# ZJU-FAST-Lab/Implicit-SVSDF-Planner

Measured on AMD Instinct MI355X. Metric: SVSDF query-points/sec (cost+grad) per optimizer evaluation, higher is better.
Workload: dtype f64

## Files before the change

implicit-svsdf-planner_amd/csrc/svsdf_body_classify.hpp:

```cpp
  extern __shared__ double classify_lds[];
  const TrajL tr = stage_traj(trg, classify_lds);
  const int start = ctl->start, count = ctl->count;
  const int lane = (int)(threadIdx.x & 63);
  for (int e0 = (int)((blockIdx.x * blockDim.x + threadIdx.x) & ~63u); e0 < count; e0 += gridDim.x * blockDim.x) {
    const int e = e0 + lane;
    const bool in_range = e < count;
    const int i = start + (in_range ? e : 0);
    const double px = px_[i], py = py_[i];
    const double sdf = sdf_[i], ts = t_[i];
    const bool inter = in_range && !(sdf > 0);
    double vx = 0.0, vy = 0.0, w = 0.0;
    if (in_range && sdf > 0) {
      int piece = 0;
      const Pose p = pose_at(tr, ts, piece);
      double rx, ry;
      if constexpr (SC) {
        double i00, i11;
        scale_inv(scl, ts, i00, i11);
        rel_scaled(p, px, py, i00, i11, rx, ry);
      } else {
        const double dx = px - p.x, dy = py - p.y;
        rx = p.cs * dx + p.sn * dy;
        ry = (-p.sn) * dx + p.cs * dy;
      }
      double gx, gy;
      shape_grad<SHAPE>(sp, rx, ry, gx, gy);
      res_sdf[i] = sdf; res_t[i] = ts; res_gx[i] = gx; res_gy[i] = gy;
    } else if (inter) {
      double sl;
      int piece = locate_local(tr, ts, 0, sl);
      piece_vel(tr.c + piece * 18, sl, vx, vy, w);
      if (sqrt(vx * vx + vy * vy + w * w) < 0.01) {
        if (ts < 0.1) {
          for (double t_scan = ts; t_scan <= tr.dur; t_scan += 0.1) {
            piece = locate_local(tr, t_scan, piece, sl);
            piece_vel(tr.c + piece * 18, sl, vx, vy, w);
            if (sqrt(vx * vx + vy * vy + w * w) >= 0.01) break;
          }
        } else if (ts > tr.dur - 0.1) {
          for (double t_scan = ts; t_scan >= 0; t_scan -= 0.1) {
// ... 41 lines not shown
```

implicit-svsdf-planner_amd/csrc/svsdf_capi.hip:

```cpp
#include "svsdf_ctx.hpp"

using namespace svsdf;
using namespace svsdf_impl;

namespace {

double shape_circumradius(int shape_id, const double *poly_xy, int nverts) {
  switch (shape_id) {
    case SVSDF_SHAPE_sdUnevenCapsule: return 6.0;
    case SVSDF_SHAPE_sdCutDisk: return 5.0;
    case SVSDF_SHAPE_sdTrapezoid: return std::sqrt(3.0 * 3.0 + 2.0 * 2.0);
    case SVSDF_SHAPE_sdRhombus: return 4.5;
    case SVSDF_SHAPE_star: return 2.8;
    case SVSDF_SHAPE_sdTunnel: return std::sqrt(2.5 * 2.5 + 1.5 * 1.5);
    case SVSDF_SHAPE_sdHorseshoe: return std::hypot(1.5 + 0.20, 1.55);
    case SVSDF_SHAPE_sdHeart: return 4.0 * (std::sqrt(0.25 * 0.25 + 0.75 * 0.75) + std::sqrt(2.0) / 4.0);
    case SVSDF_SHAPE_sdOrientedVesica: return std::sqrt(2.0 * 2.0 + 4.0 * 4.0);
    case SVSDF_SHAPE_sdRoundedCross: return 2.0;
    case SVSDF_SHAPE_sdRoundedX: return 3.0 / std::sqrt(2.0) + 0.25;
    case SVSDF_SHAPE_bigX: return 5.0 / std::sqrt(2.0) + 0.25;
    case SVSDF_SHAPE_sdMoon: return 3.0;
    case SVSDF_SHAPE_sdPie: return 3.0;
    case SVSDF_SHAPE_sdPie2: return 3.0;
    case SVSDF_SHAPE_sdArc: return 2.3333 + 0.5;
// ... 136 lines not shown
    pa.hdr.slabs = reinterpret_cast<const PolyRec *>(ctx->d_poly + o_slab);
    pa.hdr.over = reinterpret_cast<const unsigned short *>(ctx->d_poly + o_over);
    std::memcpy(blob.data(), &pa.hdr, sizeof(PolyAccel));
    std::memcpy(blob.data() + o_edges, pa.edges.data(), pa.edges.size() * sizeof(PolyEdge));
    std::memcpy(blob.data() + o_cell, pa.cells.data(), pa.cells.size() * sizeof(PolyRec));
    std::memcpy(blob.data() + o_slab, pa.slabs.data(), pa.slabs.size() * sizeof(PolyRec));
    if (!pa.over.empty()) std::memcpy(blob.data() + o_over, pa.over.data(), pa.over.size() * sizeof(unsigned short));
    if (hipMemcpy(ctx->d_poly, blob.data(), total, hipMemcpyHostToDevice) != hipSuccess)
      return bail("hipMemcpy polygon failed");
    sp.nverts = (int)pa.edges.size();
    sp.accel = reinterpret_cast<const PolyAccel *>(ctx->d_poly);
    sp.edges = pa.hdr.edges;
    ctx->poly_lds = sp.nverts <= kPolyLdsMaxVerts;
    if (const char *e = std::getenv("SVSDF_POLY_LDS")) ctx->poly_lds = ctx->poly_lds && std::atoi(e) != 0;
    ctx->cfg.polygon_nverts = (int)(v.size() / 2);
    ctx->cfg.polygon_nloops = (int)loops.size();
  }
  ctx->G_env = 0;
  if (const char *e = std::getenv("SVSDF_G")) { const int g = std::atoi(e); if (g == 1 || g == 2 || g == 4 || g == 8 || g == 16 || g == 32) { ctx->G_env = g; ctx->G = g; ctx->G_late = std::max(g, 8); } }
  if (const char *e = std::getenv("SVSDF_G_LATE")) { const int g = std::atoi(e); if (g == 1 || g == 2 || g == 4 || g == 8 || g == 16 || g == 32) { ctx->G_late = g; ctx->G_late_env = g; } }
  if (const char *e = std::getenv("SVSDF_PRUNE")) ctx->prune = std::atoi(e) != 0;
  if (const char *e = std::getenv("SVSDF_BATCHES")) ctx->want_batches = (std::string(e) == "measure") ? -1 : std::max(0, std::min(std::atoi(e), (int)kMaxBatches));
  if (const char *e = std::getenv("SVSDF_SELECT_DELTA")) { ctx->select_delta = std::atof(e); ctx->select_env = true; }
  {
    int n = 0;
    if (hipDeviceGetAttribute(&n, hipDeviceAttributeMultiprocessorCount, ctx->device) == hipSuccess && n > 0) ctx->n_cu = n;
    if (hipDeviceGetAttribute(&n, hipDeviceAttributeMaxSharedMemoryPerBlock, ctx->device) == hipSuccess && n > 0) ctx->lds_limit = (size_t)n;
    if (hipDeviceGetAttribute(&n, hipDeviceAttributeWallClockRate, ctx->device) == hipSuccess && n > 0) ctx->wall_clock_khz = (double)n;
  }
  if (const char *e = std::getenv("SVSDF_CULL")) { ctx->cull = std::atoi(e) != 0; ctx->cull2 = std::atoi(e) >= 2; }
  if (const char *e = std::getenv("SVSDF_ROUND_BPC")) ctx->round_blocks_per_cu = std::max(1, std::min(std::atoi(e), 16));
  if (const char *e = std::getenv("SVSDF_SCAN_ANCHORS")) ctx->scan_anchors = std::atoi(e) != 0;
  if (const char *e = std::getenv("SVSDF_LAYER_TABLES")) { const int v = std::atoi(e); ctx->layer_tables = (std::string(e) == "auto") ? -1 : (v == 0 || v == 2 || v == 3) ? v : -1; }
  if (const char *e = std::getenv("SVSDF_TAIL_DUO")) ctx->tail_duo = std::atoi(e) != 0;
  if (const char *e = std::getenv("SVSDF_TAIL_LOCAL")) ctx->tail_local = std::atoi(e) != 0;
  if (const char *e = std::getenv("SVSDF_TAIL_LATENCY")) ctx->tail_latency = std::atoi(e) != 0;
  if (const char *e = std::getenv("SVSDF_TAIL")) ctx->tail_mode = (std::string(e) == "off") ? -2 : (std::string(e) == "auto") ? -1 : std::max(0, std::atoi(e));
  if (const char *e = std::getenv("SVSDF_UB_FULL")) { ctx->ub_full = std::atoi(e) != 0; ctx->ub_lazy = std::atoi(e) == 2; ctx->ub_anchor = std::atoi(e) == 3; ctx->ub_env = true; }
  if (const char *e = std::getenv("SVSDF_PROFILE")) ctx->profile = std::atoi(e) != 0;
  if (const char *e = std::getenv("SVSDF_PIECE_TIME")) {
    ctx->cfg.flags &= ~(SVSDF_FLAG_EXACT_PIECE_TIME | SVSDF_FLAG_FAST_PIECE_TIME);
    if (std::string(e) == "exact") ctx->cfg.flags |= SVSDF_FLAG_EXACT_PIECE_TIME;
    else if (std::string(e) == "fast") ctx->cfg.flags |= SVSDF_FLAG_FAST_PIECE_TIME;
  }
  for (int b = 0; b < kMaxBatches; ++b) {
    if (hipEventCreateWithFlags(&ctx->ev_done[b], hipEventDisableTiming) != hipSuccess)
      return bail("event creation failed");
  }
  if (hipEventCreateWithFlags(&ctx->ev_prep, hipEventDisableTiming) != hipSuccess) return bail("event creation failed");
  if (hipMalloc((void **)&ctx->d_traj, sizeof(TrajDev)) != hipSuccess ||
      hipMalloc((void **)&ctx->d_ctl, kMaxBatches * sizeof(BatchCtl) + 8 * 8 * (kMaxIter + 4)) != hipSuccess ||
      hipMalloc((void **)&ctx->d_nonfinite, sizeof(int)) != hipSuccess ||
      hipMalloc((void **)&ctx->d_sums, kOutPartial * sizeof(double)) != hipSuccess ||
      hipMalloc((void **)&ctx->d_out, kOutDoubles * sizeof(double)) != hipSuccess ||
      hipHostMalloc((void **)&ctx->h_out, kOutDoubles * sizeof(double), hipHostMallocDefault) != hipSuccess ||
      hipMalloc((void **)&ctx->d_ticket, sizeof(unsigned)) != hipSuccess)
    return bail("device allocation failed");
  if (hipMemsetAsync(ctx->d_ticket, 0, sizeof(unsigned), ctx->stream) != hipSuccess) return bail("hipMemset failed");
  {
    void *dp = nullptr;
    const char *e = std::getenv("SVSDF_HOST_WRITE");
    if (!(e && std::atoi(e) == 0) && hipHostGetDevicePointer(&dp, ctx->h_out, 0) == hipSuccess) ctx->h_out_dev = (double *)dp;
    (void)hipGetLastError();
  }
  if (hipMemsetAsync(ctx->d_ctl, 0, kMaxBatches * sizeof(BatchCtl) + 8 * 8 * (kMaxIter + 4), ctx->stream) != hipSuccess) return bail("hipMemset failed");
  {
    const double r0 = shape_circumradius(cfg->shape_id, ctx->poly_xy.data(), (int)(ctx->poly_xy.size() / 2));
    const double analytic = (r0 + std::hypot(sp.tx, sp.ty)) * (1.0 + 1e-12) + 1e-6;
    if (hipMemsetAsync(ctx->d_out, 0, 2 * sizeof(double), ctx->stream) != hipSuccess) return bail("hipMemset failed");
    const int nrad = 512, nang = 4096;
    const unsigned grid = (unsigned)((nrad * nang + kBlock - 1) / kBlock);
    (void)launch_k_rbound(cfg->shape_id, grid, ctx->stream, ctx->sp, 60.0, nrad, nang, ctx->d_out);
    double rbl[2] = {0.0, 0.0};
    if (hipMemcpyAsync(rbl, ctx->d_out, 2 * sizeof(double), hipMemcpyDeviceToHost, ctx->stream) != hipSuccess ||
        hipStreamSynchronize(ctx->stream) != hipSuccess)
      return bail("shape bound kernel failed");
    const double rb = rbl[0];
    ctx->r_bound_sampled = rb;
    ctx->lipschitz_excess = rbl[1];
    const char *nl = std::getenv("SVSDF_ASSUME_NOT_LIPSCHITZ");
    if (rbl[1] > 0.0 || (nl && std::atoi(nl) != 0)) { ctx->lipschitz_ok = false; ctx->cull2 = false; }
    if (rb > analytic)
      return bail("svsdf_create: sampled shape bound " + std::to_string(rb) + " exceeds the analytic circumradius " +
                  std::to_string(analytic) + " (internal error: the pruning bound would be unsafe)");
    ctx->r_bound = analytic;
    ctx->sp.r_bound = ctx->r_bound;
  }
  return ctx;
}

void svsdf_destroy(svsdf_ctx *ctx) {
  if (!ctx) return;
  if (ctx->host_only) { delete ctx; return; }
  if (!ctx->subs.empty() || !ctx->workers.empty()) {
    destroy_group_resources(ctx);
    for (svsdf_ctx *s : ctx->subs) svsdf_destroy(s);
    delete ctx;
    return;
  }
  (void)hipSetDevice(ctx->device);
  (void)hipDeviceSynchronize();
  void *bufs[] = {ctx->d_poly, ctx->d_px, ctx->d_py, ctx->d_traj, ctx->d_in, ctx->d_pose, ctx->d_chunks, ctx->d_ltab,
                  ctx->d_sdf, ctx->d_t, ctx->d_res_sdf, ctx->d_res_t, ctx->d_res_gx, ctx->d_res_gy, ctx->gs.pt,
                  ctx->gs.r, ctx->gs.theta0, ctx->gs.theta_res, ctx->gs.iter, ctx->gs.nsamp, ctx->gs.phase, ctx->gs.req,
                  ctx->gs.list[0], ctx->gs.list[1], ctx->gs.solve, ctx->gs.sqx, ctx->gs.sqy, ctx->gs.sqth,
                  ctx->gs.sq_ub, ctx->gs.sq_k, ctx->gs.sq_sdf, ctx->gs.sq_t, ctx->d_ctl,
                  ctx->d_block_partials, ctx->d_sums,
                  ctx->d_out, ctx->d_nonfinite, ctx->d_fe, ctx->d_fe_flag, ctx->d_ticket};
  for (void *p : bufs)
    if (p) (void)hipFree(p);
  if (ctx->h_in) (void)hipHostFree(ctx->h_in);
  if (ctx->h_out) (void)hipHostFree(ctx->h_out);
  if (ctx->h_fe) (void)hipHostFree(ctx->h_fe);
  for (hipEvent_t e : ctx->ev_pool) (void)hipEventDestroy(e);
  if (ctx->ev_prep) (void)hipEventDestroy(ctx->ev_prep);
  for (int b = 0; b < kMaxBatches; ++b)
    if (ctx->ev_done[b]) (void)hipEventDestroy(ctx->ev_done[b]);
  if (ctx->stream_slot >= 0) {
    StreamSet ss;
    ss.main = ctx->stream;
    for (int b = 0; b < kMaxBatches; ++b) ss.batch[b] = ctx->bstream[b];
    ss.slot = ctx->stream_slot;
    release_streams(ctx->device, ss);
  }
  delete ctx;
}

int svsdf_set_points(svsdf_ctx *ctx, const double *xyz_aos, size_t P) {
  if (!ctx || (!xyz_aos && P)) return fail(ctx, SVSDF_ERR_INVALID, "svsdf_set_points: null argument");
  return set_points_host(ctx, xyz_aos, P);
}

int svsdf_set_points_device(svsdf_ctx *ctx, const double *d_xyz_aos, size_t P) {
  if (!ctx || (!d_xyz_aos && P)) return fail(ctx, SVSDF_ERR_INVALID, "svsdf_set_points_device: null argument");
  if (ctx->host_only) return fail(ctx, SVSDF_ERR_NO_DEVICE, "host-only context: no device entry points");
  if (P > 0xffffffffull) return fail(ctx, SVSDF_ERR_INVALID, "too many points");
  if (ctx->subs.empty()) {
    const auto t0 = std::chrono::steady_clock::now();
// ... 159 lines not shown
    const int nb = ctx->saved_nbatch;
    ctx->saved_nbatch = 0;
    HIPCHK(hipSetDevice(ctx->device));
    return set_batches(ctx, nb);
  }
  return SVSDF_OK;
}

int svsdf_shape_bound(const svsdf_ctx *ctx, double out2[2]) {
  if (!ctx || !out2) return SVSDF_ERR_INVALID;
  const svsdf_ctx *c = ctx->subs.empty() ? ctx : ctx->subs[0];
  out2[0] = c->r_bound;
  out2[1] = c->r_bound_sampled;
  return SVSDF_OK;
}

int svsdf_shape_selfcheck(const svsdf_ctx *ctx, double out3[3]) {
  if (!ctx || !out3) return SVSDF_ERR_INVALID;
  const svsdf_ctx *c = ctx->subs.empty() ? ctx : ctx->subs[0];
  out3[0] = c->r_bound;
  out3[1] = c->r_bound_sampled;
  out3[2] = c->lipschitz_ok ? 0.0 : std::max(c->lipschitz_excess, 1e-300);
  return SVSDF_OK;
}

int svsdf_get_plan(const svsdf_ctx *ctx, svsdf_plan *out) {
  if (!ctx || !out) return SVSDF_ERR_INVALID;
  const svsdf_ctx *c = ctx->subs.empty() ? ctx : ctx->subs[0];
  out->bound_mode = bound_mode_of(c);
  out->batches = (c->saved_nbatch > 0) ? c->saved_nbatch : c->nbatch;
  out->lanes_per_query = (c->scaled && c->G > 0) ? svsdf::scaled_lanes(c->G) : c->G;
  out->tail_iter = (c->tail_mode == -2 || c->scaled) ? -2 : (c->tail_mode >= 0) ? c->tail_mode : (c->have_prev_nactive ? choose_tail_iter(c) : SVSDF_PLAN_AUTO);
  out->layer_tables = c->layer_tables;
  out->settled = ((c->ub_env || c->ub_tune > 0) && c->bt_state == 0 && c->an_state == 0 && c->lz_state == 0 && c->have_prev_nsolve) ? 1 : 0;
  return SVSDF_OK;
}

int svsdf_set_plan(svsdf_ctx *ctx, const svsdf_plan *plan) {
  if (!ctx || !plan) return fail(ctx, SVSDF_ERR_INVALID, "svsdf_set_plan: null argument");
  const int g = plan->lanes_per_query;
  if (plan->bound_mode < SVSDF_PLAN_AUTO || plan->bound_mode > 3 || plan->batches < -2 || plan->batches == 0 || plan->batches > kMaxBatches ||
      !(g == SVSDF_PLAN_AUTO || g == 1 || g == 2 || g == 4 || g == 8 || g == 16 || g == 32) || plan->tail_iter < -2 || plan->tail_iter >= kMaxIter ||
      !(plan->layer_tables == SVSDF_PLAN_AUTO || plan->layer_tables == 0 || plan->layer_tables == 2 || plan->layer_tables == 3))
    return fail(ctx, SVSDF_ERR_INVALID, "svsdf_set_plan: field out of range");
  if (!ctx->subs.empty()) {
    int rc = SVSDF_OK;
    for (svsdf_ctx *s : ctx->subs) { const int r = svsdf_set_plan(s, plan); if (r && !rc) { rc = r; ctx->err = s->err; } }
    return rc;
  }
  if (ctx->host_only) return SVSDF_OK;
  HIPCHK(hipSetDevice(ctx->device));
  ctx->layer_tables = plan->layer_tables;
  if (plan->bound_mode == SVSDF_PLAN_AUTO) {
    if (ctx->ub_env) { ctx->ub_env = false; ctx->ub_tune = 0; ctx->have_prev_nsolve = false; ctx->have_prev_nactive = false; }
  } else {
    const bool full = plan->bound_mode != 0, lazy = plan->bound_mode == 2, anchor = plan->bound_mode == 3;
    if (!ctx->ub_env || full != ctx->ub_full || lazy != ctx->ub_lazy || anchor != ctx->ub_anchor) { ctx->have_prev_nsolve = false; ctx->have_prev_nactive = false; ctx->ub_tune = 0; }
    ctx->ub_env = true; ctx->ub_full = full; ctx->ub_lazy = lazy; ctx->ub_anchor = anchor; ctx->an_state = 0; ctx->lz_state = 0;
  }
  ctx->want_batches = (plan->batches == SVSDF_PLAN_AUTO) ? 0 : (plan->batches == -2) ? -1 : plan->batches;
  ctx->bt_state = 0;
  if (ctx->want_batches <= 0) ctx->ub_tune = 0;
  else if (ctx->points_set) {
    if (ctx->saved_nbatch > 0) ctx->saved_nbatch = ctx->want_batches;
    else if (ctx->nbatch != ctx->want_batches) { const int rc = set_batches(ctx, ctx->want_batches); if (rc) return rc; }
  }
  ctx->G_env = (g == SVSDF_PLAN_AUTO) ? 0 : g;
  if (ctx->G_env) { ctx->G = g; if (!ctx->G_late_env) ctx->G_late = std::max(g, 8); }
  else if (ctx->points_set) {
    const size_t Ps = ctx->P;
    ctx->G = default_lanes(ctx, Ps);
    if (!ctx->G_late_env) ctx->G_late = std::max(ctx->G, 8);
  }
  ctx->tail_mode = (plan->tail_iter == SVSDF_PLAN_AUTO) ? -1 : plan->tail_iter;
  return SVSDF_OK;
}

int svsdf_set_scale(svsdf_ctx *ctx, const svsdf_scale *scale) {
  if (!ctx) return SVSDF_ERR_INVALID;
  svsdf::ScaleDev d{};
  bool on = false;
  if (scale) {
    if (scale->struct_size != (int)sizeof(svsdf_scale))
      return fail(ctx, SVSDF_ERR_INVALID, "svsdf_set_scale: struct_size is not sizeof(svsdf_scale)");
    on = scale->enabled != 0;
// ... 213 lines not shown
```

implicit-svsdf-planner_amd/csrc/svsdf_ctx.hpp:

```cpp
#pragma once
#include <hip/hip_runtime.h>

#include <dlfcn.h>

#include <algorithm>
#include <chrono>
#include <cmath>
#include <condition_variable>
#include <cstdint>
#include <cstdio>
#include <cstdlib>
#include <cstring>
#include <functional>
#include <limits>
#include <memory>
#include <mutex>
#include <numeric>
#include <string>
#include <thread>
#include <vector>

#include "../../include/svsdf_c.h"
#include "svsdf_launch.hpp"
#include "svsdf_minco.hpp"
// ... 29 lines not shown
    done = false;
    cv.notify_all();
  }
  int wait() {
    std::unique_lock<std::mutex> lk(m);
    cv.wait(lk, [this] { return done; });
    return rc;
  }
  ~Worker() {
    { std::lock_guard<std::mutex> lk(m); quit = true; cv.notify_all(); }
    if (th.joinable()) th.join();
  }
};

struct svsdf_ctx {
  svsdf_config cfg{};
  int device = 0;
  hipStream_t stream = nullptr;
  hipStream_t bstream[svsdf::kMaxBatches] = {};
  int stream_slot = -1;
  hipEvent_t ev_prep = nullptr, ev_done[svsdf::kMaxBatches] = {};
  svsdf::ShapeParams sp{};
  bool poly_lds = false;
  unsigned char *d_poly = nullptr;
  std::vector<double> poly_xy;
  std::vector<int> poly_loops;
  std::string err;

  size_t P = 0;
  bool points_set = false;
  std::vector<long long> shard_idx;
  double *d_px = nullptr, *d_py = nullptr;
  int nbatch = 1;
  int bstart[svsdf::kMaxBatches] = {}, bcount[svsdf::kMaxBatches] = {};
  svsdf::BatchCtl *d_ctl = nullptr;

  svsdf::TrajDev *d_traj = nullptr;
  double *d_in = nullptr;
  double *h_in = nullptr;
  size_t in_cap = 0;
  svsdf::Pose *d_pose = nullptr;
  svsdf::Chunk *d_chunks = nullptr;
  size_t pose_cap = 0;
  svsdf::Pose *d_ltab = nullptr;
  size_t ltab_cap = 0;
  int layer_tables = -1;
  int ltab_mode = 0;
  long long prev_solves = 0;
  double r_bound = 0.0;
  double r_bound_sampled = 0.0;
  double lipschitz_excess = 0.0;
  bool lipschitz_ok = true;
  double traj_duration = 0.0;
  bool have_duration = false;
  bool host_only = false;
  int N = 0, K = 0;
  int piece_time_mode = 0;
  int stats_piece_time = 0;

  int G = 0 , G_late = 8, prune = 1, block = 64, want_batches = 0, waves_per_cu = 16;
  bool block_env = false;
  int late_iter = 4, first_iters = 12, it_done = 0, round_lp8_iters = 3, delta_all_iter = 5;
  int n_cu = 256;
  int round_blocks_per_cu = 4;
  double wall_clock_khz = 100000.0;
  bool adaptive_iters = true;
  bool ub_full = false;
// ... 3 lines not shown
  unsigned long long an_full_evals = 0;
  int lz_state = 0;
  unsigned long long lz_cheap_solves = 0;
  bool ub_env = false;
  int ub_tune = 0;
  double ub_ratio = 0.0;
  double ub_threshold = 0.5;
  bool ub_thr_env = false;
  bool scan_anchors = true;
  int round_list = 3;
  bool cull = true;
  bool cull_ok = false;
  bool cull2 = true;
  double slack_max = 0.0;
  int G_env = 0, G_late_env = 0;
  int bt_state = 0, bt_k = 0, bt_rep = 0, bt_ncand = 0, bt_cand[3] = {1, 1, 1};
  double bt_ms[3] = {0, 0, 0}, bt_samples[3] = {0, 0, 0};
  long long prev_nsolve[svsdf::kMaxIter] = {};
  bool have_prev_nsolve = false;
  int tail_mode = -1;
  long long tail_below = 0;
  int tail_all_after = 1 << 30;
  int tail_iter = -1;
  bool tail_duo = true;
  bool tail_latency = true;
  bool tail_local = true;
  long long prev_nactive[svsdf::kMaxIter] = {};
  int prev_tail_iter = -1;
  bool have_prev_nactive = false;
  long long wide32_below = 2000, wide16_below = 5000, wide8_below = 40000;
  bool select_env = false, all_iter_env = false;
  double scan_delta = 0.002;
  double select_delta = 0.1;
  bool scaled = false;
  svsdf::ScaleDev scale{};

  double *d_sdf = nullptr, *d_t = nullptr;
  double *d_res_sdf = nullptr, *d_res_t = nullptr, *d_res_gx = nullptr, *d_res_gy = nullptr;
  svsdf::GsipState gs{};
  size_t icap = 0;
  bool icap_fitted = false;
  double *d_block_partials = nullptr;
  size_t block_partials_cap = 0;
  double *d_sums = nullptr;
  double *d_out = nullptr;
  double *h_out = nullptr;
  double *h_out_dev = nullptr;
  unsigned *d_ticket = nullptr;
  int *d_nonfinite = nullptr;
  int h_nonfinite = 0;
  size_t e_end = 0;

  double *d_fe = nullptr, *h_fe = nullptr;
  size_t fe_cap = 0;
  int *d_fe_flag = nullptr;
  std::vector<int> h_fe_flag;
  size_t fe_edges_cap = 0;

  bool profile = false;
  bool profile_span = false;
  int saved_nbatch = 0;
  std::vector<hipEvent_t> ev_pool;
  size_t ev_used = 0;
  std::vector<std::pair<size_t, size_t>> refine_events;
  std::vector<std::pair<size_t, size_t>> round_events;
  std::vector<std::pair<size_t, size_t>> tail_events;
  svsdf_stats stats{};
  svsdf_launch_rec launches[SVSDF_LAUNCH_REC_CAP];
  int n_launches = 0;

  std::vector<svsdf_ctx *> subs;
  std::vector<std::unique_ptr<Worker>> workers;
  int combine = 0;
  std::vector<void *> comms;
  std::vector<double *> d_red;
  double *h_red = nullptr;
  std::vector<double> comb;
  const double *h_partial = nullptr;
  double combine_ms = 0.0, setup_ms = 0.0, fanout_ms = 0.0;
  bool group_serial = false;

  std::vector<double> ol_key, ol_xy;
  std::vector<int> ol_loops;
  svsdf_outline_stats ol_stats{};
  bool ol_valid = false;
  size_t lds_limit = 65536;
  std::string launch_err;

  svsdf_host::MincoS3 minco;
  std::vector<double> T, pgC, pgT, cm, gC, gradq, gradT, xlast;
  double energy_cost = 0.0;
  double costs3[3] = {0, 0, 0};
};

namespace svsdf_impl {

constexpr size_t kOutPartial = 19 * svsdf::kMaxPieces + 1;
constexpr size_t kOutDoubles = kOutPartial + 14 + 2 * svsdf::kMaxIter;
constexpr int kRepeat = -12345;

extern thread_local std::string g_last_error;
extern const char *kShapeNames[SVSDF_SHAPE_COUNT];
int fail(svsdf_ctx *ctx, int code, const std::string &msg);

#define HIPCHK(expr)                                                                              \
  do {                                                                                            \
    hipError_t e_ = (expr);                                                                       \
    if (e_ != hipSuccess)                                                                         \
      return fail(ctx, SVSDF_ERR_HIP_BASE + (int)e_, std::string(#expr) + ": " + hipGetErrorString(e_)); \
  } while (0)

template <typename T>
int dev_alloc(svsdf_ctx *ctx, T **p, size_t count) {
  if (*p) { (void)hipFree(*p); *p = nullptr; }
  if (count == 0) count = 1;
  HIPCHK(hipMalloc((void **)p, count * sizeof(T)));
  return SVSDF_OK;
}

inline int bound_mode_of(const svsdf_ctx *c) { return c->ub_full ? (c->ub_lazy ? 2 : ((c->ub_anchor && c->lipschitz_ok) ? 3 : 1)) : 0; }
inline int default_lanes(const svsdf_ctx *ctx, size_t Ps) {
  const int g = (Ps < 3000) ? 32 : (Ps < 20000) ? 16 : (Ps < 75000) ? 8 : (Ps < 150000) ? 4 : 2;
  return (ctx->cfg.shape_id == (int)svsdf::kPolygon) ? std::max(g, 4) : g;
}

struct StreamSet { hipStream_t main = nullptr; hipStream_t batch[svsdf::kMaxBatches] = {}; int slot = -1; };
bool acquire_streams(int device, StreamSet &out);
void release_streams(int device, StreamSet &s);
int set_batches(svsdf_ctx *ctx, int nb);
int choose_tail_iter(const svsdf_ctx *ctx);
int swept_field(svsdf_ctx *ctx, int N, const double *coeffs, const double *T, double *sdf_sorted);
int evaluate_points(svsdf_ctx *ctx, int N, const double *coeffs, const double *T, bool allow_cull, bool with_partial);
void fill_mode_stats(svsdf_ctx *ctx);
inline void reset_launches(svsdf_ctx *ctx) { ctx->n_launches = 0; }
inline svsdf_launch_rec *record_launch(svsdf_ctx *ctx, int kernel, int shape, unsigned grid, unsigned block, size_t lds,
                                       long long work, int batch) {
  if (ctx->n_launches >= SVSDF_LAUNCH_REC_CAP) { ++ctx->n_launches; return nullptr; }
  svsdf_launch_rec *r = &ctx->launches[ctx->n_launches++];
  *r = svsdf_launch_rec{};
  r->struct_size = (int)sizeof(svsdf_launch_rec);
  r->kernel = kernel; r->shape = shape; r->grid = grid; r->block = block; r->lds_bytes = lds; r->work = work; r->batch = batch;
  return r;
}
int compiled_shape(int shape);
int run_pipeline_leaf(svsdf_ctx *ctx, int N, const double *coeffs, const double *T);
void accumulate(int N, const double *partial, double *cost, double *gradT, double *gradC);
void shard_plan(const double *xyz, size_t P, int rk, int ws, int flags, std::vector<long long> &out);
struct CloudPlan {
  int device = 0;
  const double *d_xyz = nullptr;
  size_t P = 0;
  double *d_part = nullptr;
  unsigned long long *d_keys = nullptr, *d_keys2 = nullptr;
  const unsigned long long *sorted = nullptr;
  void *d_tmp = nullptr;
  void release();
};
int plan_cloud(svsdf_ctx *ctx, const double *d_xyz, size_t P, CloudPlan &plan);
int take_stripe(svsdf_ctx *ctx, svsdf_ctx *planner, const CloudPlan &plan, int rk, int ws);
int upload_shard_device(svsdf_ctx *ctx, const double *d_xyz, size_t P, int rk, int ws);
long long sincos_mismatches(svsdf_ctx *ctx, double lo, double hi, int n);
int debug_sdf_at(svsdf_ctx *ctx, int N, const double *coeffs, const double *T, size_t n, const double *pxy, const double *t, double *out8);
// ... 13 lines not shown
```

implicit-svsdf-planner_amd/csrc/svsdf_group.hip:

```cpp
#include "svsdf_ctx.hpp"

using namespace svsdf;

namespace svsdf_impl {

int upload_group_device(svsdf_ctx *ctx, const double *d_xyz, size_t P) {
  const int G = (int)ctx->subs.size();
  svsdf_ctx *s0 = ctx->subs[0];
  CloudPlan plan;
  int rc = plan_cloud(s0, d_xyz, P, plan);
  for (int k = 0; k < G && !rc; ++k) {
    rc = take_stripe(ctx->subs[k], s0, plan, ctx->cfg.rank * G + k, ctx->cfg.world_size * G);
    if (rc) {
      ctx->err = "device " + std::to_string(ctx->subs[k]->device) + " (stripe " + std::to_string(k) + "): " + ctx->subs[k]->err;
      g_last_error = ctx->err;
    }
  }
  if (rc && ctx->err.empty()) ctx->err = s0->err;
  plan.release();
  ctx->P = 0;
  ctx->shard_idx.clear();
  for (svsdf_ctx *s : ctx->subs) {
    if (rc) { s->P = 0; s->points_set = false; }
    ctx->P += s->P;
// ... 71 lines not shown
    if (!h)
      for (const char *name : {"librccl.so.1", "librccl.so", "/opt/rocm/lib/librccl.so.1"}) {
        h = dlopen(name, RTLD_NOW | RTLD_LOCAL);
        if (h) break;
      }
    if (!h) return false;
    CommInitAll = reinterpret_cast<decltype(CommInitAll)>(dlsym(h, "ncclCommInitAll"));
    CommDestroy = reinterpret_cast<decltype(CommDestroy)>(dlsym(h, "ncclCommDestroy"));
    AllReduce = reinterpret_cast<decltype(AllReduce)>(dlsym(h, "ncclAllReduce"));
    GetErrorString = reinterpret_cast<decltype(GetErrorString)>(dlsym(h, "ncclGetErrorString"));
    CommCount = reinterpret_cast<decltype(CommCount)>(dlsym(h, "ncclCommCount"));
    return CommInitAll && CommDestroy && AllReduce;
  }
};
RcclApi g_rccl;
constexpr int kNcclFloat64 = 8, kNcclSum = 0;

void merge_stats(svsdf_ctx *ctx) {
  svsdf_stats t{};
  for (svsdf_ctx *s : ctx->subs) {
    const svsdf_stats &a = s->stats;
    t.points += a.points; t.interior_points += a.interior_points; t.solves += a.solves;
    t.gsip_samples += a.gsip_samples; t.sdf_evals += a.sdf_evals; t.scan_evals += a.scan_evals;
    t.round_scan_evals += a.round_scan_evals; t.speculative_evals += a.speculative_evals;
    t.round_ms = std::max(t.round_ms, a.round_ms); t.round_ms_sum = std::max(t.round_ms_sum, a.round_ms_sum);
    t.batches = std::max(t.batches, a.batches);
    t.culled_points += a.culled_points;
    t.device_ms = std::max(t.device_ms, a.device_ms); t.solve_ms = std::max(t.solve_ms, a.solve_ms);
    t.solve_ms_sum = std::max(t.solve_ms_sum, a.solve_ms_sum);
    t.solve_launches = std::max(t.solve_launches, a.solve_launches);
    t.tail_launches = std::max(t.tail_launches, a.tail_launches);
    t.tail_iter = std::max(t.tail_iter, a.tail_iter);
    t.tail_points += a.tail_points;
    t.tail_ms = std::max(t.tail_ms, a.tail_ms); t.tail_ms_sum = std::max(t.tail_ms_sum, a.tail_ms_sum);
    t.gsip_iterations = std::max(t.gsip_iterations, a.gsip_iterations);
    t.gsip_bound_mode = std::max(t.gsip_bound_mode, a.gsip_bound_mode);
    t.piece_time_exact = std::max(t.piece_time_exact, a.piece_time_exact);
    t.bound_ratio = std::max(t.bound_ratio, a.bound_ratio);
    if (a.shader_clock_mhz > 0.0) t.shader_clock_mhz = (t.shader_clock_mhz > 0.0) ? std::min(t.shader_clock_mhz, a.shader_clock_mhz) : a.shader_clock_mhz;
  }
  t.bound_mode_decided = 1;
  t.plan_settled = 1;
  for (svsdf_ctx *s : ctx->subs) { t.bound_mode_decided &= s->stats.bound_mode_decided; t.plan_settled &= s->stats.plan_settled; }
  t.n_devices = (int)ctx->subs.size();
  t.combine = ctx->combine;
  t.combine_ms = ctx->combine_ms;
  t.fanout_ms = ctx->fanout_ms;
  t.setup_ms = ctx->setup_ms;
  ctx->stats = t;
}

int run_pipeline_group(svsdf_ctx *ctx, int N, const double *coeffs, const double *T) {
  const int G = (int)ctx->subs.size();
  const size_t plen = 19 * (size_t)N + 1;
  const bool rccl = ctx->combine == SVSDF_COMBINE_RCCL;
  int rc = group_run(ctx, [&](int k) -> int {
    svsdf_ctx *s = ctx->subs[k];
    int r = run_pipeline_leaf(s, N, coeffs, T);
    if (!rccl) return r;
    (void)hipSetDevice(s->device);
    if (r) (void)hipMemsetAsync(s->d_out, 0xFF, plen * sizeof(double), s->stream);
    const int e = g_rccl.AllReduce(s->d_out, ctx->d_red[k], plen, kNcclFloat64, kNcclSum, ctx->comms[k], s->stream);
    if (e && !r) r = fail(s, SVSDF_ERR_RCCL, std::string("ncclAllReduce: ") + (g_rccl.GetErrorString ? g_rccl.GetErrorString(e) : "error"));
    if (k == 0 && hipMemcpyAsync(ctx->h_red, ctx->d_red[0], plen * sizeof(double), hipMemcpyDeviceToHost, s->stream) != hipSuccess && !r)
      r = fail(s, SVSDF_ERR_RCCL, "read-back of the reduced partial failed");
    if (hipStreamSynchronize(s->stream) != hipSuccess && !r) r = fail(s, SVSDF_ERR_RCCL, "stream sync after ncclAllReduce failed");
// ... 137 lines not shown
```

implicit-svsdf-planner_amd/csrc/svsdf_kernels.hpp:

```cpp
#pragma once
#include <hip/hip_runtime.h>

#include "svsdf_shapes.hpp"

namespace svsdf {

#ifndef SVSDF_SOLVE_WAVES
#define SVSDF_SOLVE_WAVES 1
#endif
#ifndef SVSDF_ELASTIC
#define SVSDF_ELASTIC 1
#endif
#ifndef SVSDF_FUSED_PASS
#define SVSDF_FUSED_PASS 1
#endif
constexpr int kMaxPieces = 128;
constexpr int kMaxSlots = 24;
constexpr int kMaxRounds = 9;
constexpr int kBlock = 256;
constexpr int kMaxBatches = 8;
constexpr int kMaxCand = 48;
constexpr int kMaxIter = 24;
constexpr int kWorkCounters = kMaxIter + 2;
constexpr double kUnsolved = -1e300;
// ... 7 lines not shown
  double S[kMaxPieces + 1];
  double c[kMaxPieces * 18];
};

struct Pose { double x, y, cs, sn; };
constexpr int kLayerSteps = 21;
struct LayerTab { const Pose *l2, *l3; };

constexpr int kChunk = 8;
struct Chunk { double cx, cy, rb, slack; };
struct ChunkAnchor { double adx, rot2; int ka, pad_; double pad2_; };
#ifndef SVSDF_ANCHOR_MIN
#define SVSDF_ANCHOR_MIN 3
#endif

constexpr int kStatSlots = 32;
#ifdef SVSDF_SITE_STATS
struct StatSlot { unsigned long long solves, evals, scan, culled, round_scan, spec, pad[26]; };
#else
struct StatSlot { unsigned long long solves, evals, scan, culled, round_scan, spec, pad[10]; };
#endif
__device__ __forceinline__ StatSlot *stat_slot(StatSlot *slots) {
  return slots + (((blockIdx.x * blockDim.x + threadIdx.x) >> 6) & (kStatSlots - 1));
}
struct BatchCtl {
  int start, count;
  int n_active[kMaxIter + 2];
  int n_solve[kMaxIter + 2];
  int n_seed[kMaxIter + 2];
  unsigned work[kWorkCounters];
  unsigned rwork[kMaxIter + 2];
  int nonfinite;
  int n_int;
  StatSlot stat[kStatSlots];
  unsigned long long clk[2];
};

typedef const __attribute__((address_space(4))) double *UniformDoubles;

struct TrajL {
  const double *T, *S, *c;
  UniformDoubles Tu;
  int N;
  int exact;
  double dur;
};

__host__ __device__ __forceinline__ int traj_lds_doubles(int N) { return 20 * N + 1; }

__device__ __forceinline__ TrajL stage_traj(const TrajDev *__restrict__ g, double *lds) {
  const int N = g->N;
  double *T = lds, *S = lds + N, *c = lds + 2 * N + 1;
  for (int i = threadIdx.x; i < N; i += blockDim.x) T[i] = g->T[i];
  for (int i = threadIdx.x; i <= N; i += blockDim.x) S[i] = g->S[i];
  for (int i = threadIdx.x; i < 18 * N; i += blockDim.x) c[i] = g->c[i];
  __syncthreads();
  TrajL tr;
  tr.T = T; tr.S = S; tr.c = c; tr.N = N; tr.dur = g->dur; tr.exact = g->exact;
  tr.Tu = (UniformDoubles)(g->T);
  return tr;
}

template <int SHAPE>
__device__ __forceinline__ void stage_poly_edges(const ShapeParams &sp, double *lds) {
  if constexpr (SHAPE == kPolygonLds) {
    const double *src = reinterpret_cast<const double *>(sp.edges);
    for (int i = threadIdx.x; i < kPolyEdgeDoubles * sp.nverts; i += blockDim.x) lds[i] = src[i];
  }
}
// ... 260 lines not shown
  const double dx = px - p.x, dy = py - p.y;
  rx = (p.cs * i00) * dx + (p.sn * i11) * dy;
  ry = ((-p.sn) * i00) * dx + (p.cs * i11) * dy;
}
template <int SHAPE>
__device__ __forceinline__ double sdf_at_sc(const TrajL &tr, const ShapeParams &sp, const ScaleDev &scl, double px,
                                            double py, double t, PieceCache &pc) {
  const Pose p = pose_at(tr, t, pc);
  double i00, i11, rx, ry;
  scale_inv(scl, t, i00, i11);
  rel_scaled(p, px, py, i00, i11, rx, ry);
  return shape_sdf<SHAPE>(sp, rx, ry);
}
template <int SHAPE>
__device__ __forceinline__ double sdf_at_sc(const TrajL &tr, const ShapeParams &sp, const ScaleDev &scl, double px,
                                            double py, double t, int &piece) {
  const Pose p = pose_at(tr, t, piece);
  double i00, i11, rx, ry;
  scale_inv(scl, t, i00, i11);
  rel_scaled(p, px, py, i00, i11, rx, ry);
  return shape_sdf<SHAPE>(sp, rx, ry);
}
template <int SHAPE, bool SC, typename PC>
__device__ __forceinline__ double sdf_desc(const TrajL &tr, const ShapeParams &sp, const ScaleDev &scl, double px,
                                           double py, double t, PC &pc) {
  if constexpr (SC) return sdf_at_sc<SHAPE>(tr, sp, scl, px, py, t, pc);
  else return sdf_at<SHAPE>(tr, sp, px, py, t, pc);
}

#ifdef SVSDF_API_TU
__global__ void __launch_bounds__(1024) k_prep(const double *__restrict__ in, int N, double dur, int K, int exact,
                       TrajDev *__restrict__ tr, Pose *__restrict__ pose,
                       Chunk *__restrict__ chunks, double r_bound, BatchCtl *__restrict__ ctl,
                       int nbatch, int *__restrict__ nonfinite) {
  extern __shared__ double prep_lds[];
  if (threadIdx.x == 0 && nonfinite) *nonfinite = 0;
  const double *coeffs = in, *T = in + 18 * N, *tk = in + 19 * N, *slack = in + 19 * N + K;
  for (int b = threadIdx.x; b < nbatch; b += blockDim.x) {
    BatchCtl &c = ctl[b];
    for (int r = 0; r < kMaxIter + 2; ++r) { c.n_active[r] = 0; c.n_solve[r] = 0; c.n_seed[r] = 0; }
    for (int r = 0; r < kWorkCounters; ++r) c.work[r] = 0u;
    for (int r = 0; r < kMaxIter + 2; ++r) c.rwork[r] = 0u;
    c.nonfinite = 0;
    c.n_int = 0;
    c.clk[0] = 0ull; c.clk[1] = 0ull;
  }
  for (int i = threadIdx.x; i < nbatch * kStatSlots; i += blockDim.x) {
    StatSlot &ss = ctl[i / kStatSlots].stat[i % kStatSlots];
    ss.solves = 0ull; ss.evals = 0ull; ss.scan = 0ull; ss.culled = 0ull; ss.round_scan = 0ull; ss.spec = 0ull;
#ifdef SVSDF_SITE_STATS
    for (int j = 0; j < 26; ++j) ss.pad[j] = 0ull;
#endif
  }
  if (threadIdx.x == 0) {
    tr->N = N; tr->K = K; tr->dur = dur; tr->exact = exact;
    double s = 0.0;
    for (int i = 0; i < N; ++i) { tr->T[i] = T[i]; tr->S[i] = s; s += T[i]; }
    tr->S[N] = s;
  }
  for (int e = threadIdx.x; e < 18 * N; e += blockDim.x) {
    const int i = e / 18, k = (e % 18) / 3, d = e % 3;
    tr->c[e] = coeffs[(size_t)d * 6 * N + 6 * i + k];
  }
  __threadfence_block();
  __syncthreads();
  const TrajL tl = stage_traj(tr, prep_lds);
  for (int k = threadIdx.x; k < K; k += blockDim.x) {
    int piece = 0;
    pose[k] = pose_at(tl, tk[k], piece);
// ... 54 lines not shown
constexpr int kLayerRows = kLayerSteps + 2;
__global__ void __launch_bounds__(256) k_layer_tables(const TrajDev *__restrict__ trg, const double *__restrict__ tk, int K,
                                                      int rows , Pose *__restrict__ out) {
  extern __shared__ double lt_lds[];
  const TrajL tr = stage_traj(trg, lt_lds);
  const long long e = (long long)blockIdx.x * blockDim.x + threadIdx.x;
  if (e >= (long long)K * rows * kLayerSteps) return;
  const int i = (int)(e % kLayerSteps), r = (int)((e / kLayerSteps) % rows), k = (int)(e / ((long long)kLayerSteps * rows));
  double seed = tk[k];
  double dt = 0.15;
  dt *= 0.1;
  if (r > 0) {
    if (r >= 2) {
      const double t0 = dmax(0.0, seed - 10 * dt);
      const double loop_terminal = dmin(tr.dur, seed + 10 * dt);
      double t = t0;
      for (int j = 0; j < r - 2; ++j) t += dt;
      if (!(t <= loop_terminal)) return;
      seed = t;
    }
    dt *= 0.1;
  }
  const double t0 = dmax(0.0, seed - 10 * dt);
  const double loop_terminal = dmin(tr.dur, seed + 10 * dt);
  double t = t0;
  for (int j = 0; j < i; ++j) t += dt;
  if (!(t <= loop_terminal)) return;
  PieceCache pc = piece_cache_init();
  Pose *dst = (r == 0) ? out + (size_t)k * kLayerSteps
                       : out + (size_t)K * kLayerSteps + ((size_t)k * (kLayerSteps + 1) + (size_t)(r - 1)) * kLayerSteps;
  dst[i] = pose_at(tr, t, pc);
}

#endif

template <int SHAPE>
__global__ void k_rbound(ShapeParams sp, double rmax, int nrad, int nang, double *__restrict__ out) {
  const int idx = blockIdx.x * blockDim.x + threadIdx.x;
  double v = -1e300, lip = -1e300;
  if (idx < nrad * nang) {
    const int ir = idx / nang, ia = idx % nang;
    const double r = rmax * (double)(ir + 1) / (double)nrad;
    const double a = 2.0 * kPI * (double)ia / (double)nang;
    const double x = r * cos(a), y = r * sin(a);
    const double f0 = shape_sdf<SHAPE>(sp, x, y);
    v = r - f0;
    auto excess = [&](double xx, double yy) {
      const double d = norm2(xx - x, yy - y);
      return fabs(shape_sdf<SHAPE>(sp, xx, yy) - f0) - d * (1.0 + 1e-9) - 1e-12;
    };
    const double r2 = rmax * (double)(ir + 2) / (double)nrad, a2 = 2.0 * kPI * (double)(ia + 1) / (double)nang;
    lip = fmax(fmax(excess(x + 1e-3, y), excess(x, y + 1e-3)), fmax(excess(r2 * cos(a), r2 * sin(a)), excess(r * cos(a2), r * sin(a2))));
  }
  for (int m = 32; m >= 1; m >>= 1) { v = fmax(v, __shfl_xor(v, m, 64)); lip = fmax(lip, __shfl_xor(lip, m, 64)); }
  if ((threadIdx.x & 63) == 0) {
    if (v > 0.0) atomicMax((unsigned long long *)out, (unsigned long long)__double_as_longlong(v));
    if (lip > 0.0) atomicMax((unsigned long long *)(out + 1), (unsigned long long)__double_as_longlong(lip));
  }
}

struct QuerySet {
  const double *qx, *qy;
  size_t stride;
  const int *count_ptr;
  int count_fixed;
  const int *list;
  int base;
  int n_outer;
  const int *slots;
  const int *seed_k;
  const double *seed_d;
};

__device__ __forceinline__ long long qs_total(const QuerySet &qs, int &n) {
  n = qs.count_ptr ? *qs.count_ptr : qs.count_fixed;
  return qs.slots ? (long long)n : (long long)n * qs.n_outer;
}
__device__ __forceinline__ bool qs_slot(const QuerySet &qs, int n, long long q, size_t &slot) {
  if (qs.slots) { slot = (size_t)qs.slots[q]; return true; }
  const int e = (int)(q % n), j = (int)(q / n);
  const int a = qs.list ? qs.list[e] : e;
  slot = (size_t)j * qs.stride + (size_t)qs.base + (size_t)a;
  return true;
}

#ifdef SVSDF_SITE_STATS
#define SVSDF_SITE(cnt, site, evaluates)                                                     \
  do {                                                                                       \
    const unsigned long long ex__ = __ballot(1);                                             \
    if ((int)(threadIdx.x & 63) == __ffsll((long long)ex__) - 1) ++(cnt)[site];              \
    if (evaluates) ++(cnt)[4 + (site)];                                                      \
  } while (0)
#define SVSDF_SITE_CLOCK() ((unsigned long long)__builtin_readcyclecounter())
#define SVSDF_SITE_CYCLES(cnt, slot, t0) do { if ((threadIdx.x & 63) == 0) (cnt)[slot] += SVSDF_SITE_CLOCK() - (t0); } while (0)
#define SVSDF_PHASE(cnt, slot, t0) do { if ((threadIdx.x & 63) == 0) { const unsigned long long n__ = SVSDF_SITE_CLOCK(); (cnt)[slot] += n__ - (t0); (t0) = n__; } } while (0)
#else
#define SVSDF_SITE(cnt, site, evaluates) do { } while (0)
#define SVSDF_SITE_CLOCK() 0ull
#define SVSDF_SITE_CYCLES(cnt, slot, t0) do { (void)(t0); } while (0)
#define SVSDF_PHASE(cnt, slot, t0) do { (void)(t0); } while (0)
#endif

template <int G>
struct Grp {
  static_assert(G == 1 || G == 2 || G == 4 || G == 8 || G == 16 || G == 32, "group size");
  __device__ static __forceinline__ int li() { return (int)(threadIdx.x & (G - 1)); }
  __device__ static __forceinline__ double bcast(double v, int src) {
    if constexpr (G == 1) return v; else return __shfl(v, src, G);
  }
  template <int STEP>
  __device__ static __forceinline__ int xchg(int v) {
    if constexpr (STEP == 0) return __builtin_amdgcn_update_dpp(v, v, 0xB1, 0xF, 0xF, false);
    else if constexpr (STEP == 1) return __builtin_amdgcn_update_dpp(v, v, 0x4E, 0xF, 0xF, false);
    else if constexpr (STEP == 2) return __builtin_amdgcn_update_dpp(v, v, 0x141, 0xF, 0xF, false);
    else if constexpr (STEP == 3) return __builtin_amdgcn_update_dpp(v, v, 0x140, 0xF, 0xF, false);
    else return __shfl_xor(v, 16, 32);
// ... 649 lines not shown
#define SVSDF_LAZY_REPS 2
#endif
enum : int { kPhaseEval = 0, kPhaseSupp = 1, kPhaseNew = 2 };
#ifndef SVSDF_LEAN_HANDOFF
#define SVSDF_LEAN_HANDOFF 0
#endif
#ifdef SVSDF_POINT_MAJOR
__host__ __device__ __forceinline__ size_t sample_slot(size_t , size_t ia, int j) { return ia * (size_t)kMaxSlots + (size_t)j; }
#else
__host__ __device__ __forceinline__ size_t sample_slot(size_t stride, size_t ia, int j) { return (size_t)j * stride + ia; }
#endif

struct GsipState {
  int *pt;
  double *r;
  double *theta0;
  double *theta_res;
  int *iter;
  int *nsamp;
  int *phase;
  unsigned *req;
  int *list[2];
  int *solve;
  double *sqx, *sqy, *sqth, *sq_ub, *sq_sdf, *sq_t;
  int *sq_k;
};

template <int SHAPE>
__global__ void __launch_bounds__(kBlock)
k_classify(const TrajDev *__restrict__ trg, ShapeParams sp, const double *__restrict__ px_,
           const double *__restrict__ py_, const double *__restrict__ sdf_,
           const double *__restrict__ t_, double *__restrict__ res_sdf,
           double *__restrict__ res_t, double *__restrict__ res_gx, double *__restrict__ res_gy,
           GsipState gs, BatchCtl *__restrict__ ctl, int *__restrict__ n_int, int icap) {
  constexpr bool SC = false;
  const ScaleDev scl{};
#include "svsdf_body_classify.hpp"
}
template <int SHAPE>
__global__ void __launch_bounds__(kBlock)
k_classify_sc(const TrajDev *__restrict__ trg, ShapeParams sp, const double *__restrict__ px_,
              const double *__restrict__ py_, const double *__restrict__ sdf_,
              const double *__restrict__ t_, double *__restrict__ res_sdf,
              double *__restrict__ res_t, double *__restrict__ res_gx, double *__restrict__ res_gy,
              GsipState gs, BatchCtl *__restrict__ ctl, int *__restrict__ n_int, int icap, ScaleDev scl) {
  constexpr bool SC = true;
#include "svsdf_body_classify.hpp"
}

template <int NP>
struct RoundOut {
  bool list_me[NP];
  unsigned mlist[NP];
  int n_emit;
  bool push_next, finished;
};
template <int SHAPE, int LP, int MODE, bool EAGER = false>
__device__ __forceinline__ void round_point(const ShapeParams &sp, const Pose *pose, const Chunk *chunks, int K, int nch,
                                            const double *__restrict__ px_, const double *__restrict__ py_,
                                            const GsipState &gs, size_t stride, int start, int a, double delta,
                                            double band_delta, double *__restrict__ res_sdf, double *__restrict__ res_t,
                                            double *__restrict__ res_gx, double *__restrict__ res_gy, unsigned &n_scan,
                                            RoundOut<(kMaxSlots + LP - 1) / LP> &out, unsigned short *clist, int clist_on,
                                            unsigned long long (&rc)[16], int duo = -1, const ChunkAnchor *__restrict__ anch_ = nullptr) {
#ifdef SVSDF_NO_SCAN_ANCHORS
  const ChunkAnchor *__restrict__ anch = nullptr; (void)anch_;
#else
#ifdef SVSDF_ANCHORS_NOT_LP8_M3
  const ChunkAnchor *__restrict__ anch = (MODE == 1 || (MODE == 3 && LP == 32)) ? anch_ : nullptr;
#else
  const ChunkAnchor *__restrict__ anch = ((MODE == 1 || MODE == 3) && !is_polygon<SHAPE>()) ? anch_ : nullptr;
#endif
#endif
  constexpr bool FULL = MODE == 1;
  unsigned long long tph = SVSDF_SITE_CLOCK();
  constexpr int NP = (kMaxSlots + LP - 1) / LP;
  const int l = (int)(threadIdx.x & (LP - 1));
  const unsigned lt_mask = (1u << l) - 1u;
// ... 673 lines not shown
  if (live) {
    const unsigned e = qlist[q];
    slot = (size_t)(e & 0x7fffffffu);
    px = gs.sqx[slot]; py = gs.sqy[slot];
    const bool seeded = (e >> 31) != 0u;
    if (seeded) { best_k = gs.sq_k[slot]; best_d = gs.sq_ub[slot]; }
    if (!seeded || best_k < 0) {
      bool culled;
      scan_layer1<SHAPE, G>(sp, pose, chunks, K, nch, px, py, prune, __longlong_as_double(0x7ff0000000000000ll), best_d, best_k,
                            culled, n_scan, nullptr, -1, nullptr);
    }
  }
  SVSDF_SITE_CYCLES(sc, 8, t_scan0);
  double x = 0.0, fx = 0.0;
  descend_from_seed<SHAPE, G, 1>(tr, tk, sp, px, py, live, best_k, best_d, x, fx, n_eval, n_spec, sc, wave_lds);
  if (live && li == 0) {
    gs.sq_sdf[slot] = fx;
    gs.sq_t[slot] = x;
    ++n_solved;
  }
}

#ifndef SVSDF_TAIL_WAVES
#define SVSDF_TAIL_WAVES 3
#endif
constexpr int kTailLatencyWaves = 2;
template <int SHAPE, int MODE, int WAVES = SVSDF_TAIL_WAVES>
__global__ void __launch_bounds__(kTailBlock, WAVES)
k_tail(const TrajDev *__restrict__ trg, const double *__restrict__ tk, const Pose *__restrict__ pose_g,
       const Chunk *__restrict__ chunks_g, ShapeParams sp, const double *__restrict__ px_, const double *__restrict__ py_,
       GsipState gs, size_t stride, int it0, int prev_mode, double delta, double band_delta, int all_after, int ppw,
       double *__restrict__ res_sdf, double *__restrict__ res_t, double *__restrict__ res_gx, double *__restrict__ res_gy,
       BatchCtl *__restrict__ ctl, int clist_on, int prune) {
  extern __shared__ double tail_lds[];
  constexpr int LP = 32;
  const int n_act = ctl->n_active[it0];
  const int wave_g = (int)((blockIdx.x * blockDim.x + threadIdx.x) >> 6);
  if (n_act <= 0 || (int)blockIdx.x * (kTailBlock / 64) * ppw >= n_act) return;
  const int K = trg->K;
  const int nch = (K + kChunk - 1) / kChunk;
  stage_poly_edges<SHAPE>(sp, tail_lds);
  double *tab_lds = tail_lds + poly_lds_doubles<SHAPE>(sp.nverts);
  Pose *pose = reinterpret_cast<Pose *>(tab_lds);
  Chunk *chunks = reinterpret_cast<Chunk *>(tab_lds + 4 * (size_t)K);
  {
    const double *src = reinterpret_cast<const double *>(pose_g);
    for (int i = threadIdx.x; i < 4 * K; i += blockDim.x) tab_lds[i] = src[i];
    const double *srcc = reinterpret_cast<const double *>(chunks_g);
    for (int i = threadIdx.x; i < 4 * nch; i += blockDim.x) tab_lds[4 * (size_t)K + i] = srcc[i];
  }
  const TrajL tr = stage_traj(trg, tab_lds + 4 * (size_t)K + 4 * (size_t)nch);
  const size_t tables = poly_lds_doubles<SHAPE>(sp.nverts) + 4 * (size_t)K + 4 * (size_t)nch + (size_t)traj_lds_doubles(tr.N);
  const bool local = it0 == 0 && (clist_on & 4) != 0;
  const size_t wave_stride = local ? kTailWaveLds : kTailWaveLds - kTailLocalBytes;
  char *wave_lds = reinterpret_cast<char *>(tail_lds + ((tables + 1) & ~(size_t)1)) + (threadIdx.x >> 6) * wave_stride;
  unsigned short *clist_w = reinterpret_cast<unsigned short *>(wave_lds + ((ladder_lds_bytes(2) + 15) & ~(size_t)15));
  unsigned *qlist = reinterpret_cast<unsigned *>(clist_w + 2 * kMaxCand);
  GsipState gl = gs;
  if (local) {
    double *ld = reinterpret_cast<double *>(qlist + 64);
    gl.r = ld; gl.theta0 = ld + 2; gl.theta_res = ld + 4;
    gl.sqx = ld + 6; gl.sqy = gl.sqx + 2 * kMaxSlots; gl.sqth = gl.sqy + 2 * kMaxSlots; gl.sq_ub = gl.sqth + 2 * kMaxSlots;
    gl.sq_sdf = gl.sq_ub + 2 * kMaxSlots; gl.sq_t = gl.sq_sdf + 2 * kMaxSlots;
    int *li_ = reinterpret_cast<int *>(gl.sq_t + 2 * kMaxSlots);
    gl.pt = li_; gl.iter = li_ + 2; gl.nsamp = li_ + 4; gl.phase = li_ + 6; gl.req = reinterpret_cast<unsigned *>(li_ + 8);
    gl.sq_k = li_ + 10;
  }
  const GsipState ga = local ? gl : gs;
  const size_t stride_a = local ? (size_t)2 : stride;
  const int start = ctl->start;
  const int *cur = gs.list[it0 & 1] + start;
  const int lane = (int)(threadIdx.x & 63);
  const int h = lane >> 5, l = lane & (LP - 1);
  const bool duo = ppw == 1 && MODE != 0 && (clist_on & 8) == 0;
  const int hs = duo ? 0 : h;
  const unsigned lt_mask = (1u << l) - 1u;
  unsigned n_eval = 0, n_scan = 0, n_solved = 0, n_spec = 0, n_rscan = 0;
  unsigned long long rc[16] = {0, 0, 0, 0, 0, 0, 0, 0, 0, 0, 0, 0, 0, 0, 0, 0};
  unsigned long long sc[12] = {0, 0, 0, 0, 0, 0, 0, 0, 0, 0, 0, 0};
  const unsigned long long t_wave0 = SVSDF_SITE_CLOCK();
  int n_emit_tot = 0;
  const int n_static = (int)(gridDim.x * (blockDim.x >> 6)) * ppw;
  int q_next = wave_g * ppw, q_end = min(wave_g * ppw + ppw, n_act);
  bool exhausted = false;
  int a = -1;
  int steps = 0;
  bool own = false;
  for (int guard = 0; guard < (1 << 24); ++guard) {
#pragma unroll
    for (int hh = 0; hh < 2; ++hh) {
      const int ah = __builtin_amdgcn_readlane(a, hh * 32);
      if (ah >= 0 || hh >= ppw) continue;
      if (q_next >= q_end && !exhausted) {
        unsigned b = 0;
        if (lane == 0) b = atomicAdd(&ctl->work[min(it0 + 1, kWorkCounters - 1)], (unsigned)kTailFetch);
        b = __builtin_amdgcn_readfirstlane(b);
        const long long bb = (long long)b + n_static;
        if (bb >= n_act) exhausted = true;
        else { q_next = (int)bb; q_end = (int)min((long long)n_act, bb + kTailFetch); }
      }
      if (q_next < q_end) {
        const int e = q_next++;
        if (h == hh || duo) {
          a = cur[e]; steps = 0; own = false;
          if (local && l == 0 && h == hh) {
            const size_t ia_ = (size_t)a;
            gl.pt[hs] = gs.pt[ia_]; gl.r[hs] = gs.r[ia_]; gl.theta0[hs] = gs.theta0[ia_]; gl.theta_res[hs] = gs.theta_res[ia_];
            gl.iter[hs] = gs.iter[ia_]; gl.nsamp[hs] = gs.nsamp[ia_]; gl.phase[hs] = gs.phase[ia_]; gl.req[hs] = 0u;
          }
        }
      }
    }
    if (__builtin_amdgcn_readlane(a, 0) < 0 && __builtin_amdgcn_readlane(a, 32) < 0) break;
    if (local) {
      __builtin_amdgcn_fence(__ATOMIC_RELEASE, "workgroup");
      __builtin_amdgcn_wave_barrier();
      __builtin_amdgcn_fence(__ATOMIC_ACQUIRE, "workgroup");
    }
    RoundOut<1> ro;
    ro.list_me[0] = false; ro.mlist[0] = 0u; ro.n_emit = 0; ro.push_next = false; ro.finished = false;
    if (a >= 0) {
      const double dl = (steps >= all_after) ? 1e300 : delta, bd = (steps >= all_after) ? 1e300 : band_delta;
      round_point<SHAPE, LP, MODE, true>(sp, pose, chunks, K, nch, px_, py_, ga, stride_a, start, local ? hs : a, dl, bd, res_sdf, res_t, res_gx,
                                   res_gy, n_rscan, ro, clist_w + (size_t)h * kMaxCand, clist_on, rc, duo ? h : -1,
                                   (clist_on & 16) ? reinterpret_cast<const ChunkAnchor *>(chunks_g + nch) : nullptr);
      ++steps;
      if (ro.n_emit > 0) own = true;
      if (l == 0 && (!duo || h == 0)) n_emit_tot += ro.n_emit;
    }
    const size_t ia = local ? (size_t)hs : (size_t)(a >= 0 ? a : 0);
    if (ro.finished) a = -1;
    const unsigned m_mine = (a >= 0 && (!duo || h == 0)) ? ro.mlist[0] : 0u;
    const int n0 = __popc((unsigned)__builtin_amdgcn_readlane((int)m_mine, 0));
    const int n1 = __popc((unsigned)__builtin_amdgcn_readlane((int)m_mine, 32));
    const int nq = n0 + n1;
    if ((m_mine >> l) & 1u) {
      const bool seeded = own ? (MODE != 0) : (prev_mode != 0);
      qlist[(h ? n0 : 0) + __popc(m_mine & lt_mask)] = (unsigned)sample_slot(stride_a, ia, l) | (seeded ? 0x80000000u : 0u);
    }
    __builtin_amdgcn_fence(__ATOMIC_RELEASE, "workgroup");
    __builtin_amdgcn_wave_barrier();
    __builtin_amdgcn_fence(__ATOMIC_ACQUIRE, "workgroup");
    if (nq > 0) {
      if (nq <= 2) {
        tail_solve_pass<SHAPE, 32>(tr, tk, sp, pose, chunks, K, nch, ga, qlist, 0, nq, prune, wave_lds, n_eval, n_scan, n_solved, n_spec, sc);
      } else if (nq <= 8) {
        tail_solve_pass<SHAPE, 8>(tr, tk, sp, pose, chunks, K, nch, ga, qlist, 0, nq, prune, wave_lds, n_eval, n_scan, n_solved, n_spec, sc);
      } else {
        for (int base = 0; base < nq; base += 32)
          tail_solve_pass<SHAPE, 2>(tr, tk, sp, pose, chunks, K, nch, ga, qlist, base, nq, prune, wave_lds, n_eval, n_scan, n_solved, n_spec, sc);
      }
      __builtin_amdgcn_fence(__ATOMIC_RELEASE, "workgroup");
      __builtin_amdgcn_wave_barrier();
      __builtin_amdgcn_fence(__ATOMIC_ACQUIRE, "workgroup");
    }
  }
  unsigned long long te = (unsigned long long)n_eval + n_scan, ts = n_solved, tc = n_scan, tp = n_spec, tr_ = n_rscan;
  int em = n_emit_tot;
#pragma unroll
  for (int m = 32; m >= 1; m >>= 1) {
    te += __shfl_xor(te, m, 64); ts += __shfl_xor(ts, m, 64); tc += __shfl_xor(tc, m, 64); tp += __shfl_xor(tp, m, 64);
    tr_ += __shfl_xor(tr_, m, 64); em += __shfl_xor(em, m, 64);
  }
  if (lane == 0 && (te || tr_ || em)) {
    StatSlot *ss = stat_slot(ctl->stat);
    if (te) atomicAdd(&ss->evals, te);
    if (ts) atomicAdd(&ss->solves, ts);
    if (tc) atomicAdd(&ss->scan, tc);
    if (tp) atomicAdd(&ss->spec, tp);
    if (tr_) atomicAdd(&ss->round_scan, tr_);
    if (em) atomicAdd(&ctl->n_seed[it0], em);
    if (ts) atomicAdd(&ctl->n_solve[it0], (int)ts);
  }
#ifdef SVSDF_SITE_STATS
  if (lane == 0) {
    rc[6] = SVSDF_SITE_CLOCK() - t_wave0;
    StatSlot *ss = stat_slot(ctl->stat);
    for (int i = 0; i < 8; ++i) if (rc[i]) atomicAdd(&ss->pad[12 + i], rc[i]);
    for (int i = 8; i < 11; ++i) if (sc[i]) atomicAdd(&ss->pad[i], sc[i]);
  }
  {
    unsigned long long ex = rc[8], ln = rc[12];
#pragma unroll
    for (int m = 32; m >= 1; m >>= 1) { ex += __shfl_xor(ex, m, 64); ln += __shfl_xor(ln, m, 64); }
    if (lane == 0 && ex) { StatSlot *ss = stat_slot(ctl->stat); atomicAdd(&ss->pad[20], ex); atomicAdd(&ss->pad[21], ln); }
    unsigned long long steps = ex;
#pragma unroll
    for (int i = 0; i < 4; ++i) {
      unsigned long long v = sc[i];
#pragma unroll
      for (int m = 32; m >= 1; m >>= 1) v += __shfl_xor(v, m, 64);
      steps += v;
    }
    if (lane == 0) { StatSlot *ss = stat_slot(ctl->stat); atomicMax(&ss->pad[22], steps); atomicMax(&ss->pad[23], rc[6]); }
  }
#pragma unroll
  for (int i = 0; i < 8; ++i) {
    unsigned long long v = sc[i];
#pragma unroll
    for (int m = 32; m >= 1; m >>= 1) v += __shfl_xor(v, m, 64);
    if (lane == 0 && v) atomicAdd(&stat_slot(ctl->stat)->pad[i], v);
  }
#endif
}

__device__ __forceinline__ bool smoothed_l1(double x, double mu, double &f, double &df) {
  if (x < 0.0) return false;
  else if (x > mu) { f = x - 0.5 * mu; df = 1.0; return true; }
  else {
    const double xdmu = x / mu;
    const double sqrxdmu = xdmu * xdmu;
    const double mumxd2 = mu - 0.5 * x;
    f = mumxd2 * sqrxdmu * xdmu;
    df = sqrxdmu * ((-0.5) * xdmu + 3.0 * mumxd2 / mu);
    return true;
  }
}

#ifdef SVSDF_API_TU
template <bool SC = false>
__device__ __forceinline__ bool assemble_terms(const TrajL &tr, const double *__restrict__ px_, const double *__restrict__ py_,
                                               int idx, const double *__restrict__ res_sdf, const double *__restrict__ res_t,
                                               const double *__restrict__ res_gx, const double *__restrict__ res_gy,
                                               double safety_hor, double weight_p, double (&v)[20], int &i, int &bad,
                                               const ScaleDev &scl = ScaleDev{}) {
  const double px = px_[idx], py = py_[idx];
  const double sdf_value = res_sdf[idx];
  const double time_star = res_t[idx];
  double gr0 = res_gx[idx], gr1 = res_gy[idx];
  if (!(sdf_value == sdf_value) || !(time_star == time_star) || !(gr0 == gr0) || !(gr1 == gr1)) ++bad;
  double sdf_cost = -1.0, sdf_out_grad = 0.0;
  smoothed_l1(safety_hor - sdf_value, 0.01, sdf_cost, sdf_out_grad);
  if (!(sdf_cost > 0)) return false;
  double s1;
  i = locate_local(tr, time_star, 0, s1);
  const double *c = tr.c + i * 18;
// ... 154 lines not shown
                                            const int *__restrict__ nonfinite, unsigned long long *__restrict__ stats_out) {
  for (int k = threadIdx.x; k <= 18 * N; k += blockDim.x) partial[k] = sums[k];
  if (threadIdx.x == 0) {
    double suf = 0.0;
    for (int j = N - 1; j >= 0; --j) { partial[1 + 18 * N + j] = suf; suf += sums[1 + 18 * N + j]; }
  }
  if (threadIdx.x < 64) {
    const int lane = (int)threadIdx.x;
    unsigned long long so = 0, ev = 0, sc = 0, cu = 0, rs = 0, sp_ = 0, seeded = 0, iters = 0, ns = 0, na = 0;
    for (int b = 0; b < nbatch; ++b) {
      if (lane < kStatSlots) {
        const StatSlot &ss = ctl[b].stat[lane];
        so += ss.solves; ev += ss.evals; sc += ss.scan; cu += ss.culled; rs += ss.round_scan; sp_ += ss.spec;
      }
      if (lane < kMaxIter) {
        ns += (unsigned long long)ctl[b].n_solve[lane];
        na += (unsigned long long)ctl[b].n_active[lane];
      }
      if (lane <= it_end && lane < kMaxIter + 2) {
        seeded += (unsigned long long)ctl[b].n_seed[lane];
        if (ctl[b].n_solve[lane] > 0 && (unsigned long long)(lane + 1) > iters) iters = (unsigned long long)(lane + 1);
      }
    }
#pragma unroll
    for (int m = 32; m >= 1; m >>= 1) {
      so += __shfl_xor(so, m, 64); ev += __shfl_xor(ev, m, 64); sc += __shfl_xor(sc, m, 64); cu += __shfl_xor(cu, m, 64);
      rs += __shfl_xor(rs, m, 64); sp_ += __shfl_xor(sp_, m, 64); seeded += __shfl_xor(seeded, m, 64);
      const unsigned long long oi = __shfl_xor(iters, m, 64);
      iters = (oi > iters) ? oi : iters;
    }
    if (lane < kMaxIter) {
      stats_out[9 + lane] = ns;
      stats_out[11 + kMaxIter + lane] = na;
    }
    if (lane == 0) {
      unsigned long long in = 0, nf = (unsigned long long)__hip_atomic_load(nonfinite, __ATOMIC_RELAXED, __HIP_MEMORY_SCOPE_AGENT), rem = 0;
      for (int b = 0; b < nbatch; ++b) {
        in += (unsigned long long)ctl[b].n_active[0]; nf += (unsigned long long)ctl[b].nonfinite;
        rem += (unsigned long long)ctl[b].n_solve[it_end];
      }
      stats_out[0] = so; stats_out[1] = ev; stats_out[2] = sc; stats_out[3] = in; stats_out[4] = nf;
      stats_out[5] = rem; stats_out[6] = seeded; stats_out[7] = iters; stats_out[8] = cu;
      stats_out[9 + kMaxIter] = rs;
      stats_out[10 + kMaxIter] = sp_;
      stats_out[11 + 2 * kMaxIter] = (unsigned long long)ctl[0].n_int;
      stats_out[12 + 2 * kMaxIter] = ctl[0].clk[0];
      stats_out[13 + 2 * kMaxIter] = ctl[0].clk[1];
    }
  }
}

__device__ __forceinline__ void copy_result_to_host(double *__restrict__ host_out, const double *__restrict__ out, int N,
                                                    int out_partial, int out_doubles) {
  const int plen = 19 * N + 1;
  for (int k = threadIdx.x; k < plen; k += blockDim.x) host_out[k] = out[k];
  for (int k = out_partial + threadIdx.x; k < out_doubles; k += blockDim.x) host_out[k] = out[k];
}

__global__ void k_finish(const double *__restrict__ sums, int N, double *__restrict__ partial,
                         const BatchCtl *__restrict__ ctl, int nbatch, int it_end,
                         const int *__restrict__ nonfinite, unsigned long long *__restrict__ stats_out,
                         double *__restrict__ host_out, int out_doubles) {
  finish_body(sums, N, partial, ctl, nbatch, it_end, nonfinite, stats_out);
  if (host_out) {
    __threadfence();
    __syncthreads();
    copy_result_to_host(host_out, partial, N, (int)(reinterpret_cast<const double *>(stats_out) - partial), out_doubles);
  }
}

__global__ void __launch_bounds__(kBlock)
k_reduce(const TrajDev *__restrict__ trg, const double *__restrict__ px_, const double *__restrict__ py_, int P,
         const double *__restrict__ res_sdf, const double *__restrict__ res_t, const double *__restrict__ res_gx,
         const double *__restrict__ res_gy, double safety_hor, double weight_p, double *__restrict__ block_partials,
         int *__restrict__ nonfinite, double *__restrict__ out, const BatchCtl *__restrict__ ctl, int nbatch, int it_end,
         int out_partial, int out_doubles, unsigned *__restrict__ ticket, double *__restrict__ host_out, int fuse) {
  constexpr bool SC = false;
  const ScaleDev scl{};
#include "svsdf_body_reduce.hpp"
}
// ... 87 lines not shown
```

implicit-svsdf-planner_amd/csrc/svsdf_launch.hpp:

```cpp
#pragma once
#include <hip/hip_runtime.h>

#include "svsdf_kernels.hpp"
#include "svsdf_frontend.hpp"

namespace svsdf {

constexpr int kNSlices = 4;

struct SolveLaunch {
  const TrajDev *traj; const double *tk; const Pose *pose; const Chunk *chunks; ShapeParams sp; QuerySet qs;
  double *out_sdf, *out_t; int prune; BatchCtl *ctl; int work_idx; double cull_thresh;
  const double *rot; double slack_max;
  const ScaleDev *scl = nullptr;
  const Pose *ltab = nullptr;
};
struct RoundLaunch {
  const TrajDev *traj; const Pose *pose; const Chunk *chunks; ShapeParams sp; const double *px, *py; GsipState gs;
  size_t stride; int it; double delta, band_delta; double *res_sdf, *res_t, *res_gx, *res_gy; BatchCtl *ctl;
  int clist_on;
};
struct TailLaunch {
  const TrajDev *traj; const double *tk; const Pose *pose; const Chunk *chunks; ShapeParams sp; const double *px, *py;
  GsipState gs; size_t stride; int it0, prev_mode; double delta, band_delta; int all_after, ppw;
  double *res_sdf, *res_t, *res_gx, *res_gy; BatchCtl *ctl; int clist_on, prune;
  int latency;
};
struct ClassifyLaunch {
  const TrajDev *traj; ShapeParams sp; const double *px, *py, *sdf, *t; double *res_sdf, *res_t, *res_gx, *res_gy;
  GsipState gs; BatchCtl *ctl; int *n_int; int icap;
  const ScaleDev *scl = nullptr;
};
constexpr int kScaledLanes[3] = {4, 8, 32};
inline int scaled_lanes(int G) { return G >= 32 ? 32 : G >= 8 ? 8 : 4; }

bool launch_k_solve(int shape, int G, unsigned grid, unsigned block, size_t lds, hipStream_t st, const SolveLaunch &a);
bool launch_k_round(int shape, int lp, int mode, unsigned grid, size_t lds, hipStream_t st, const RoundLaunch &a);
bool launch_k_classify(int shape, unsigned grid, size_t lds, hipStream_t st, const ClassifyLaunch &a);
bool launch_k_tail(int shape, int mode, unsigned grid, size_t lds, hipStream_t st, const TailLaunch &a);
bool launch_k_rbound(int shape, unsigned grid, hipStream_t st, ShapeParams sp, double rmax, int nrad, int nang, double *out);
bool launch_k_subsw(int shape, dim3 grid, hipStream_t st, ShapeParams sp, const double *father, const double *child,
                    const unsigned long long *offs, const double *pts, const double *kt, int nkt, int *flag);
bool launch_k_shape_kernels(int shape, unsigned grid, hipStream_t st, ShapeParams sp, int ks, int count, double resu,
                            int size_side, double safemargin, const double *yaw, unsigned char *map);
bool launch_k_debug_sdf_at(int shape, unsigned grid, size_t lds, hipStream_t st, const TrajDev *traj, ShapeParams sp,
                           const double *pxy, const double *t, int n, double *out, const ScaleDev *scl = nullptr);

#define SVSDF_DECLARE_SLICE(K)                                                                                              \
  bool launch_k_solve_s##K(int shape, int G, unsigned grid, unsigned block, size_t lds, hipStream_t st, const SolveLaunch &a); \
  bool launch_k_round_s##K(int shape, int lp, int mode, unsigned grid, size_t lds, hipStream_t st, const RoundLaunch &a);      \
  bool launch_k_classify_s##K(int shape, unsigned grid, size_t lds, hipStream_t st, const ClassifyLaunch &a);                  \
  bool launch_k_tail_s##K(int shape, int mode, unsigned grid, size_t lds, hipStream_t st, const TailLaunch &a);                \
  bool launch_k_rbound_s##K(int shape, unsigned grid, hipStream_t st, ShapeParams sp, double rmax, int nrad, int nang, double *out); \
  bool launch_k_subsw_s##K(int shape, dim3 grid, hipStream_t st, ShapeParams sp, const double *father, const double *child,    \
                           const unsigned long long *offs, const double *pts, const double *kt, int nkt, int *flag);         \
  bool launch_k_shape_kernels_s##K(int shape, unsigned grid, hipStream_t st, ShapeParams sp, int ks, int count, double resu,   \
                                   int size_side, double safemargin, const double *yaw, unsigned char *map);                   \
  bool launch_k_debug_sdf_at_s##K(int shape, unsigned grid, size_t lds, hipStream_t st, const TrajDev *traj, ShapeParams sp,    \
                                  const double *pxy, const double *t, int n, double *out, const ScaleDev *scl);
SVSDF_DECLARE_SLICE(0)
SVSDF_DECLARE_SLICE(1)
SVSDF_DECLARE_SLICE(2)
SVSDF_DECLARE_SLICE(3)
#undef SVSDF_DECLARE_SLICE
// ... 3 lines not shown
```

implicit-svsdf-planner_amd/csrc/svsdf_pipeline.hip:

```cpp
#include <hipcub/hipcub.hpp>

#define SVSDF_API_TU
#include "svsdf_ctx.hpp"

using namespace svsdf;

namespace svsdf_impl {

thread_local std::string g_last_error;

int fail(svsdf_ctx *ctx, int code, const std::string &msg) {
  g_last_error = msg;
  if (ctx) ctx->err = msg;
  return code;
}

const char *kShapeNames[SVSDF_SHAPE_COUNT] = {
    "sdUnevenCapsule", "sdCutDisk", "sdTrapezoid", "sdRhombus", "star", "sdTunnel",
    "sdHorseshoe", "sdHeart", "sdOrientedVesica", "sdRoundedCross", "sdRoundedX", "bigX",
    "sdMoon", "sdPie", "sdPie2", "sdArc", "Polygon"};
inline uint32_t part1by1(uint32_t x) {
  x &= 0x0000ffff;
  x = (x ^ (x << 8)) & 0x00ff00ff;
  x = (x ^ (x << 4)) & 0x0f0f0f0f;
// ... 93 lines not shown
  shape = svsdf_impl::compiled_shape(shape);
  SVSDF_SLICE_DISPATCH(launch_k_round, lp, mode, grid, lds, st, a)
}
bool launch_k_classify(int shape, unsigned grid, size_t lds, hipStream_t st, const ClassifyLaunch &a) {
  shape = svsdf_impl::compiled_shape(shape);
  SVSDF_SLICE_DISPATCH(launch_k_classify, grid, lds, st, a)
}
bool launch_k_tail(int shape, int mode, unsigned grid, size_t lds, hipStream_t st, const TailLaunch &a) {
  shape = svsdf_impl::compiled_shape(shape);
  SVSDF_SLICE_DISPATCH(launch_k_tail, mode, grid, lds, st, a)
}
bool launch_k_rbound(int shape, unsigned grid, hipStream_t st, ShapeParams sp, double rmax, int nrad, int nang, double *out) {
  shape = svsdf_impl::compiled_shape(shape);
  SVSDF_SLICE_DISPATCH(launch_k_rbound, grid, st, sp, rmax, nrad, nang, out)
}
bool launch_k_subsw(int shape, dim3 grid, hipStream_t st, ShapeParams sp, const double *father, const double *child,
                    const unsigned long long *offs, const double *pts, const double *kt, int nkt, int *flag) {
  shape = svsdf_impl::compiled_shape(shape);
  SVSDF_SLICE_DISPATCH(launch_k_subsw, grid, st, sp, father, child, offs, pts, kt, nkt, flag)
}
bool launch_k_debug_sdf_at(int shape, unsigned grid, size_t lds, hipStream_t st, const TrajDev *traj, ShapeParams sp,
                           const double *pxy, const double *t, int n, double *out, const ScaleDev *scl) {
  shape = svsdf_impl::compiled_shape(shape);
  SVSDF_SLICE_DISPATCH(launch_k_debug_sdf_at, grid, lds, st, traj, sp, pxy, t, n, out, scl)
}
bool launch_k_shape_kernels(int shape, unsigned grid, hipStream_t st, ShapeParams sp, int ks, int count, double resu,
                            int size_side, double safemargin, const double *yaw, unsigned char *map) {
  shape = svsdf_impl::compiled_shape(shape);
  SVSDF_SLICE_DISPATCH(launch_k_shape_kernels, grid, st, sp, ks, count, resu, size_side, safemargin, yaw, map)
}
}
namespace svsdf_impl {

size_t table_lds_doubles(const svsdf_ctx *ctx) {
  return 4 * (size_t)ctx->K + 4 * (size_t)((ctx->K + kChunk - 1) / kChunk);
}

void launch_solve(svsdf_ctx *ctx, int G, hipStream_t st, const QuerySet &qs, long long max_queries, double *out_sdf,
                  double *out_t, BatchCtl *ctl, int work_idx,
                  double cull_thresh = std::numeric_limits<double>::infinity()) {
  const double *d_tk = ctx->d_in + 19 * (size_t)ctx->N;
  if (ctx->scaled) {
    G = scaled_lanes(G);
    cull_thresh = std::numeric_limits<double>::infinity();
  }
  const bool solo = G == 32 && !ctx->G_env && max_queries <= (long long)ctx->n_cu * 4;
  const long long lanes = std::max<long long>(max_queries * (solo ? 64 : G), 64);
  const size_t wlds = ladder_lds_bytes(G);
  bool poly_lds = ctx->poly_lds;
  size_t lds = 0, lds_total = 0;
  int blk = ctx->block;
  for (int attempt = 0; attempt < 2; ++attempt) {
    lds = (table_lds_doubles(ctx) + (size_t)traj_lds_doubles(ctx->N) + (poly_lds ? (size_t)svsdf::kPolyEdgeDoubles * (size_t)ctx->sp.nverts : 0)) * sizeof(double);
    blk = ctx->block;
    if (!ctx->block_env) blk = ((lds + wlds) * 12 <= 160 * 1024) ? 64 : ((lds + 2 * wlds) * 6 <= 160 * 1024) ? 128 : 256;
    lds_total = ((lds + 15) & ~(size_t)15) + (size_t)(blk / 64) * wlds;
    if (lds_total <= ctx->lds_limit || !poly_lds) break;
    poly_lds = false;
  }
  if (lds_total > ctx->lds_limit) {
    if (ctx->launch_err.empty()) ctx->launch_err = "trajectory too long for the LDS pose table (" + std::to_string(lds_total) + " B of " + std::to_string(ctx->lds_limit) + " B per block)";
    return;
  }
  const unsigned grid = (unsigned)std::min<long long>((lanes + blk - 1) / blk, (long long)(256 * ctx->waves_per_cu * 64) / blk);
  size_t e0 = 0, e1 = 0;
  if (ctx->profile) { e0 = next_event(ctx); (void)hipEventRecord(ctx->ev_pool[e0], st); }
// ... 23 lines not shown
  const long long pts = std::max(1, ctx->bcount[b]);
  bool poly_lds = ctx->poly_lds;
  size_t lds = (table_lds_doubles(ctx) + (poly_lds ? (size_t)svsdf::kPolyEdgeDoubles * (size_t)ctx->sp.nverts : 0)) * sizeof(double);
  if (lds + 16384 > ctx->lds_limit && poly_lds) {
    poly_lds = false;
    lds = table_lds_doubles(ctx) * sizeof(double);
  }
  if (lds + 16384 > ctx->lds_limit) {
    if (ctx->launch_err.empty()) ctx->launch_err = "trajectory too long for the LDS pose table (k_round)";
    return;
  }
  const double sel = (scans && !ctx->select_env) ? ctx->scan_delta : ctx->select_delta;
  const int all_it = (scans && !ctx->all_iter_env) ? 7 : ctx->delta_all_iter;
  const double delta = (it >= all_it || ctx->scaled) ? 1e300 : sel;
  const double band_delta = (it >= all_it || ctx->scaled) ? 1e300 : ctx->select_delta;
  const int lp = (it < ctx->round_lp8_iters + (mode == 2 ? 1 : 0)) ? 8 : 32;
  const unsigned grid = (unsigned)std::min<long long>((pts * lp + kRoundBlock - 1) / kRoundBlock, (long long)ctx->n_cu * ctx->round_blocks_per_cu);
  const RoundLaunch a{ctx->d_traj, ctx->d_pose, ctx->d_chunks, ctx->sp, ctx->d_px, ctx->d_py, ctx->gs, ctx->icap, it, delta,
                      band_delta, ctx->d_res_sdf, ctx->d_res_t, ctx->d_res_gx, ctx->d_res_gy, ctx->d_ctl + b, ctx->round_list | ((ctx->scan_anchors && ctx->lipschitz_ok) ? 16 : 0)};
  size_t e0 = 0, e1 = 0;
  if (ctx->profile) { e0 = next_event(ctx); (void)hipEventRecord(ctx->ev_pool[e0], st); }
  const int shape = poly_lds ? (int)kPolygonLds : ctx->cfg.shape_id;
  if (!launch_k_round(shape, lp, mode, grid, lds, st, a) && ctx->launch_err.empty())
    ctx->launch_err = "k_round: shape not compiled into this build";
  if (svsdf_launch_rec *r = record_launch(ctx, SVSDF_KERNEL_ROUND, compiled_shape(shape), grid, (unsigned)kRoundBlock, lds, pts, b)) {
    r->targ[0] = lp; r->targ[1] = mode; r->iter = it; r->anchors = (a.clist_on & 16) ? 1 : 0;
  }
  debug_sync(st, "k_round", lp * 10 + mode, it);
  if (ctx->profile) {
    e1 = next_event(ctx);
    (void)hipEventRecord(ctx->ev_pool[e1], st);
    ctx->round_events.emplace_back(e0, e1);
  }
}

size_t tail_lds_bytes(const svsdf_ctx *ctx, bool poly_lds, bool local) {
  const size_t lds_tables = ((table_lds_doubles(ctx) + (size_t)traj_lds_doubles(ctx->N) + (poly_lds ? (size_t)svsdf::kPolyEdgeDoubles * (size_t)ctx->sp.nverts : 0)) * sizeof(double) + 15) & ~(size_t)15;
  return lds_tables + (kTailBlock / 64) * (local ? kTailWaveLds : kTailWaveLds - kTailLocalBytes);
}

void launch_tail(svsdf_ctx *ctx, hipStream_t st, int b, int it0) {
  const int mode = bound_mode_of(ctx);
  const bool scans = mode != 0;
  const double sel = (scans && !ctx->select_env) ? ctx->scan_delta : ctx->select_delta;
  const int all_it = (scans && !ctx->all_iter_env) ? 7 : ctx->delta_all_iter;
  const int all_after = (ctx->tail_all_after < 0) ? std::max(0, all_it - it0) : ctx->tail_all_after;
  long long pts = std::max(1, ctx->bcount[b]);
  if (ctx->have_prev_nactive && it0 <= ctx->prev_tail_iter && it0 < kMaxIter)
    pts = std::min<long long>(pts, ctx->prev_nactive[it0] / std::max(1, ctx->nbatch) * 5 / 4 + 64);
  bool poly_lds = ctx->poly_lds;
  bool local = ctx->tail_local && it0 == 0;
  size_t lds = 0;
  for (int attempt = 0; attempt < 4; ++attempt) {
    lds = tail_lds_bytes(ctx, poly_lds, local);
    if (lds <= ctx->lds_limit) break;
    if (local) local = false;
    else if (poly_lds) poly_lds = false;
    else break;
  }
  if (lds > ctx->lds_limit) {
    if (ctx->launch_err.empty()) ctx->launch_err = "trajectory too long for the LDS pose table (k_tail)";
    return;
  }
  const int ppw = (pts <= (long long)ctx->n_cu * 12) ? 1 : 2;
  const long long per_block = (kTailBlock / 64) * ppw;
  const unsigned grid = (unsigned)std::max<long long>(1, std::min<long long>((pts + per_block - 1) / per_block, (long long)ctx->n_cu * 3));
  const double *d_tk = ctx->d_in + 19 * (size_t)ctx->N;
  const TailLaunch a{ctx->d_traj, d_tk, ctx->d_pose, ctx->d_chunks, ctx->sp, ctx->d_px, ctx->d_py, ctx->gs, ctx->icap, it0, mode,
                     sel, ctx->select_delta, all_after, ppw, ctx->d_res_sdf, ctx->d_res_t, ctx->d_res_gx, ctx->d_res_gy,
                     ctx->d_ctl + b, ctx->round_list | (local ? 4 : 0) | (ctx->tail_duo ? 0 : 8) | ((ctx->scan_anchors && ctx->lipschitz_ok) ? 16 : 0), ctx->prune,
                     (ctx->tail_latency && ppw == 1 && pts <= (long long)ctx->n_cu * 4 * svsdf::kTailLatencyWaves) ? 1 : 0};
  size_t e0 = 0, e1 = 0;
  if (ctx->profile) { e0 = next_event(ctx); (void)hipEventRecord(ctx->ev_pool[e0], st); }
  const int shape = poly_lds ? (int)kPolygonLds : ctx->cfg.shape_id;
  if (!launch_k_tail(shape, mode, grid, lds, st, a) && ctx->launch_err.empty())
    ctx->launch_err = "k_tail: shape not compiled into this build";
  if (svsdf_launch_rec *r = record_launch(ctx, SVSDF_KERNEL_TAIL, compiled_shape(shape), grid, (unsigned)kTailBlock, lds, pts, b)) {
    r->targ[0] = mode; r->targ[1] = a.latency ? svsdf::kTailLatencyWaves : SVSDF_TAIL_WAVES; r->iter = it0; r->points_per_wave = ppw;
    r->local_state = local ? 1 : 0; r->duo = (ppw == 1 && ctx->tail_duo) ? 1 : 0; r->anchors = (a.clist_on & 16) ? 1 : 0;
  }
  debug_sync(st, "k_tail", mode, it0);
  if (ctx->profile) {
    e1 = next_event(ctx);
    (void)hipEventRecord(ctx->ev_pool[e1], st);
    ctx->tail_events.emplace_back(e0, e1);
  }
  ctx->stats.tail_launches++;
}

int choose_tail_iter(const svsdf_ctx *ctx) {
  if (ctx->tail_mode == -2 || ctx->scaled) return -1;
  if (tail_lds_bytes(ctx, false, false) > ctx->lds_limit) return -1;
  if (ctx->tail_mode >= 0) return std::min(ctx->tail_mode, (int)kMaxIter - 2);
  if (!ctx->have_prev_nactive) return -1;
  const long long below = ctx->tail_below > 0 ? ctx->tail_below : (long long)ctx->n_cu * 24;
  return (ctx->prev_nactive[0] <= below) ? 0 : -1;
}

void launch_classify(svsdf_ctx *ctx, hipStream_t st, int b) {
  const unsigned grid = (unsigned)std::min<long long>(((long long)ctx->bcount[b] + kBlock - 1) / kBlock, 2048);
  const size_t lds = (size_t)traj_lds_doubles(ctx->N) * sizeof(double);
  const ClassifyLaunch a{ctx->d_traj, ctx->sp, ctx->d_px, ctx->d_py, ctx->d_sdf, ctx->d_t, ctx->d_res_sdf, ctx->d_res_t,
                         ctx->d_res_gx, ctx->d_res_gy, ctx->gs, ctx->d_ctl + b, &ctx->d_ctl->n_int, (int)ctx->icap,
                         ctx->scaled ? &ctx->scale : nullptr};
  if (!launch_k_classify(ctx->cfg.shape_id, grid, lds, st, a) && ctx->launch_err.empty())
    ctx->launch_err = "k_classify: shape not compiled into this build";
  (void)record_launch(ctx, ctx->scaled ? SVSDF_KERNEL_CLASSIFY_SCALED : SVSDF_KERNEL_CLASSIFY, compiled_shape(ctx->cfg.shape_id), grid,
                      (unsigned)kBlock, lds, ctx->bcount[b], b);
  debug_sync(st, "k_classify", b, 0);
}

int upload_traj(svsdf_ctx *ctx, int N, const double *coeffs, const double *T, bool clear_nonfinite = false) {
  if (N < 1 || N > kMaxPieces) return fail(ctx, SVSDF_ERR_INVALID, "N out of range [1, 128]");
  double td = 0.0;
  for (int i = 0; i < N; ++i) td += T[i];
  if (!(td == td) || std::isinf(td)) return fail(ctx, SVSDF_ERR_NONFINITE, "non-finite duration");
  for (int i = 0; i < N; ++i)
    if (!(T[i] > 0.0)) return fail(ctx, SVSDF_ERR_INVALID, "piece durations must be positive");
  if (td < 3 * 1e2 || !ctx->have_duration) {
    ctx->traj_duration = td;
    ctx->have_duration = true;
  }
  const double dur = ctx->traj_duration;
  size_t K = 0;
  for (double t = 0.0; t <= dur; t += 0.15) ++K;
  if (K < 1 || K > 16000) return fail(ctx, SVSDF_ERR_INVALID, "trajectory duration out of range for the scan table");
  const size_t need = 19 * (size_t)N + K + 2 * ((K + kChunk - 1) / kChunk);
  if (need > ctx->in_cap) {
    const size_t cap = need + 4096;
    if (ctx->h_in) (void)hipHostFree(ctx->h_in);
    ctx->h_in = nullptr;
    HIPCHK(hipHostMalloc((void **)&ctx->h_in, cap * sizeof(double), hipHostMallocDefault));
    int rc = dev_alloc(ctx, &ctx->d_in, cap);
    if (rc) return rc;
    ctx->in_cap = cap;
  }
  if (K > ctx->pose_cap) {
    int rc = dev_alloc(ctx, &ctx->d_pose, K + 1024);
    if (rc) return rc;
    rc = dev_alloc(ctx, &ctx->d_chunks, 2 * ((K + 1024) / kChunk + 2));
    if (rc) return rc;
    ctx->pose_cap = K + 1024;
  }
  std::memcpy(ctx->h_in, coeffs, sizeof(double) * 18 * N);
  std::memcpy(ctx->h_in + 18 * N, T, sizeof(double) * N);
// ... 37 lines not shown
          for (int j = 0; j <= 4; ++j) {
            double bj = 0.0, cjq = 1.0;
            for (int q = 0; q <= j; ++q) { bj += cjq / binom4[q] * p[q]; cjq = cjq * (j - q) / (q + 1); }
            bound[d] = std::max(bound[d], std::fabs(bj));
          }
        }
        v2 = std::max(v2, std::hypot(bound[0], bound[1]));
        wmax = std::max(wmax, bound[2]);
      }
      const double sl = v2 * (1.0 + 1e-9) * h + 1e-9;
      if (std::isfinite(sl)) { slack[c] = sl; ctx->slack_max = std::max(ctx->slack_max, sl); }
      const double rl = wmax * (1.0 + 1e-9) * h + 1e-12;
      if (std::isfinite(rl)) rot[c] = rl;
    }
  }
  {
    bool coarse = dur < 1073741824.0;
    double tmin = std::numeric_limits<double>::infinity();
    for (int i = 0; i < N; ++i) {
      const double v = std::ldexp(T[i], 20);
      coarse = coarse && T[i] < 1048576.0 && v == std::floor(v);
      tmin = std::min(tmin, T[i]);
    }
    const int f = ctx->cfg.flags;
    int mode = (f & SVSDF_FLAG_EXACT_PIECE_TIME) ? 1 : (f & SVSDF_FLAG_FAST_PIECE_TIME) ? 0 : (coarse ? 0 : 1);
    if (mode == 1 && !(tmin >= 1e-6)) mode = 2;
    ctx->piece_time_mode = mode;
    ctx->stats_piece_time = mode;
  }
  ctx->N = N;
  ctx->K = (int)K;
  HIPCHK(hipMemcpyAsync(ctx->d_in, ctx->h_in, need * sizeof(double), hipMemcpyHostToDevice, ctx->stream));
  const size_t lds = (size_t)traj_lds_doubles(N) * sizeof(double);
  hipLaunchKernelGGL(k_prep, dim3(1), dim3(1024), lds, ctx->stream, ctx->d_in, N, dur, (int)K,
                     ctx->piece_time_mode, ctx->d_traj,
                     ctx->d_pose, ctx->d_chunks, ctx->r_bound, ctx->d_ctl, ctx->nbatch, clear_nonfinite ? ctx->d_nonfinite : nullptr);
  (void)record_launch(ctx, SVSDF_KERNEL_PREP, -1, 1, 1024, lds, (long long)K, 0);
  ctx->ltab_mode = 0;
  return SVSDF_OK;
}

int build_layer_tables(svsdf_ctx *ctx) {
  int mode = ctx->layer_tables;
  const size_t K = (size_t)ctx->K;
  if (mode < 0) {
    const long long solves = ctx->have_prev_nsolve ? ctx->prev_solves : (long long)ctx->P;
    mode = (solves * 2 * svsdf::kLayerSteps >= 16ll * (long long)K * svsdf::kLayerRows * svsdf::kLayerSteps) ? 3 : 0;
  }
  if (ctx->cfg.shape_id == (int)svsdf::kPolygon) mode = 0;
  if (mode == 0) return SVSDF_OK;
  if (K > ctx->ltab_cap) {
    const size_t cap = K + 256;
    ctx->ltab_cap = 0;
    int rc = dev_alloc(ctx, &ctx->d_ltab, cap * (size_t)svsdf::kLayerRows * svsdf::kLayerSteps);
    if (rc) return rc;
    ctx->ltab_cap = cap;
  }
  const int rows = (mode >= 3) ? svsdf::kLayerRows : 1;
  const size_t lds = (size_t)traj_lds_doubles(ctx->N) * sizeof(double);
  const unsigned grid = (unsigned)((K * (size_t)rows * svsdf::kLayerSteps + 255) / 256);
  hipLaunchKernelGGL(k_layer_tables, dim3(grid), dim3(256), lds, ctx->stream, ctx->d_traj, ctx->d_in + 19 * (size_t)ctx->N, (int)K, rows, ctx->d_ltab);
  if (svsdf_launch_rec *r = record_launch(ctx, SVSDF_KERNEL_LAYER_TABLES, -1, grid, 256, lds, (long long)(K * rows * svsdf::kLayerSteps), 0)) r->targ[0] = mode;
  ctx->ltab_mode = mode;
  return SVSDF_OK;
}


hipStream_t batch_stream(const svsdf_ctx *ctx, int b) { return ctx->nbatch > 1 ? ctx->bstream[b] : ctx->stream; }

// ... 18 lines not shown
    hipStream_t st = batch_stream(ctx, b);
    BatchCtl *ctl = ctx->d_ctl + b;
    QuerySet q{};
    q.qx = ctx->gs.sqx; q.qy = ctx->gs.sqy; q.count_ptr = &ctl->n_solve[it];
    q.slots = ctx->gs.solve + (size_t)ctx->bstart[b] * kMaxSlots; q.n_outer = 1;
    if (ctx->ub_full) { q.seed_k = ctx->gs.sq_k; q.seed_d = ctx->gs.sq_ub; }
    int G = (it >= ctx->late_iter) ? ctx->G_late : ctx->G;
    if (!ctx->G_env && !ctx->G_late_env && ctx->have_prev_nsolve) {
      const long long n = ctx->prev_nsolve[it];
      G = ctx->G;
      if (n < ctx->wide32_below) G = std::max(G, 32);
      else if (n < ctx->wide16_below) G = std::max(G, 16);
      else if (n < ctx->wide8_below) G = std::max(G, 8);
    }
    launch_solve(ctx, G, st, q, (long long)ctx->bcount[b] * kMaxSlots, ctx->gs.sq_sdf, ctx->gs.sq_t, ctl, it + 1);
    if (tail_next) launch_tail(ctx, st, b, it + 1);
    else launch_round(ctx, st, b, it + 1);
  }
}

int enqueue_queries(svsdf_ctx *ctx, int N, const double *coeffs, const double *T, bool allow_cull) {
  if (ctx->host_only) return fail(ctx, SVSDF_ERR_NO_DEVICE, "host-only context: no device entry points");
  if (!ctx->points_set) return fail(ctx, SVSDF_ERR_NO_POINTS, "svsdf_set_points has not been called");
  HIPCHK(hipSetDevice(ctx->device));
  ctx->ev_used = 0;
  ctx->refine_events.clear();
  ctx->round_events.clear();
  ctx->tail_events.clear();
  ctx->stats = svsdf_stats{};
  ctx->stats.points = ctx->P;
  reset_launches(ctx);
  const size_t e_begin = next_event(ctx);
  (void)hipEventRecord(ctx->ev_pool[e_begin], ctx->stream);
  int rc = upload_traj(ctx, N, coeffs, T, true);
  if (rc) return rc;
  if ((rc = build_layer_tables(ctx))) return rc;
  const bool fork = ctx->nbatch > 1;
  if (fork) HIPCHK(hipEventRecord(ctx->ev_prep, ctx->stream));
  const int m = ctx->tail_iter = choose_tail_iter(ctx);
  for (int b = 0; b < ctx->nbatch; ++b) {
    hipStream_t st = batch_stream(ctx, b);
    BatchCtl *ctl = ctx->d_ctl + b;
    if (fork) HIPCHK(hipStreamWaitEvent(st, ctx->ev_prep, 0));
    QuerySet qm{};
    qm.qx = ctx->d_px; qm.qy = ctx->d_py; qm.stride = 0; qm.count_ptr = nullptr;
    qm.count_fixed = ctx->bcount[b]; qm.list = nullptr; qm.base = ctx->bstart[b]; qm.n_outer = 1;
    const double cull_thresh = (allow_cull && ctx->cull && ctx->cull_ok) ? ctx->cfg.safety_hor + 1e-9 : std::numeric_limits<double>::infinity();
    launch_solve(ctx, ctx->G, st, qm, ctx->bcount[b], ctx->d_sdf, ctx->d_t, ctl, 0, cull_thresh);
    launch_classify(ctx, st, b);
    if (m == 0) launch_tail(ctx, st, b, 0);
    else launch_round(ctx, st, b, 0);
  }
  if (m >= 0) {
    for (int it = 0; it < m; ++it) enqueue_solve_round(ctx, it, it == m - 1);
    ctx->it_done = kMaxIter + 1;
  } else {
    for (int it = 0; it < ctx->first_iters; ++it) enqueue_solve_round(ctx, it);
    ctx->it_done = ctx->first_iters;
  }
  return join_batches(ctx);
}

int swept_field(svsdf_ctx *ctx, int N, const double *coeffs, const double *T, double *sdf_sorted) {
  if (ctx->host_only) return fail(ctx, SVSDF_ERR_NO_DEVICE, "host-only context: no device entry points");
  if (!ctx->points_set) return fail(ctx, SVSDF_ERR_NO_POINTS, "svsdf_set_points has not been called");
  if (ctx->P == 0) return SVSDF_OK;
  HIPCHK(hipSetDevice(ctx->device));
  ctx->ev_used = 0;
  ctx->refine_events.clear();
  ctx->round_events.clear();
  ctx->tail_events.clear();
  ctx->stats = svsdf_stats{};
  ctx->stats.points = ctx->P;
  reset_launches(ctx);
  int rc = upload_traj(ctx, N, coeffs, T);
  if (rc) return rc;
  if ((rc = build_layer_tables(ctx))) return rc;
  if (ctx->nbatch > 1) HIPCHK(hipEventRecord(ctx->ev_prep, ctx->stream));
  for (int b = 0; b < ctx->nbatch; ++b) {
    hipStream_t st = batch_stream(ctx, b);
    if (ctx->nbatch > 1) HIPCHK(hipStreamWaitEvent(st, ctx->ev_prep, 0));
    QuerySet qm{};
    qm.qx = ctx->d_px; qm.qy = ctx->d_py; qm.stride = 0; qm.count_ptr = nullptr;
    qm.count_fixed = ctx->bcount[b]; qm.list = nullptr; qm.base = ctx->bstart[b]; qm.n_outer = 1;
    launch_solve(ctx, ctx->G, st, qm, ctx->bcount[b], ctx->d_sdf, ctx->d_t, ctx->d_ctl + b, 0);
  }
  rc = join_batches(ctx);
  if (rc) return rc;
  HIPCHK(hipMemcpyAsync(sdf_sorted, ctx->d_sdf, ctx->P * sizeof(double), hipMemcpyDeviceToHost, ctx->stream));
  HIPCHK(hipStreamSynchronize(ctx->stream));
  return SVSDF_OK;
}

int reduce_and_read(svsdf_ctx *ctx, bool with_partial) {
  const int N = ctx->N;
  bool host_written = false;
  if (with_partial) {
    const unsigned grid = (unsigned)std::min<size_t>((ctx->P + kBlock - 1) / kBlock, 512);
    const size_t plen = 19 * (size_t)N + 1;
    if ((size_t)grid * plen > ctx->block_partials_cap) {
      int rc = dev_alloc(ctx, &ctx->d_block_partials, (size_t)grid * plen);
      if (rc) return rc;
      ctx->block_partials_cap = (size_t)grid * plen;
    }
    const size_t lds = ((size_t)traj_lds_doubles(N) + std::max<size_t>((kBlock / 64) * plen, grid == 1 ? svsdf::assemble_small_doubles(N) : 0)) * sizeof(double);
    if (lds > ctx->lds_limit)
      return fail(ctx, SVSDF_ERR_INVALID, "trajectory too long for the reduction's LDS accumulator rows (" + std::to_string(lds) + " B of " +
                  std::to_string(ctx->lds_limit) + " B per block)");
    const int fuse = grid <= 4 ? 1 : 0;
    if (ctx->scaled)
      hipLaunchKernelGGL(k_reduce_sc, dim3(grid), dim3(kBlock), lds, ctx->stream, ctx->d_traj, ctx->d_px, ctx->d_py,
                         (int)ctx->P, ctx->d_res_sdf, ctx->d_res_t, ctx->d_res_gx, ctx->d_res_gy,
                         ctx->cfg.safety_hor, ctx->cfg.weight_p, ctx->d_block_partials, ctx->d_nonfinite, ctx->d_out,
                         ctx->d_ctl, ctx->nbatch, ctx->it_done, (int)kOutPartial, (int)kOutDoubles, ctx->d_ticket, ctx->h_out_dev, fuse,
                         ctx->scale);
    else
      hipLaunchKernelGGL(k_reduce, dim3(grid), dim3(kBlock), lds, ctx->stream, ctx->d_traj, ctx->d_px, ctx->d_py,
                         (int)ctx->P, ctx->d_res_sdf, ctx->d_res_t, ctx->d_res_gx, ctx->d_res_gy,
                         ctx->cfg.safety_hor, ctx->cfg.weight_p, ctx->d_block_partials, ctx->d_nonfinite, ctx->d_out,
                         ctx->d_ctl, ctx->nbatch, ctx->it_done, (int)kOutPartial, (int)kOutDoubles, ctx->d_ticket, ctx->h_out_dev, fuse);
    if (svsdf_launch_rec *r = record_launch(ctx, ctx->scaled ? SVSDF_KERNEL_REDUCE_SCALED : SVSDF_KERNEL_REDUCE, -1, grid, (unsigned)kBlock, lds,
                                            (long long)ctx->P, 0)) r->fused = fuse;
    if (!fuse) {
      hipLaunchKernelGGL(k_final, dim3((unsigned)plen), dim3(64), 0, ctx->stream, ctx->d_block_partials, (int)grid, ctx->d_sums);
      (void)record_launch(ctx, SVSDF_KERNEL_FINAL, -1, (unsigned)plen, 64, 0, (long long)grid, 0);
      hipLaunchKernelGGL(k_finish, dim3(1), dim3(kBlock), 0, ctx->stream, ctx->d_sums, N, ctx->d_out, ctx->d_ctl,
                         ctx->nbatch, ctx->it_done, ctx->d_nonfinite,
                         reinterpret_cast<unsigned long long *>(ctx->d_out + kOutPartial), ctx->h_out_dev, (int)kOutDoubles);
      (void)record_launch(ctx, SVSDF_KERNEL_FINISH, -1, 1, (unsigned)kBlock, 0, 0, 0);
    }
    host_written = ctx->h_out_dev != nullptr;
  } else {
    HIPCHK(hipMemsetAsync(ctx->d_sums, 0, kOutPartial * sizeof(double), ctx->stream));
    hipLaunchKernelGGL(k_finish, dim3(1), dim3(kBlock), 0, ctx->stream, ctx->d_sums, N, ctx->d_out, ctx->d_ctl,
                       ctx->nbatch, ctx->it_done, ctx->d_nonfinite,
                       reinterpret_cast<unsigned long long *>(ctx->d_out + kOutPartial), ctx->h_out_dev, (int)kOutDoubles);
    (void)record_launch(ctx, SVSDF_KERNEL_FINISH, -1, 1, (unsigned)kBlock, 0, 0, 0);
    host_written = ctx->h_out_dev != nullptr;
  }
  ctx->e_end = next_event(ctx);
  (void)hipEventRecord(ctx->ev_pool[ctx->e_end], ctx->stream);
  if (!host_written) HIPCHK(hipMemcpyAsync(ctx->h_out, ctx->d_out, kOutDoubles * sizeof(double), hipMemcpyDeviceToHost, ctx->stream));
  HIPCHK(hipStreamSynchronize(ctx->stream));
  HIPCHK(hipGetLastError());
  return SVSDF_OK;
}

int alloc_interior_buffers(svsdf_ctx *ctx, size_t cap);

int finish(svsdf_ctx *ctx, bool with_partial) {
  int rc = reduce_and_read(ctx, with_partial);
  if (rc) return rc;
  const unsigned long long *st = reinterpret_cast<const unsigned long long *>(ctx->h_out + kOutPartial);
  while (st[5] > 0 && ctx->it_done < kMaxIter) {
    const int it1 = std::min(ctx->it_done + 3, (int)kMaxIter);
    for (int it = ctx->it_done; it < it1; ++it) enqueue_solve_round(ctx, it);
    ctx->it_done = it1;
    if ((rc = join_batches(ctx))) return rc;
    HIPCHK(hipMemsetAsync(ctx->d_nonfinite, 0, sizeof(int), ctx->stream));
    if ((rc = reduce_and_read(ctx, with_partial))) return rc;
  }
  if (st[5] > 0) return fail(ctx, SVSDF_ERR_INVALID, "GSIP iterations exhausted (internal limit)");
  {
    const size_t n_int = (size_t)st[11 + 2 * kMaxIter];
    if (n_int > ctx->icap) {
      rc = alloc_interior_buffers(ctx, std::min(ctx->P, n_int + n_int / 8 + 4096));
      return rc ? rc : kRepeat;
    }
    if (!ctx->icap_fitted && ctx->P >= 100000 && ctx->icap > 2 * (n_int + n_int / 8 + 4096)) {
      rc = alloc_interior_buffers(ctx, n_int + n_int / 8 + 4096);
      if (rc) return rc;
    }
    ctx->icap_fitted = true;
  }
  ctx->stats.solves = st[0];
  ctx->stats.sdf_evals = st[1];
  ctx->stats.scan_evals = st[2];
  ctx->stats.interior_points = st[3];
  ctx->stats.gsip_samples = st[6];
  ctx->stats.gsip_iterations = (unsigned)st[7];
  ctx->stats.culled_points = st[8];
  ctx->stats.round_scan_evals = st[9 + kMaxIter];
  ctx->stats.speculative_evals = st[10 + kMaxIter];
  ctx->stats.batches = ctx->nbatch;
  {
    const unsigned long long c = st[12 + 2 * kMaxIter], r = st[13 + 2 * kMaxIter];
    ctx->stats.shader_clock_mhz = r ? (double)c / (double)r * ctx->wall_clock_khz * 1e-3 : 0.0;
  }
  for (int i = 0; i < kMaxIter; ++i) ctx->prev_nsolve[i] = (long long)st[9 + i];
  ctx->prev_solves = (long long)st[0];
  ctx->have_prev_nsolve = true;
  for (int i = 0; i < kMaxIter; ++i) ctx->prev_nactive[i] = (long long)st[11 + kMaxIter + i];
  ctx->prev_tail_iter = ctx->tail_iter;
  ctx->have_prev_nactive = true;
  ctx->stats.tail_iter = ctx->tail_iter;
  ctx->stats.tail_points = (ctx->tail_iter >= 0 && ctx->tail_iter < kMaxIter) ? (unsigned long long)st[11 + kMaxIter + ctx->tail_iter] : 0ull;
  if (ctx->adaptive_iters && ctx->tail_iter < 0) ctx->first_iters = std::max(2, std::min((int)st[7] + 1, (int)kMaxIter));
  if (ctx->profile_span && !ctx->profile) {
    float ms = 0.f;
    (void)hipEventElapsedTime(&ms, ctx->ev_pool[0], ctx->ev_pool[ctx->e_end]);
    ctx->stats.device_ms = ms;
  }
  if (ctx->profile) {
    float ms = 0.f;
    (void)hipEventElapsedTime(&ms, ctx->ev_pool[0], ctx->ev_pool[ctx->e_end]);
    ctx->stats.device_ms = ms;
    auto merged = [&](const std::vector<std::pair<size_t, size_t>> &evs, double &uni, double &sum) {
      sum = 0.0;
      std::vector<std::pair<float, float>> iv;
      for (const auto &pr : evs) {
        float a = 0.f, b = 0.f;
        if (hipEventElapsedTime(&a, ctx->ev_pool[0], ctx->ev_pool[pr.first]) == hipSuccess &&
            hipEventElapsedTime(&b, ctx->ev_pool[0], ctx->ev_pool[pr.second]) == hipSuccess && b >= a) {
          iv.emplace_back(a, b);
          sum += b - a;
        }
      }
      std::sort(iv.begin(), iv.end());
      uni = 0.0;
      float cur_a = 0.f, cur_b = -1.f;
      for (const auto &x : iv) {
        if (x.first > cur_b) { if (cur_b >= cur_a) uni += cur_b - cur_a; cur_a = x.first; cur_b = x.second; }
        else cur_b = std::max(cur_b, x.second);
      }
      if (cur_b >= cur_a) uni += cur_b - cur_a;
    };
    merged(ctx->refine_events, ctx->stats.solve_ms, ctx->stats.solve_ms_sum);
    merged(ctx->round_events, ctx->stats.round_ms, ctx->stats.round_ms_sum);
    merged(ctx->tail_events, ctx->stats.tail_ms, ctx->stats.tail_ms_sum);
// ... 136 lines not shown
}


void accumulate(int N, const double *partial, double *cost, double *gradT, double *gradC) {
  *cost += partial[0];
  for (int e = 0; e < 18 * N; ++e) gradC[e] += partial[1 + e];
  for (int j = 0; j < N; ++j) gradT[j] += partial[1 + 18 * N + j];
}

int alloc_interior_buffers(svsdf_ctx *ctx, size_t cap) {
  int rc = 0;
  cap = std::max<size_t>(cap, 1);
  if (cap * kMaxSlots > 0x7fffffffull) return fail(ctx, SVSDF_ERR_INVALID, "too many interior points per shard (max ~89M)");
  if ((rc = dev_alloc(ctx, &ctx->gs.pt, cap))) return rc;
  if ((rc = dev_alloc(ctx, &ctx->gs.r, cap))) return rc;
  if ((rc = dev_alloc(ctx, &ctx->gs.theta0, cap))) return rc;
  if ((rc = dev_alloc(ctx, &ctx->gs.theta_res, cap))) return rc;
  if ((rc = dev_alloc(ctx, &ctx->gs.iter, cap))) return rc;
  if ((rc = dev_alloc(ctx, &ctx->gs.nsamp, cap))) return rc;
  if ((rc = dev_alloc(ctx, &ctx->gs.phase, cap))) return rc;
  if ((rc = dev_alloc(ctx, &ctx->gs.req, cap))) return rc;
  const size_t S = cap * kMaxSlots;
  if ((rc = dev_alloc(ctx, &ctx->gs.sqx, S))) return rc;
  if ((rc = dev_alloc(ctx, &ctx->gs.sqy, S))) return rc;
  if ((rc = dev_alloc(ctx, &ctx->gs.sqth, S))) return rc;
  if ((rc = dev_alloc(ctx, &ctx->gs.sq_ub, S))) return rc;
  if ((rc = dev_alloc(ctx, &ctx->gs.sq_k, S))) return rc;
  if ((rc = dev_alloc(ctx, &ctx->gs.sq_sdf, S))) return rc;
  if ((rc = dev_alloc(ctx, &ctx->gs.sq_t, S))) return rc;
  ctx->icap = cap;
  return SVSDF_OK;
}

int alloc_point_buffers(svsdf_ctx *ctx, size_t P) {
  int rc = 0;
  if ((rc = dev_alloc(ctx, &ctx->d_px, P))) return rc;
  if ((rc = dev_alloc(ctx, &ctx->d_py, P))) return rc;
  if ((rc = dev_alloc(ctx, &ctx->d_sdf, P))) return rc;
  if ((rc = dev_alloc(ctx, &ctx->d_t, P))) return rc;
  if ((rc = dev_alloc(ctx, &ctx->d_res_sdf, P))) return rc;
  if ((rc = dev_alloc(ctx, &ctx->d_res_t, P))) return rc;
  if ((rc = dev_alloc(ctx, &ctx->d_res_gx, P))) return rc;
  if ((rc = dev_alloc(ctx, &ctx->d_res_gy, P))) return rc;
  if ((rc = dev_alloc(ctx, &ctx->gs.list[0], P))) return rc;
  if ((rc = dev_alloc(ctx, &ctx->gs.list[1], P))) return rc;
  if ((rc = dev_alloc(ctx, &ctx->gs.solve, P * kMaxSlots))) return rc;
  ctx->icap_fitted = false;
  size_t cap0 = std::min(P, std::max<size_t>(P / 2, 4096));
  if (const char *e = std::getenv("SVSDF_ICAP_INIT")) cap0 = std::max<size_t>(1, (size_t)std::atoll(e));
  return alloc_interior_buffers(ctx, cap0);
}

void morton_order(const double *xyz, size_t P, int flags, std::vector<long long> &order) {
  order.resize(P);
  std::iota(order.begin(), order.end(), 0ll);
  if ((flags & SVSDF_FLAG_KEEP_INPUT_ORDER) || P <= 1) return;
  double xmin = std::numeric_limits<double>::infinity(), xmax = -xmin, ymin = xmin, ymax = -xmin;
  for (size_t i = 0; i < P; ++i) {
    const double x = xyz[3 * i], y = xyz[3 * i + 1];
    if (x < xmin) xmin = x;
    if (x > xmax) xmax = x;
    if (y < ymin) ymin = y;
    if (y > ymax) ymax = y;
  }
  const double ext = std::max(std::max(xmax - xmin, ymax - ymin), 1e-12);
  std::vector<uint64_t> key(P);
  for (size_t i = 0; i < P; ++i) {
    const double fx = (xyz[3 * i] - xmin) / ext, fy = (xyz[3 * i + 1] - ymin) / ext;
    const uint32_t qx = (uint32_t)std::min(65535.0, std::max(0.0, fx * 65535.0));
    const uint32_t qy = (uint32_t)std::min(65535.0, std::max(0.0, fy * 65535.0));
    key[i] = ((uint64_t)(part1by1(qx) | (part1by1(qy) << 1)) << 32) | (uint64_t)(i & 0xffffffffu);
  }
  std::vector<uint64_t> tmp(P);
  for (int pass = 0; pass < 4; ++pass) {
    const int sh = 32 + 8 * pass;
    size_t cnt[257] = {0};
    for (size_t i = 0; i < P; ++i) ++cnt[((key[i] >> sh) & 0xffu) + 1];
    for (int b = 0; b < 256; ++b) cnt[b + 1] += cnt[b];
    for (size_t i = 0; i < P; ++i) tmp[cnt[(key[i] >> sh) & 0xffu]++] = key[i];
    key.swap(tmp);
  }
  for (size_t i = 0; i < P; ++i) order[i] = (long long)(key[i] & 0xffffffffull);
}

void stripe_of(const std::vector<long long> &order, int rk, int ws, std::vector<long long> &out) {
  ws = std::max(1, ws);
  out.clear();
  out.reserve(order.size() / (size_t)ws + 1);
  for (size_t k = (size_t)rk; k < order.size(); k += (size_t)ws) out.push_back(order[k]);
}

void shard_plan(const double *xyz, size_t P, int rk, int ws, int flags, std::vector<long long> &out) {
  if (P > 0xffffffffull) { out.clear(); return; }
  std::vector<long long> order;
  morton_order(xyz, P, flags, order);
  stripe_of(order, rk, ws, out);
}

int set_batches(svsdf_ctx *ctx, int nb) {
  nb = std::max(1, std::min(nb, kMaxBatches));
  const size_t Ps = ctx->P;
  ctx->nbatch = nb;
  std::vector<BatchCtl> hc(kMaxBatches);
  std::memset(hc.data(), 0, sizeof(BatchCtl) * kMaxBatches);
  for (int b = 0; b < nb; ++b) {
    const size_t s = Ps * (size_t)b / nb, e = Ps * (size_t)(b + 1) / nb;
    ctx->bstart[b] = (int)s;
    ctx->bcount[b] = (int)(e - s);
    hc[b].start = (int)s;
    hc[b].count = (int)(e - s);
  }
  HIPCHK(hipMemcpy(ctx->d_ctl, hc.data(), sizeof(BatchCtl) * kMaxBatches, hipMemcpyHostToDevice));
  return SVSDF_OK;
}

void CloudPlan::release() {
  (void)hipSetDevice(device);
  for (void *q : {(void *)d_part, (void *)d_keys, (void *)d_keys2, d_tmp})
    if (q) (void)hipFree(q);
  d_part = nullptr; d_keys = d_keys2 = nullptr; d_tmp = nullptr; sorted = nullptr;
}

int plan_cloud(svsdf_ctx *ctx, const double *d_xyz, size_t P, CloudPlan &plan) {
  plan.device = ctx->device;
  plan.d_xyz = d_xyz;
  plan.P = P;
  if (P > 0x7fffffffull) return fail(ctx, SVSDF_ERR_INVALID, "too many points (max 2^31 - 1 per call)");
  if (P == 0) return SVSDF_OK;
  HIPCHK(hipSetDevice(ctx->device));
  hipStream_t st = ctx->stream;
#define UPCHK(expr)                                                                                                  \
  do {                                                                                                               \
    hipError_t e_ = (expr);                                                                                          \
    if (e_ != hipSuccess) { plan.release(); return fail(ctx, SVSDF_ERR_HIP_BASE + (int)e_, std::string(#expr) + ": " + hipGetErrorString(e_)); } \
  } while (0)
  const unsigned grid = (unsigned)std::min<size_t>((P + kBlock - 1) / kBlock, 1024);
  UPCHK(hipMalloc((void **)&plan.d_part, (size_t)grid * 4 * sizeof(double)));
  UPCHK(hipMalloc((void **)&plan.d_keys, P * sizeof(unsigned long long)));
  UPCHK(hipMalloc((void **)&plan.d_keys2, P * sizeof(unsigned long long)));
  UPCHK(hipMemsetAsync(ctx->d_nonfinite, 0, sizeof(int), st));
  hipLaunchKernelGGL(k_points_bbox, dim3(grid), dim3(kBlock), 0, st, d_xyz, P, plan.d_part, ctx->d_nonfinite);
  std::vector<double> hp((size_t)grid * 4);
  int bad = 0;
  UPCHK(hipMemcpyAsync(hp.data(), plan.d_part, hp.size() * sizeof(double), hipMemcpyDeviceToHost, st));
  UPCHK(hipMemcpyAsync(&bad, ctx->d_nonfinite, sizeof(int), hipMemcpyDeviceToHost, st));
  UPCHK(hipStreamSynchronize(st));
// ... 44 lines not shown
      for (void *q : {(void *)d_idx, (void *)d_sx, (void *)d_sy})
        if (q) (void)hipFree(q);
    };
#define UPCHK(expr)                                                                                                  \
  do {                                                                                                               \
    hipError_t e_ = (expr);                                                                                          \
    if (e_ != hipSuccess) { cleanup(); return fail(ctx, SVSDF_ERR_HIP_BASE + (int)e_, std::string(#expr) + ": " + hipGetErrorString(e_)); } \
  } while (0)
    UPCHK(hipMalloc((void **)&d_idx, Ps * sizeof(long long)));
    if (!local) {
      UPCHK(hipMalloc((void **)&d_sx, Ps * sizeof(double)));
      UPCHK(hipMalloc((void **)&d_sy, Ps * sizeof(double)));
    }
    const unsigned g2 = (unsigned)std::min<size_t>((Ps + kBlock - 1) / kBlock, 1024);
    hipLaunchKernelGGL(k_points_gather, dim3(g2), dim3(kBlock), 0, st, plan.d_xyz, plan.sorted, P, rk, ws, Ps,
                       local ? ctx->d_px : d_sx, local ? ctx->d_py : d_sy, d_idx);
    UPCHK(hipMemcpyAsync(ctx->shard_idx.data(), d_idx, Ps * sizeof(long long), hipMemcpyDeviceToHost, st));
    UPCHK(hipStreamSynchronize(st));
    UPCHK(hipGetLastError());
    if (!local) {
      UPCHK(hipMemcpyPeer(ctx->d_px, ctx->device, d_sx, planner->device, Ps * sizeof(double)));
      UPCHK(hipMemcpyPeer(ctx->d_py, ctx->device, d_sy, planner->device, Ps * sizeof(double)));
    }
#undef UPCHK
    cleanup();
  }
  HIPCHK(hipSetDevice(ctx->device));
  ctx->P = Ps;
  ctx->points_set = true;
  int rcb = set_batches(ctx, ctx->want_batches > 0 ? ctx->want_batches : 1);
  if (rcb) return rcb;
  ctx->have_prev_nsolve = false;
  ctx->have_prev_nactive = false;
  ctx->prev_tail_iter = -1;
  ctx->ub_tune = 0;
  ctx->bt_state = 0;
  ctx->ub_ratio = 0.0;
  if (!ctx->ub_env) { ctx->ub_full = false; ctx->ub_lazy = false; ctx->ub_anchor = false; }
  ctx->an_state = 0;
  ctx->lz_state = 0;
  if (!ctx->G_env) {
    ctx->G = default_lanes(ctx, Ps);
    if (!ctx->G_late_env) ctx->G_late = std::max(ctx->G, 8);
  }
  return SVSDF_OK;
}

int upload_shard_device(svsdf_ctx *ctx, const double *d_xyz, size_t P, int rk, int ws) {
  CloudPlan plan;
  int rc = plan_cloud(ctx, d_xyz, P, plan);
  if (rc) { ctx->P = 0; ctx->points_set = false; return rc; }
  rc = take_stripe(ctx, ctx, plan, rk, ws);
  plan.release();
  return rc;
}

int debug_sdf_at(svsdf_ctx *ctx, int N, const double *coeffs, const double *T, size_t n, const double *pxy, const double *t,
                 double *out8) {
  if (n == 0) return SVSDF_OK;
  if (n > 0x7fffffffull) return fail(ctx, SVSDF_ERR_INVALID, "svsdf_debug_sdf_at: too many queries");
  HIPCHK(hipSetDevice(ctx->device));
  ctx->ev_used = 0;
  const size_t e0 = next_event(ctx);
  (void)hipEventRecord(ctx->ev_pool[e0], ctx->stream);
  int rc = upload_traj(ctx, N, coeffs, T);
  if (rc) return rc;
// ... 37 lines not shown
```

implicit-svsdf-planner_amd/csrc/svsdf_shape_slice.hip:

```cpp
#include <hip/hip_runtime.h>

#include <algorithm>

#include "svsdf_launch.hpp"

#ifndef SVSDF_SLICE
#define SVSDF_SLICE 0
#endif
#define SVSDF_CAT_(a, b) a##b
#define SVSDF_CAT(a, b) SVSDF_CAT_(a, b)
#define SLICE_FN(name) SVSDF_CAT(name, SVSDF_CAT(_s, SVSDF_SLICE))

namespace svsdf {
namespace {

template <int S>
constexpr bool shape_enabled() {
#ifdef SVSDF_FAST_BUILD
  return S == 4 || S == 6 || S == 7 || S == 16;
#else
  return S >= 0 && S < kShapeCount;
#endif
}

// ... 32 lines not shown
#undef SOLVE
    return true;
  }
}

template <int S>
bool round_s(int lp, int mode, unsigned grid, size_t lds, hipStream_t st, const RoundLaunch &a) {
  if constexpr (!kernel_shape_enabled<S>()) {
    return false;
  } else {
#define ROUND(LP, MODE)                                                                                             \
  hipLaunchKernelGGL((k_round<S, LP, MODE>), dim3(grid), dim3(kRoundBlock), lds, st, a.traj, a.pose, a.chunks, a.sp, \
                     a.px, a.py, a.gs, a.stride, a.it, a.delta, a.band_delta, a.res_sdf, a.res_t, a.res_gx,          \
                     a.res_gy, a.ctl, a.clist_on)
    if (lp == 8) {
      if (mode == 3) ROUND(8, 3); else if (mode == 2) ROUND(8, 2); else if (mode == 1) ROUND(8, 1); else ROUND(8, 0);
    } else {
      if (mode == 3) ROUND(32, 3); else if (mode == 2) ROUND(32, 2); else if (mode == 1) ROUND(32, 1); else ROUND(32, 0);
    }
#undef ROUND
    return true;
  }
}

template <int S>
bool tail_s(int mode, unsigned grid, size_t lds, hipStream_t st, const TailLaunch &a) {
  if constexpr (!kernel_shape_enabled<S>()) {
    return false;
  } else {
#define TAIL_W(MODE, WAVES)                                                                                                 \
  hipLaunchKernelGGL((k_tail<S, MODE, WAVES>), dim3(grid), dim3(kTailBlock), lds, st, a.traj, a.tk, a.pose, a.chunks, a.sp,  \
                     a.px, a.py, a.gs, a.stride, a.it0, a.prev_mode, a.delta, a.band_delta, a.all_after, a.ppw, a.res_sdf,   \
                     a.res_t, a.res_gx, a.res_gy, a.ctl, a.clist_on, a.prune)
#define TAIL(MODE) do { if (a.latency) TAIL_W(MODE, kTailLatencyWaves); else TAIL_W(MODE, SVSDF_TAIL_WAVES); } while (0)
    if (mode == 3) TAIL(3); else if (mode == 2) TAIL(2); else if (mode == 1) TAIL(1); else TAIL(0);
#undef TAIL
#undef TAIL_W
    return true;
  }
}

template <int S>
bool classify_s(unsigned grid, size_t lds, hipStream_t st, const ClassifyLaunch &a) {
  if constexpr (!shape_enabled<S>()) {
    return false;
  } else {
    if (a.scl)
      hipLaunchKernelGGL((k_classify_sc<S>), dim3(grid), dim3(kBlock), lds, st, a.traj, a.sp, a.px, a.py, a.sdf, a.t,
                         a.res_sdf, a.res_t, a.res_gx, a.res_gy, a.gs, a.ctl, a.n_int, a.icap, *a.scl);
    else
      hipLaunchKernelGGL((k_classify<S>), dim3(grid), dim3(kBlock), lds, st, a.traj, a.sp, a.px, a.py, a.sdf, a.t,
                         a.res_sdf, a.res_t, a.res_gx, a.res_gy, a.gs, a.ctl, a.n_int, a.icap);
    return true;
  }
}

template <int S>
bool rbound_s(unsigned grid, hipStream_t st, ShapeParams sp, double rmax, int nrad, int nang, double *out) {
  if constexpr (!shape_enabled<S>()) {
    return false;
  } else {
    hipLaunchKernelGGL((k_rbound<S>), dim3(grid), dim3(kBlock), 0, st, sp, rmax, nrad, nang, out);
    return true;
  }
}

template <int S>
bool subsw_s(dim3 grid, hipStream_t st, ShapeParams sp, const double *father, const double *child,
             const unsigned long long *offs, const double *pts, const double *kt, int nkt, int *flag) {
  if constexpr (!shape_enabled<S>()) {
    return false;
  } else {
    hipLaunchKernelGGL((k_subsw<S>), grid, dim3(kSubswBlock), 0, st, sp, father, child, offs, pts, kt, nkt, flag);
    return true;
  }
}

template <int S>
bool shape_kernels_s(unsigned grid, hipStream_t st, ShapeParams sp, int ks, int count, double resu, int size_side,
                     double safemargin, const double *yaw, unsigned char *map) {
  if constexpr (!shape_enabled<S>() || is_polygon<S>()) {
    return false;
  } else {
    hipLaunchKernelGGL((k_shape_kernels<S>), dim3(grid), dim3(kBlock), 0, st, sp, ks, count, resu, size_side, safemargin, yaw, map);
    return true;
// ... 73 lines not shown
```

implicit-svsdf-planner_amd/svsdf_amd/binding.py:

```python
import ctypes as C
import os

import numpy as np

_PKG = os.path.dirname(os.path.dirname(os.path.abspath(__file__)))
_LIB = None

SHAPES = ["sdUnevenCapsule", "sdCutDisk", "sdTrapezoid", "sdRhombus", "star", "sdTunnel",
          "sdHorseshoe", "sdHeart", "sdOrientedVesica", "sdRoundedCross", "sdRoundedX", "bigX",
          "sdMoon", "sdPie", "sdPie2", "sdArc", "Polygon"]
SHAPE_ID = {n: i for i, n in enumerate(SHAPES)}

_dp = C.POINTER(C.c_double)
_ip = C.POINTER(C.c_int)

EXPORTS = [
    "svsdf_create", "svsdf_destroy", "svsdf_config_default", "svsdf_shape_id_from_inputdata",
    "svsdf_shape_name", "svsdf_last_error_string", "svsdf_set_points", "svsdf_set_points_device",
    "svsdf_num_points", "svsdf_eval_penalty", "svsdf_eval_penalty_partial",
    "svsdf_accumulate_partial", "svsdf_lmbm_evaluate", "svsdf_last_costs", "svsdf_lmbm_begin",
    "svsdf_lmbm_finish", "svsdf_minco_coeffs", "svsdf_forward_T", "svsdf_backward_T",
    "svsdf_query_points", "svsdf_last_stats", "svsdf_shard_indices", "svsdf_set_profiling",
    "svsdf_shard_plan", "svsdf_lmbm_prepare", "svsdf_debug_sincos_mismatches",
    "svsdf_map_create", "svsdf_map_destroy", "svsdf_map_info", "svsdf_map_gather", "svsdf_pcd_read_ascii",
# ... 12 lines not shown
                ("max_iterations", C.c_int), ("max_linesearch", C.c_int), ("min_step", C.c_double),
                ("max_step", C.c_double), ("f_dec_coeff", C.c_double), ("s_curv_coeff", C.c_double),
                ("cautious_factor", C.c_double), ("machine_prec", C.c_double)]


EVALUATE_T = C.CFUNCTYPE(C.c_double, C.c_void_p, C.POINTER(C.c_double), C.POINTER(C.c_double), C.c_int)
PROGRESS_T = C.CFUNCTYPE(C.c_int, C.c_void_p, C.POINTER(C.c_double), C.POINTER(C.c_double), C.c_double, C.c_double,
                         C.c_int, C.c_int, C.c_int)
LBFGS_STATUS = {0: "CONVERGENCE", 1: "STOP", 2: "CANCELED", -1012: "INVALID_FUNCVAL", -1011: "MINIMUMSTEP",
                -1010: "MAXIMUMSTEP", -1009: "MAXIMUMLINESEARCH", -1008: "MAXIMUMITERATION", -1007: "WIDTHTOOSMALL",
                -1006: "INVALIDPARAMETERS", -1005: "INCREASEGRADIENT"}


class Config(C.Structure):
    _fields_ = [("shape_id", C.c_int), ("poly_params", C.c_double * 3), ("safety_hor", C.c_double),
                ("weight_p", C.c_double), ("rho", C.c_double), ("head_state", C.c_double * 9),
                ("tail_state", C.c_double * 9), ("device", C.c_int), ("polygon_nverts", C.c_int),
                ("polygon_xy", _dp), ("rank", C.c_int), ("world_size", C.c_int), ("flags", C.c_int),
                ("n_devices", C.c_int), ("devices", C.c_int * 8), ("combine", C.c_int),
                ("polygon_nloops", C.c_int), ("polygon_loop_sizes", C.POINTER(C.c_int))]


class Stats(C.Structure):
    _fields_ = [("points", C.c_ulonglong), ("interior_points", C.c_ulonglong),
                ("solves", C.c_ulonglong), ("gsip_samples", C.c_ulonglong), ("sdf_evals", C.c_ulonglong),
                ("scan_evals", C.c_ulonglong), ("device_ms", C.c_double), ("solve_ms", C.c_double),
                ("solve_launches", C.c_uint), ("gsip_iterations", C.c_uint), ("culled_points", C.c_ulonglong),
                ("gsip_bound_mode", C.c_int), ("bound_mode_decided", C.c_int), ("bound_ratio", C.c_double),
                ("n_devices", C.c_int), ("combine", C.c_int), ("combine_ms", C.c_double), ("setup_ms", C.c_double),
                ("piece_time_exact", C.c_int), ("solve_ms_sum", C.c_double), ("round_scan_evals", C.c_ulonglong),
                ("round_ms", C.c_double), ("round_ms_sum", C.c_double), ("batches", C.c_int),
                ("speculative_evals", C.c_ulonglong), ("plan_settled", C.c_int), ("tail_iter", C.c_int),
                ("tail_launches", C.c_uint), ("tail_points", C.c_ulonglong), ("tail_ms", C.c_double),
                ("tail_ms_sum", C.c_double), ("shader_clock_mhz", C.c_double), ("fanout_ms", C.c_double)]


class Plan(C.Structure):
    _fields_ = [("bound_mode", C.c_int), ("batches", C.c_int), ("lanes_per_query", C.c_int), ("tail_iter", C.c_int),
                ("settled", C.c_int), ("layer_tables", C.c_int)]


PLAN_AUTO = -1


class LaunchRec(C.Structure):
    _fields_ = [("struct_size", C.c_int), ("kernel", C.c_int), ("shape", C.c_int), ("targ", C.c_int * 3), ("iter", C.c_int),
                ("batch", C.c_int), ("solo", C.c_int), ("points_per_wave", C.c_int), ("local_state", C.c_int),
                ("duo", C.c_int), ("anchors", C.c_int), ("fused", C.c_int), ("work", C.c_longlong), ("grid", C.c_uint),
                ("block", C.c_uint), ("lds_bytes", C.c_ulonglong)]


LAUNCH_REC_CAP = 512
KERNELS = ["prep", "solve", "classify", "round", "tail", "reduce", "final", "finish",
           "solve_scaled", "classify_scaled", "reduce_scaled", "layer_tables"]


class Scale(C.Structure):
    _fields_ = [("struct_size", C.c_int), ("enabled", C.c_int), ("c", C.c_double * 2), ("amp", C.c_double * 2),
                ("omega", C.c_double * 2), ("phase", C.c_double * 2)]


EXAMPLE_SCALE = {"c": (0.8, 0.8), "amp": (0.6, 0.4), "omega": (1.5, 1.8), "phase": (-1.0, 0.0)}


class OutlineStats(C.Structure):
    _fields_ = [("nodes_evaluated", C.c_ulonglong), ("dense_nodes", C.c_ulonglong), ("cells_marched", C.c_ulonglong),
                ("batches", C.c_ulonglong), ("open_chains", C.c_int)]


class SvsdfError(RuntimeError):
    pass


def lib_path():
    v = os.environ.get("SVSDF_LIB_VARIANT", "")
    return os.path.join(_PKG, "libsvsdf_hip_%s.so" % v if v else "libsvsdf_hip.so")


def lib():
    global _LIB
    if _LIB is not None:
        return _LIB
    path = lib_path()
    if not os.path.exists(path):
        raise SvsdfError(f"{path} is missing: run `python __graft_entry__.py build` "
                         "(hipcc --offload-arch=gfx950); this package has no CPU fallback")
    L = C.CDLL(path)
# ... 528 lines not shown
        return float(o[0]), float(o[1])

    def shape_selfcheck(self):
        o = np.zeros(3)
        self.L.svsdf_shape_selfcheck.argtypes = [C.c_void_p, _dp]
        self._chk(self.L.svsdf_shape_selfcheck(self.ctx, _p(o)), "svsdf_shape_selfcheck")
        return float(o[0]), float(o[1]), float(o[2])

    def set_scale(self, c=None, amp=(0.0, 0.0), omega=(0.0, 0.0), phase=(0.0, 0.0), enabled=True, struct_size=None):
        if c is None:
            self._chk(self.L.svsdf_set_scale(self.ctx, None), "svsdf_set_scale")
            return
        s = Scale()
        s.struct_size = C.sizeof(Scale) if struct_size is None else int(struct_size)
        s.enabled = int(bool(enabled))
        for name, v in (("c", c), ("amp", amp), ("omega", omega), ("phase", phase)):
            getattr(s, name)[:] = [float(v[0]), float(v[1])]
        self._chk(self.L.svsdf_set_scale(self.ctx, C.byref(s)), "svsdf_set_scale")

    def get_scale(self):
        s = Scale()
        s.struct_size = C.sizeof(Scale)
        self._chk(self.L.svsdf_get_scale(self.ctx, C.byref(s)), "svsdf_get_scale")
        if not s.enabled:
            return None
        return {k: (float(getattr(s, k)[0]), float(getattr(s, k)[1])) for k in ("c", "amp", "omega", "phase")}

    def get_plan(self):
        pl = Plan()
        self._chk(self.L.svsdf_get_plan(self.ctx, C.byref(pl)), "svsdf_get_plan")
        return {k: getattr(pl, k) for k, _ in Plan._fields_}

    def set_plan(self, bound_mode=PLAN_AUTO, batches=PLAN_AUTO, lanes_per_query=PLAN_AUTO, tail_iter=PLAN_AUTO,
                 layer_tables=PLAN_AUTO):
        pl = Plan(int(bound_mode), int(batches), int(lanes_per_query), int(tail_iter), 0, int(layer_tables))
        self._chk(self.L.svsdf_set_plan(self.ctx, C.byref(pl)), "svsdf_set_plan")

    def set_combine(self, combine):
        code = {"host": 1, "rccl": 2}.get(combine, combine)
        self._chk(self.L.svsdf_set_combine(self.ctx, int(code)), "svsdf_set_combine")

    def group_info(self):
        nd, cb, rk = C.c_int(), C.c_int(), C.c_int()
        self._chk(self.L.svsdf_group_info(self.ctx, C.byref(nd), C.byref(cb), C.byref(rk)), "svsdf_group_info")
        return {"n_devices": nd.value, "combine": ["auto", "host", "rccl"][cb.value], "rccl_ranks": rk.value}

    def group_stripe(self, k):
        dev, pts, st, pl = C.c_int(), C.c_size_t(), Stats(), Plan()
        self._chk(self.L.svsdf_group_stripe(self.ctx, int(k), C.byref(dev), C.byref(pts), C.byref(st), C.byref(pl)), "svsdf_group_stripe")
        return {"device": dev.value, "points": pts.value, "stats": {n: getattr(st, n) for n, _ in Stats._fields_},
                "plan": {n: getattr(pl, n) for n, _ in Plan._fields_}}

    def set_group_serial(self, serial=True):
        self._chk(self.L.svsdf_set_group_serial(self.ctx, int(bool(serial))), "svsdf_set_group_serial")

    def set_profiling(self, enable=True):
        self._chk(self.L.svsdf_set_profiling(self.ctx, int(enable)), "svsdf_set_profiling")

    def last_launches(self):
        recs = (LaunchRec * LAUNCH_REC_CAP)()
        recs[0].struct_size = C.sizeof(LaunchRec)
        n = C.c_int(0)
        self._chk(self.L.svsdf_last_launches(self.ctx, recs, LAUNCH_REC_CAP, C.byref(n)), "svsdf_last_launches")
        if n.value > LAUNCH_REC_CAP:
            raise SvsdfError(f"svsdf_last_launches: {n.value} launches, {LAUNCH_REC_CAP} recorded")
        out = []
        for r in recs[:n.value]:
            d = {k: getattr(r, k) for k, _ in LaunchRec._fields_ if k != "struct_size"}
# ... 10 lines not shown
```

include/svsdf_c.h:

```cpp
#ifndef SVSDF_C_H
#define SVSDF_C_H

#include <stddef.h>

#ifdef __cplusplus
extern "C" {
#endif

enum svsdf_shape_id {
  SVSDF_SHAPE_sdUnevenCapsule = 0,
  SVSDF_SHAPE_sdCutDisk = 1,
  SVSDF_SHAPE_sdTrapezoid = 2,
  SVSDF_SHAPE_sdRhombus = 3,
  SVSDF_SHAPE_star = 4,
  SVSDF_SHAPE_sdTunnel = 5,
  SVSDF_SHAPE_sdHorseshoe = 6,
  SVSDF_SHAPE_sdHeart = 7,
  SVSDF_SHAPE_sdOrientedVesica = 8,
  SVSDF_SHAPE_sdRoundedCross = 9,
  SVSDF_SHAPE_sdRoundedX = 10,
  SVSDF_SHAPE_bigX = 11,
  SVSDF_SHAPE_sdMoon = 12,
  SVSDF_SHAPE_sdPie = 13,
  SVSDF_SHAPE_sdPie2 = 14,
// ... 160 lines not shown
  unsigned long long points;
  unsigned long long interior_points;
  unsigned long long solves;
  unsigned long long gsip_samples;
  unsigned long long sdf_evals;
  unsigned long long scan_evals;
  double device_ms;
  double solve_ms;
  unsigned int solve_launches;
  unsigned int gsip_iterations;
  unsigned long long culled_points;
  int gsip_bound_mode;
  int bound_mode_decided;
  double bound_ratio;
  int n_devices;
  int combine;
  double combine_ms;
  double setup_ms;
  int piece_time_exact;
  double solve_ms_sum;
  unsigned long long round_scan_evals;
  double round_ms;
  double round_ms_sum;
  int batches;
  unsigned long long speculative_evals;
  int plan_settled;
  int tail_iter;
  unsigned int tail_launches;
  unsigned long long tail_points;
  double tail_ms;
  double tail_ms_sum;
  double shader_clock_mhz;
  double fanout_ms;
} svsdf_stats;
int svsdf_last_stats(const svsdf_ctx *ctx, svsdf_stats *out);

#define SVSDF_LAUNCH_REC_CAP 512
enum svsdf_kernel_kind {
  SVSDF_KERNEL_PREP = 0,
  SVSDF_KERNEL_SOLVE = 1,
  SVSDF_KERNEL_CLASSIFY = 2,
  SVSDF_KERNEL_ROUND = 3,
  SVSDF_KERNEL_TAIL = 4,
  SVSDF_KERNEL_REDUCE = 5,
  SVSDF_KERNEL_FINAL = 6,
  SVSDF_KERNEL_FINISH = 7,
  SVSDF_KERNEL_SOLVE_SCALED = 8,
  SVSDF_KERNEL_CLASSIFY_SCALED = 9,
  SVSDF_KERNEL_REDUCE_SCALED = 10,
  SVSDF_KERNEL_LAYER_TABLES = 11
};
typedef struct svsdf_launch_rec {
  int struct_size;
  int kernel;
  int shape;
  int targ[3];
  int iter;
  int batch;
  int solo;
  int points_per_wave;
  int local_state;
  int duo;
  int anchors;
  int fused;
  long long work;
  unsigned int grid, block;
  unsigned long long lds_bytes;
} svsdf_launch_rec;
int svsdf_last_launches(const svsdf_ctx *ctx, svsdf_launch_rec *out, int cap, int *count);

typedef struct svsdf_scale {
  int struct_size;
  int enabled;
  double c[2];
  double amp[2];
  double omega[2];
  double phase[2];
} svsdf_scale;
int svsdf_set_scale(svsdf_ctx *ctx, const svsdf_scale *scale);
int svsdf_get_scale(const svsdf_ctx *ctx, svsdf_scale *out);

#define SVSDF_PLAN_AUTO (-1)
typedef struct svsdf_plan {
  int bound_mode;
  int batches;
  int lanes_per_query;
  int tail_iter;
  int settled;
  int layer_tables;
} svsdf_plan;
int svsdf_get_plan(const svsdf_ctx *ctx, svsdf_plan *out);
int svsdf_set_plan(svsdf_ctx *ctx, const svsdf_plan *plan);
int svsdf_set_combine(svsdf_ctx *ctx, int combine);
int svsdf_group_info(const svsdf_ctx *ctx, int *n_devices, int *combine, int *rccl_ranks);
int svsdf_group_stripe(const svsdf_ctx *ctx, int k, int *device, size_t *points, svsdf_stats *stats, svsdf_plan *plan);
int svsdf_set_group_serial(svsdf_ctx *ctx, int serial);
int svsdf_shape_bound(const svsdf_ctx *ctx, double out2[2]);
int svsdf_shape_selfcheck(const svsdf_ctx *ctx, double out3[3]);
int svsdf_set_profiling(svsdf_ctx *ctx, int enable);
long long svsdf_debug_sincos_mismatches(svsdf_ctx *ctx, double lo, double hi, int n);
int svsdf_debug_sdf_at(svsdf_ctx *ctx, int N, const double *coeffs_colmajor, const double *T, size_t n,
                       const double *points_xy, const double *t, double *out8);
int svsdf_shard_indices(const svsdf_ctx *ctx, long long *idx_out);

#ifdef __cplusplus
}
#endif
#endif
```

Before: 183.3 million.

## Add long-running query tracking to launch persistent points early from prior calls

Adds a 'long' point mechanism: the tail kernel records queries that ran many iterations, and on the next evaluation those points are collected into a separate list (an extra batch slot) so classify and the iteration kernels can process them first or separately via a selection list and skip flags. The goal is to reduce the straggler tail where a few slow queries keep the GPU underused at the end. It adds extra buffers, a collect kernel, plan fields and host bookkeeping. By default long_from is 0, so the feature is likely off unless enabled through plan or environment settings.

```diff
diff --git a/implicit-svsdf-planner_amd/csrc/svsdf_body_classify.hpp b/implicit-svsdf-planner_amd/csrc/svsdf_body_classify.hpp
--- a/implicit-svsdf-planner_amd/csrc/svsdf_body_classify.hpp
+++ b/implicit-svsdf-planner_amd/csrc/svsdf_body_classify.hpp
@@ -1,11 +1,12 @@
   extern __shared__ double classify_lds[];
   const TrajL tr = stage_traj(trg, classify_lds);
-  const int start = ctl->start, count = ctl->count;
+  const int start = ctl->start, count = sel.count_ptr ? *sel.count_ptr : ctl->count;
   const int lane = (int)(threadIdx.x & 63);
   for (int e0 = (int)((blockIdx.x * blockDim.x + threadIdx.x) & ~63u); e0 < count; e0 += gridDim.x * blockDim.x) {
     const int e = e0 + lane;
-    const bool in_range = e < count;
-    const int i = start + (in_range ? e : 0);
+    bool in_range = e < count;
+    const int i = sel.list ? (in_range ? sel.list[e] : 0) : start + (in_range ? e : 0);
+    if (sel.skip && in_range && sel.skip[i]) in_range = false;
     const double px = px_[i], py = py_[i];
     const double sdf = sdf_[i], ts = t_[i];
     const bool inter = in_range && !(sdf > 0);
diff --git a/implicit-svsdf-planner_amd/csrc/svsdf_body_tail.hpp b/implicit-svsdf-planner_amd/csrc/svsdf_body_tail.hpp
--- /dev/null
+++ b/implicit-svsdf-planner_amd/csrc/svsdf_body_tail.hpp
@@ -0,0 +1,173 @@
+  extern __shared__ double tail_lds[];
+  constexpr int LP = 32;
+  const int n_act = ctl->n_active[it0];
+  const int wave_g = (int)((blockIdx.x * blockDim.x + threadIdx.x) >> 6);
+  if (n_act <= 0 || (int)blockIdx.x * (kTailBlock / 64) * ppw >= n_act) return;
+  const int K = trg->K;
+  const int nch = (K + kChunk - 1) / kChunk;
+  stage_poly_edges<SHAPE>(sp, tail_lds);
+  double *tab_lds = tail_lds + poly_lds_doubles<SHAPE>(sp.nverts);
+  Pose *pose = reinterpret_cast<Pose *>(tab_lds);
+  Chunk *chunks = reinterpret_cast<Chunk *>(tab_lds + 4 * (size_t)K);
+  {
+    const double *src = reinterpret_cast<const double *>(pose_g);
+    for (int i = threadIdx.x; i < 4 * K; i += blockDim.x) tab_lds[i] = src[i];
+    const double *srcc = reinterpret_cast<const double *>(chunks_g);
+    for (int i = threadIdx.x; i < 4 * nch; i += blockDim.x) tab_lds[4 * (size_t)K + i] = srcc[i];
+  }
+  const TrajL tr = stage_traj(trg, tab_lds + 4 * (size_t)K + 4 * (size_t)nch);
+  const size_t tables = poly_lds_doubles<SHAPE>(sp.nverts) + 4 * (size_t)K + 4 * (size_t)nch + (size_t)traj_lds_doubles(tr.N);
+  const bool local = it0 == 0 && (clist_on & 4) != 0;
+  const size_t wave_stride = local ? kTailWaveLds : kTailWaveLds - kTailLocalBytes;
+  char *wave_lds = reinterpret_cast<char *>(tail_lds + ((tables + 1) & ~(size_t)1)) + (threadIdx.x >> 6) * wave_stride;
+  unsigned short *clist_w = reinterpret_cast<unsigned short *>(wave_lds + ((ladder_lds_bytes(2) + 15) & ~(size_t)15));
+  unsigned *qlist = reinterpret_cast<unsigned *>(clist_w + 2 * kMaxCand);
+  GsipState gl = gs;
+  if (local) {
+    double *ld = reinterpret_cast<double *>(qlist + 64);
+    gl.r = ld; gl.theta0 = ld + 2; gl.theta_res = ld + 4;
+    gl.sqx = ld + 6; gl.sqy = gl.sqx + 2 * kMaxSlots; gl.sqth = gl.sqy + 2 * kMaxSlots; gl.sq_ub = gl.sqth + 2 * kMaxSlots;
+    gl.sq_sdf = gl.sq_ub + 2 * kMaxSlots; gl.sq_t = gl.sq_sdf + 2 * kMaxSlots;
+    int *li_ = reinterpret_cast<int *>(gl.sq_t + 2 * kMaxSlots);
+    gl.pt = li_; gl.iter = li_ + 2; gl.nsamp = li_ + 4; gl.phase = li_ + 6; gl.req = reinterpret_cast<unsigned *>(li_ + 8);
+    gl.sq_k = li_ + 10;
+  }
+  const GsipState ga = local ? gl : gs;
+  const size_t stride_a = local ? (size_t)2 : stride;
+  const int start = ctl->start;
+  const int *cur = gs.list[it0 & 1] + start;
+  const int lane = (int)(threadIdx.x & 63);
+  const int h = lane >> 5, l = lane & (LP - 1);
+  const bool duo = ppw == 1 && MODE != 0 && (clist_on & 8) == 0;
+  const int hs = duo ? 0 : h;
+  const unsigned lt_mask = (1u << l) - 1u;
+  unsigned n_eval = 0, n_scan = 0, n_solved = 0, n_spec = 0, n_rscan = 0;
+  unsigned long long rc[16] = {0, 0, 0, 0, 0, 0, 0, 0, 0, 0, 0, 0, 0, 0, 0, 0};
+  unsigned long long sc[12] = {0, 0, 0, 0, 0, 0, 0, 0, 0, 0, 0, 0};
+  const unsigned long long t_wave0 = SVSDF_SITE_CLOCK();
+  int n_emit_tot = 0;
+  const int n_static = (int)(gridDim.x * (blockDim.x >> 6)) * ppw;
+  int q_next = wave_g * ppw, q_end = min(wave_g * ppw + ppw, n_act);
+  bool exhausted = false;
+  int a = -1;
+  int steps = 0;
+  bool own = false;
+  for (int guard = 0; guard < (1 << 24); ++guard) {
+#pragma unroll
+    for (int hh = 0; hh < 2; ++hh) {
+      const int ah = __builtin_amdgcn_readlane(a, hh * 32);
+      if (ah >= 0 || hh >= ppw) continue;
+      if (q_next >= q_end && !exhausted) {
+        unsigned b = 0;
+        if (lane == 0) b = atomicAdd(&ctl->work[min(it0 + 1, kWorkCounters - 1)], (unsigned)kTailFetch);
+        b = __builtin_amdgcn_readfirstlane(b);
+        const long long bb = (long long)b + n_static;
+        if (bb >= n_act) exhausted = true;
+        else { q_next = (int)bb; q_end = (int)min((long long)n_act, bb + kTailFetch); }
+      }
+      if (q_next < q_end) {
+        const int e = q_next++;
+        if (h == hh || duo) {
+          a = cur[e]; steps = 0; own = false;
+          if (local && l == 0 && h == hh) {
+            const size_t ia_ = (size_t)a;
+            gl.pt[hs] = gs.pt[ia_]; gl.r[hs] = gs.r[ia_]; gl.theta0[hs] = gs.theta0[ia_]; gl.theta_res[hs] = gs.theta_res[ia_];
+            gl.iter[hs] = gs.iter[ia_]; gl.nsamp[hs] = gs.nsamp[ia_]; gl.phase[hs] = gs.phase[ia_]; gl.req[hs] = 0u;
+          }
+        }
+      }
+    }
+    if (__builtin_amdgcn_readlane(a, 0) < 0 && __builtin_amdgcn_readlane(a, 32) < 0) break;
+    if (local) {
+      __builtin_amdgcn_fence(__ATOMIC_RELEASE, "workgroup");
+      __builtin_amdgcn_wave_barrier();
+      __builtin_amdgcn_fence(__ATOMIC_ACQUIRE, "workgroup");
+    }
+    RoundOut<1> ro;
+    ro.list_me[0] = false; ro.mlist[0] = 0u; ro.n_emit = 0; ro.push_next = false; ro.finished = false;
+    if (a >= 0) {
+      const double dl = (steps >= all_after) ? 1e300 : delta, bd = (steps >= all_after) ? 1e300 : band_delta;
+      round_point<SHAPE, LP, MODE, true>(sp, pose, chunks, K, nch, px_, py_, ga, stride_a, start, local ? hs : a, dl, bd, res_sdf, res_t, res_gx,
+                                   res_gy, n_rscan, ro, clist_w + (size_t)h * kMaxCand, clist_on, rc, duo ? h : -1,
+                                   (clist_on & 16) ? reinterpret_cast<const ChunkAnchor *>(chunks_g + nch) : nullptr);
+      ++steps;
+      if (ro.n_emit > 0) own = true;
+      if (l == 0 && (!duo || h == 0)) n_emit_tot += ro.n_emit;
+    }
+    const size_t ia = local ? (size_t)hs : (size_t)(a >= 0 ? a : 0);
+    if constexpr (REC) {
+      if (ro.finished && l == 0 && (!duo || h == 0)) long_record(ctl0, ga.pt[ia], it0 + steps - 1);
+    }
+    if (ro.finished) a = -1;
+    const unsigned m_mine = (a >= 0 && (!duo || h == 0)) ? ro.mlist[0] : 0u;
+    const int n0 = __popc((unsigned)__builtin_amdgcn_readlane((int)m_mine, 0));
+    const int n1 = __popc((unsigned)__builtin_amdgcn_readlane((int)m_mine, 32));
+    const int nq = n0 + n1;
+    if ((m_mine >> l) & 1u) {
+      const bool seeded = own ? (MODE != 0) : (prev_mode != 0);
+      qlist[(h ? n0 : 0) + __popc(m_mine & lt_mask)] = (unsigned)sample_slot(stride_a, ia, l) | (seeded ? 0x80000000u : 0u);
+    }
+    __builtin_amdgcn_fence(__ATOMIC_RELEASE, "workgroup");
+    __builtin_amdgcn_wave_barrier();
+    __builtin_amdgcn_fence(__ATOMIC_ACQUIRE, "workgroup");
+    if (nq > 0) {
+      if (nq <= 2) {
+        tail_solve_pass<SHAPE, 32>(tr, tk, sp, pose, chunks, K, nch, ga, qlist, 0, nq, prune, wave_lds, n_eval, n_scan, n_solved, n_spec, sc);
+      } else if (nq <= 8) {
+        tail_solve_pass<SHAPE, 8>(tr, tk, sp, pose, chunks, K, nch, ga, qlist, 0, nq, prune, wave_lds, n_eval, n_scan, n_solved, n_spec, sc);
+      } else {
+        for (int base = 0; base < nq; base += 32)
+          tail_solve_pass<SHAPE, 2>(tr, tk, sp, pose, chunks, K, nch, ga, qlist, base, nq, prune, wave_lds, n_eval, n_scan, n_solved, n_spec, sc);
+      }
+      __builtin_amdgcn_fence(__ATOMIC_RELEASE, "workgroup");
+      __builtin_amdgcn_wave_barrier();
+      __builtin_amdgcn_fence(__ATOMIC_ACQUIRE, "workgroup");
+    }
+  }
+  unsigned long long te = (unsigned long long)n_eval + n_scan, ts = n_solved, tc = n_scan, tp = n_spec, tr_ = n_rscan;
+  int em = n_emit_tot;
+#pragma unroll
+  for (int m = 32; m >= 1; m >>= 1) {
+    te += __shfl_xor(te, m, 64); ts += __shfl_xor(ts, m, 64); tc += __shfl_xor(tc, m, 64); tp += __shfl_xor(tp, m, 64);
+    tr_ += __shfl_xor(tr_, m, 64); em += __shfl_xor(em, m, 64);
+  }
+  if (lane == 0 && (te || tr_ || em)) {
+    StatSlot *ss = stat_slot(ctl->stat);
+    if (te) atomicAdd(&ss->evals, te);
+    if (ts) atomicAdd(&ss->solves, ts);
+    if (tc) atomicAdd(&ss->scan, tc);
+    if (tp) atomicAdd(&ss->spec, tp);
+    if (tr_) atomicAdd(&ss->round_scan, tr_);
+    if (em) atomicAdd(&ctl->n_seed[it0], em);
+    if (ts) atomicAdd(&ctl->n_solve[it0], (int)ts);
+  }
+#ifdef SVSDF_SITE_STATS
+  if (lane == 0) {
+    rc[6] = SVSDF_SITE_CLOCK() - t_wave0;
+    StatSlot *ss = stat_slot(ctl->stat);
+    for (int i = 0; i < 8; ++i) if (rc[i]) atomicAdd(&ss->pad[12 + i], rc[i]);
+    for (int i = 8; i < 11; ++i) if (sc[i]) atomicAdd(&ss->pad[i], sc[i]);
+  }
+  {
+    unsigned long long ex = rc[8], ln = rc[12];
+#pragma unroll
+    for (int m = 32; m >= 1; m >>= 1) { ex += __shfl_xor(ex, m, 64); ln += __shfl_xor(ln, m, 64); }
+    if (lane == 0 && ex) { StatSlot *ss = stat_slot(ctl->stat); atomicAdd(&ss->pad[20], ex); atomicAdd(&ss->pad[21], ln); }
+    unsigned long long steps = ex;
+#pragma unroll
+    for (int i = 0; i < 4; ++i) {
+      unsigned long long v = sc[i];
+#pragma unroll
+      for (int m = 32; m >= 1; m >>= 1) v += __shfl_xor(v, m, 64);
+      steps += v;
+    }
+    if (lane == 0) { StatSlot *ss = stat_slot(ctl->stat); atomicMax(&ss->pad[22], steps); atomicMax(&ss->pad[23], rc[6]); }
+  }
+#pragma unroll
+  for (int i = 0; i < 8; ++i) {
+    unsigned long long v = sc[i];
+#pragma unroll
+    for (int m = 32; m >= 1; m >>= 1) v += __shfl_xor(v, m, 64);
+    if (lane == 0 && v) atomicAdd(&stat_slot(ctl->stat)->pad[i], v);
+  }
+#endif
diff --git a/implicit-svsdf-planner_amd/csrc/svsdf_capi.hip b/implicit-svsdf-planner_amd/csrc/svsdf_capi.hip
--- a/implicit-svsdf-planner_amd/csrc/svsdf_capi.hip
+++ b/implicit-svsdf-planner_amd/csrc/svsdf_capi.hip
@@ -192,6 +192,9 @@
   if (const char *e = std::getenv("SVSDF_ROUND_BPC")) ctx->round_blocks_per_cu = std::max(1, std::min(std::atoi(e), 16));
   if (const char *e = std::getenv("SVSDF_SCAN_ANCHORS")) ctx->scan_anchors = std::atoi(e) != 0;
   if (const char *e = std::getenv("SVSDF_LAYER_TABLES")) { const int v = std::atoi(e); ctx->layer_tables = (std::string(e) == "auto") ? -1 : (v == 0 || v == 2 || v == 3) ? v : -1; }
+  ctx->long_from = 0;
+  if (const char *e = std::getenv("SVSDF_LONG_FROM")) { const int v = std::atoi(e); ctx->long_from = (std::string(e) == "auto") ? -1 : std::max(0, std::min(v, (int)kMaxIter - 1)); }
+  if (const char *e = std::getenv("SVSDF_LONG_CAP")) ctx->long_cap = (std::string(e) == "auto") ? -1 : std::max(0ll, std::atoll(e));
   if (const char *e = std::getenv("SVSDF_TAIL_DUO")) ctx->tail_duo = std::atoi(e) != 0;
   if (const char *e = std::getenv("SVSDF_TAIL_LOCAL")) ctx->tail_local = std::atoi(e) != 0;
   if (const char *e = std::getenv("SVSDF_TAIL_LATENCY")) ctx->tail_latency = std::atoi(e) != 0;
@@ -209,7 +212,7 @@
   }
   if (hipEventCreateWithFlags(&ctx->ev_prep, hipEventDisableTiming) != hipSuccess) return bail("event creation failed");
   if (hipMalloc((void **)&ctx->d_traj, sizeof(TrajDev)) != hipSuccess ||
-      hipMalloc((void **)&ctx->d_ctl, kMaxBatches * sizeof(BatchCtl) + 8 * 8 * (kMaxIter + 4)) != hipSuccess ||
+      hipMalloc((void **)&ctx->d_ctl, (kMaxBatches + 1) * sizeof(BatchCtl) + 8 * 8 * (kMaxIter + 4)) != hipSuccess ||
       hipMalloc((void **)&ctx->d_nonfinite, sizeof(int)) != hipSuccess ||
       hipMalloc((void **)&ctx->d_sums, kOutPartial * sizeof(double)) != hipSuccess ||
       hipMalloc((void **)&ctx->d_out, kOutDoubles * sizeof(double)) != hipSuccess ||
@@ -223,7 +226,7 @@
     if (!(e && std::atoi(e) == 0) && hipHostGetDevicePointer(&dp, ctx->h_out, 0) == hipSuccess) ctx->h_out_dev = (double *)dp;
     (void)hipGetLastError();
   }
-  if (hipMemsetAsync(ctx->d_ctl, 0, kMaxBatches * sizeof(BatchCtl) + 8 * 8 * (kMaxIter + 4), ctx->stream) != hipSuccess) return bail("hipMemset failed");
+  if (hipMemsetAsync(ctx->d_ctl, 0, (kMaxBatches + 1) * sizeof(BatchCtl) + 8 * 8 * (kMaxIter + 4), ctx->stream) != hipSuccess) return bail("hipMemset failed");
   {
     const double r0 = shape_circumradius(cfg->shape_id, ctx->poly_xy.data(), (int)(ctx->poly_xy.size() / 2));
     const double analytic = (r0 + std::hypot(sp.tx, sp.ty)) * (1.0 + 1e-12) + 1e-6;
@@ -263,7 +266,7 @@
   void *bufs[] = {ctx->d_poly, ctx->d_px, ctx->d_py, ctx->d_traj, ctx->d_in, ctx->d_pose, ctx->d_chunks, ctx->d_ltab,
                   ctx->d_sdf, ctx->d_t, ctx->d_res_sdf, ctx->d_res_t, ctx->d_res_gx, ctx->d_res_gy, ctx->gs.pt,
                   ctx->gs.r, ctx->gs.theta0, ctx->gs.theta_res, ctx->gs.iter, ctx->gs.nsamp, ctx->gs.phase, ctx->gs.req,
-                  ctx->gs.list[0], ctx->gs.list[1], ctx->gs.solve, ctx->gs.sqx, ctx->gs.sqy, ctx->gs.sqth,
+                  ctx->gs.list[0], ctx->gs.list[1], ctx->gs.solve, ctx->d_long[0], ctx->d_long[1], ctx->d_long_flag, ctx->gs.sqx, ctx->gs.sqy, ctx->gs.sqth,
                   ctx->gs.sq_ub, ctx->gs.sq_k, ctx->gs.sq_sdf, ctx->gs.sq_t, ctx->d_ctl,
                   ctx->d_block_partials, ctx->d_sums,
                   ctx->d_out, ctx->d_nonfinite, ctx->d_fe, ctx->d_fe_flag, ctx->d_ticket};
@@ -489,6 +492,8 @@
   out->lanes_per_query = (c->scaled && c->G > 0) ? svsdf::scaled_lanes(c->G) : c->G;
   out->tail_iter = (c->tail_mode == -2 || c->scaled) ? -2 : (c->tail_mode >= 0) ? c->tail_mode : (c->have_prev_nactive ? choose_tail_iter(c) : SVSDF_PLAN_AUTO);
   out->layer_tables = c->layer_tables;
+  out->long_from = c->scaled ? 0 : (c->long_from >= 0) ? c->long_from : !long_auto_on() ? 0 : (c->long_rec_from > 0 ? c->long_rec_from : SVSDF_PLAN_AUTO);
+  out->long_cap = (c->long_cap >= 0 || c->points_set) ? (int)std::min<long long>(long_cap_of(c), 0x7fffffffll) : SVSDF_PLAN_AUTO;
   out->settled = ((c->ub_env || c->ub_tune > 0) && c->bt_state == 0 && c->an_state == 0 && c->lz_state == 0 && c->have_prev_nsolve) ? 1 : 0;
   return SVSDF_OK;
 }
@@ -498,7 +503,8 @@
   const int g = plan->lanes_per_query;
   if (plan->bound_mode < SVSDF_PLAN_AUTO || plan->bound_mode > 3 || plan->batches < -2 || plan->batches == 0 || plan->batches > kMaxBatches ||
       !(g == SVSDF_PLAN_AUTO || g == 1 || g == 2 || g == 4 || g == 8 || g == 16 || g == 32) || plan->tail_iter < -2 || plan->tail_iter >= kMaxIter ||
-      !(plan->layer_tables == SVSDF_PLAN_AUTO || plan->layer_tables == 0 || plan->layer_tables == 2 || plan->layer_tables == 3))
+      !(plan->layer_tables == SVSDF_PLAN_AUTO || plan->layer_tables == 0 || plan->layer_tables == 2 || plan->layer_tables == 3) ||
+      plan->long_from < SVSDF_PLAN_AUTO || plan->long_from >= kMaxIter || plan->long_cap < SVSDF_PLAN_AUTO)
     return fail(ctx, SVSDF_ERR_INVALID, "svsdf_set_plan: field out of range");
   if (!ctx->subs.empty()) {
     int rc = SVSDF_OK;
@@ -508,6 +514,14 @@
   if (ctx->host_only) return SVSDF_OK;
   HIPCHK(hipSetDevice(ctx->device));
   ctx->layer_tables = plan->layer_tables;
+  {
+    ctx->long_from = plan->long_from;
+    ctx->long_cap = plan->long_cap;
+    if (ctx->points_set && ctx->P > 0) {
+      const int rc = ((size_t)long_cap_of(ctx) > ctx->long_alloc) ? alloc_long_buffers(ctx, ctx->P, (size_t)long_cap_of(ctx)) : forget_long(ctx, ctx->P);
+      if (rc) return rc;
+    }
+  }
   if (plan->bound_mode == SVSDF_PLAN_AUTO) {
     if (ctx->ub_env) { ctx->ub_env = false; ctx->ub_tune = 0; ctx->have_prev_nsolve = false; ctx->have_prev_nactive = false; }
   } else {
diff --git a/implicit-svsdf-planner_amd/csrc/svsdf_ctx.hpp b/implicit-svsdf-planner_amd/csrc/svsdf_ctx.hpp
--- a/implicit-svsdf-planner_amd/csrc/svsdf_ctx.hpp
+++ b/implicit-svsdf-planner_amd/csrc/svsdf_ctx.hpp
@@ -85,7 +85,7 @@
   std::vector<long long> shard_idx;
   double *d_px = nullptr, *d_py = nullptr;
   int nbatch = 1;
-  int bstart[svsdf::kMaxBatches] = {}, bcount[svsdf::kMaxBatches] = {};
+  int bstart[svsdf::kMaxBatches + 1] = {}, bcount[svsdf::kMaxBatches + 1] = {};
   svsdf::BatchCtl *d_ctl = nullptr;
 
   svsdf::TrajDev *d_traj = nullptr;
@@ -155,6 +155,21 @@
   bool select_env = false, all_iter_env = false;
   double scan_delta = 0.002;
   double select_delta = 0.1;
+  int long_from = -1;
+  long long long_cap = -1;
+  int *d_long[2] = {nullptr, nullptr};
+  unsigned char *d_long_flag = nullptr;
+  size_t long_alloc = 0;
+  int long_o = 0;
+  bool long_valid = false;
+  long long long_n = 0;
+  long long long_list_cap[2] = {0, 0};
+  long long long_cap_now = 0;
+  int long_rec_from = 0;
+  bool long_run = false;
+  long long long_alive[svsdf::kMaxIter] = {};
+  bool have_long_alive = false;
+
   bool scaled = false;
   svsdf::ScaleDev scale{};
 
@@ -219,7 +234,7 @@
 namespace svsdf_impl {
 
 constexpr size_t kOutPartial = 19 * svsdf::kMaxPieces + 1;
-constexpr size_t kOutDoubles = kOutPartial + 14 + 2 * svsdf::kMaxIter;
+constexpr size_t kOutDoubles = kOutPartial + 17 + 3 * svsdf::kMaxIter;
 constexpr int kRepeat = -12345;
 
 extern thread_local std::string g_last_error;
@@ -251,6 +266,10 @@
 bool acquire_streams(int device, StreamSet &out);
 void release_streams(int device, StreamSet &s);
 int set_batches(svsdf_ctx *ctx, int nb);
+int forget_long(svsdf_ctx *ctx, size_t P);
+int alloc_long_buffers(svsdf_ctx *ctx, size_t P, size_t cap);
+bool long_auto_on();
+long long long_cap_of(const svsdf_ctx *ctx);
 int choose_tail_iter(const svsdf_ctx *ctx);
 int swept_field(svsdf_ctx *ctx, int N, const double *coeffs, const double *T, double *sdf_sorted);
 int evaluate_points(svsdf_ctx *ctx, int N, const double *coeffs, const double *T, bool allow_cull, bool with_partial);
diff --git a/implicit-svsdf-planner_amd/csrc/svsdf_group.hip b/implicit-svsdf-planner_amd/csrc/svsdf_group.hip
--- a/implicit-svsdf-planner_amd/csrc/svsdf_group.hip
+++ b/implicit-svsdf-planner_amd/csrc/svsdf_group.hip
@@ -127,6 +127,8 @@
     t.tail_launches = std::max(t.tail_launches, a.tail_launches);
     t.tail_iter = std::max(t.tail_iter, a.tail_iter);
     t.tail_points += a.tail_points;
+    t.long_points += a.long_points;
+    t.long_dropped += a.long_dropped;
     t.tail_ms = std::max(t.tail_ms, a.tail_ms); t.tail_ms_sum = std::max(t.tail_ms_sum, a.tail_ms_sum);
     t.gsip_iterations = std::max(t.gsip_iterations, a.gsip_iterations);
     t.gsip_bound_mode = std::max(t.gsip_bound_mode, a.gsip_bound_mode);
diff --git a/implicit-svsdf-planner_amd/csrc/svsdf_kernels.hpp b/implicit-svsdf-planner_amd/csrc/svsdf_kernels.hpp
--- a/implicit-svsdf-planner_amd/csrc/svsdf_kernels.hpp
+++ b/implicit-svsdf-planner_amd/csrc/svsdf_kernels.hpp
@@ -63,9 +63,25 @@
   unsigned rwork[kMaxIter + 2];
   int nonfinite;
   int n_int;
+  int long_cursor[2];
+  int long_n_in;
+  int long_from, long_cap, long_out;
+  unsigned long_hist[kMaxIter];
+  int *long_list;
   StatSlot stat[kStatSlots];
   unsigned long long clk[2];
 };
+
+struct PointSel { const int *list; const int *count_ptr; const unsigned char *skip; };
+__device__ __forceinline__ void long_append(BatchCtl *ctl0, int point) {
+  const int k = atomicAdd(&ctl0->long_cursor[ctl0->long_out], 1);
+  if (k < ctl0->long_cap) ctl0->long_list[k] = point;
+}
+__device__ __forceinline__ void long_record(BatchCtl *ctl0, int point, int life) {
+  atomicAdd(&ctl0->long_hist[life < kMaxIter - 1 ? life : kMaxIter - 1], 1u);
+  const int from = ctl0->long_from;
+  if (from > 0 && life >= from) long_append(ctl0, point);
+}
 
 typedef const __attribute__((address_space(4))) double *UniformDoubles;
 
@@ -392,9 +408,24 @@
 __global__ void __launch_bounds__(1024) k_prep(const double *__restrict__ in, int N, double dur, int K, int exact,
                        TrajDev *__restrict__ tr, Pose *__restrict__ pose,
                        Chunk *__restrict__ chunks, double r_bound, BatchCtl *__restrict__ ctl,
-                       int nbatch, int *__restrict__ nonfinite) {
+                       int nbatch, int *__restrict__ nonfinite, int *__restrict__ long_in, int *__restrict__ long_out,
+                       unsigned char *__restrict__ long_flag, int long_use, int long_cap_in, int long_cap_out, int long_o,
+                       int long_from, int long_cap_rec) {
   extern __shared__ double prep_lds[];
   if (threadIdx.x == 0 && nonfinite) *nonfinite = 0;
+  if (long_flag) {
+    const int n_out = min(ctl[0].long_cursor[long_o], long_cap_out), n_in = min(ctl[0].long_cursor[long_o ^ 1], long_cap_in);
+    for (int e = threadIdx.x; e < n_out; e += blockDim.x) long_flag[long_out[e]] = 0;
+    for (int e = threadIdx.x; e < n_in; e += blockDim.x) long_flag[long_in[e]] = 0;
+    __syncthreads();
+    if (long_use)
+      for (int e = threadIdx.x; e < n_in; e += blockDim.x) long_flag[long_in[e]] = 1;
+    if (threadIdx.x == 0) {
+      ctl[0].long_cursor[long_o] = 0; ctl[0].long_n_in = long_use ? n_in : 0;
+      ctl[0].long_from = long_from; ctl[0].long_cap = long_cap_rec; ctl[0].long_out = long_o; ctl[0].long_list = long_out;
+    }
+    for (int r = threadIdx.x; r < kMaxIter; r += blockDim.x) ctl[0].long_hist[r] = 0u;
+  }
   const double *coeffs = in, *T = in + 18 * N, *tk = in + 19 * N, *slack = in + 19 * N + K;
   for (int b = threadIdx.x; b < nbatch; b += blockDim.x) {
     BatchCtl &c = ctl[b];
@@ -515,6 +546,21 @@
   dst[i] = pose_at(tr, t, pc);
 }
 
+__global__ void __launch_bounds__(256) k_long_collect(const int *__restrict__ active, const int *__restrict__ pt,
+                                                      const BatchCtl *__restrict__ ctl, int it, BatchCtl *__restrict__ ctl0) {
+  const int n = ctl->n_active[it], start = ctl->start;
+  const int cap = ctl0->long_cap;
+  int *list = ctl0->long_list;
+  const int lane = (int)(threadIdx.x & 63);
+  for (int e0 = (int)((blockIdx.x * blockDim.x + threadIdx.x) & ~63u); e0 < n; e0 += gridDim.x * blockDim.x) {
+    const int e = e0 + lane;
+    const int cnt = min(64, n - e0);
+    int base = 0;
+    if (lane == 0) base = atomicAdd(&ctl0->long_cursor[ctl0->long_out], cnt);
+    base = __shfl(base, 0, 64);
+    if (e < n && base + lane < cap) list[base + lane] = pt[active[start + e]];
+  }
+}
 #endif
 
 template <int SHAPE>
@@ -553,6 +599,7 @@
   const int *slots;
   const int *seed_k;
   const double *seed_d;
+  const unsigned char *skip;
 };
 
 __device__ __forceinline__ long long qs_total(const QuerySet &qs, int &n) {
@@ -564,7 +611,7 @@
   const int e = (int)(q % n), j = (int)(q / n);
   const int a = qs.list ? qs.list[e] : e;
   slot = (size_t)j * qs.stride + (size_t)qs.base + (size_t)a;
-  return true;
+  return !qs.skip || qs.skip[slot] == 0;
 }
 
 #ifdef SVSDF_SITE_STATS
@@ -1280,7 +1327,7 @@
            const double *__restrict__ py_, const double *__restrict__ sdf_,
            const double *__restrict__ t_, double *__restrict__ res_sdf,
            double *__restrict__ res_t, double *__restrict__ res_gx, double *__restrict__ res_gy,
-           GsipState gs, BatchCtl *__restrict__ ctl, int *__restrict__ n_int, int icap) {
+           GsipState gs, BatchCtl *__restrict__ ctl, int *__restrict__ n_int, int icap, PointSel sel) {
   constexpr bool SC = false;
   const ScaleDev scl{};
 #include "svsdf_body_classify.hpp"
@@ -1291,7 +1338,7 @@
               const double *__restrict__ py_, const double *__restrict__ sdf_,
               const double *__restrict__ t_, double *__restrict__ res_sdf,
               double *__restrict__ res_t, double *__restrict__ res_gx, double *__restrict__ res_gy,
-              GsipState gs, BatchCtl *__restrict__ ctl, int *__restrict__ n_int, int icap, ScaleDev scl) {
+              GsipState gs, BatchCtl *__restrict__ ctl, int *__restrict__ n_int, int icap, PointSel sel, ScaleDev scl) {
   constexpr bool SC = true;
 #include "svsdf_body_classify.hpp"
 }
@@ -2031,176 +2078,19 @@
        GsipState gs, size_t stride, int it0, int prev_mode, double delta, double band_delta, int all_after, int ppw,
        double *__restrict__ res_sdf, double *__restrict__ res_t, double *__restrict__ res_gx, double *__restrict__ res_gy,
        BatchCtl *__restrict__ ctl, int clist_on, int prune) {
-  extern __shared__ double tail_lds[];
-  constexpr int LP = 32;
-  const int n_act = ctl->n_active[it0];
-  const int wave_g = (int)((blockIdx.x * blockDim.x + threadIdx.x) >> 6);
-  if (n_act <= 0 || (int)blockIdx.x * (kTailBlock / 64) * ppw >= n_act) return;
-  const int K = trg->K;
-  const int nch = (K + kChunk - 1) / kChunk;
-  stage_poly_edges<SHAPE>(sp, tail_lds);
-  double *tab_lds = tail_lds + poly_lds_doubles<SHAPE>(sp.nverts);
-  Pose *pose = reinterpret_cast<Pose *>(tab_lds);
-  Chunk *chunks = reinterpret_cast<Chunk *>(tab_lds + 4 * (size_t)K);
-  {
-    const double *src = reinterpret_cast<const double *>(pose_g);
-    for (int i = threadIdx.x; i < 4 * K; i += blockDim.x) tab_lds[i] = src[i];
-    const double *srcc = reinterpret_cast<const double *>(chunks_g);
-    for (int i = threadIdx.x; i < 4 * nch; i += blockDim.x) tab_lds[4 * (size_t)K + i] = srcc[i];
-  }
-  const TrajL tr = stage_traj(trg, tab_lds + 4 * (size_t)K + 4 * (size_t)nch);
-  const size_t tables = poly_lds_doubles<SHAPE>(sp.nverts) + 4 * (size_t)K + 4 * (size_t)nch + (size_t)traj_lds_doubles(tr.N);
-  const bool local = it0 == 0 && (clist_on & 4) != 0;
-  const size_t wave_stride = local ? kTailWaveLds : kTailWaveLds - kTailLocalBytes;
-  char *wave_lds = reinterpret_cast<char *>(tail_lds + ((tables + 1) & ~(size_t)1)) + (threadIdx.x >> 6) * wave_stride;
-  unsigned short *clist_w = reinterpret_cast<unsigned short *>(wave_lds + ((ladder_lds_bytes(2) + 15) & ~(size_t)15));
-  unsigned *qlist = reinterpret_cast<unsigned *>(clist_w + 2 * kMaxCand);
-  GsipState gl = gs;
-  if (local) {
-    double *ld = reinterpret_cast<double *>(qlist + 64);
-    gl.r = ld; gl.theta0 = ld + 2; gl.theta_res = ld + 4;
-    gl.sqx = ld + 6; gl.sqy = gl.sqx + 2 * kMaxSlots; gl.sqth = gl.sqy + 2 * kMaxSlots; gl.sq_ub = gl.sqth + 2 * kMaxSlots;
-    gl.sq_sdf = gl.sq_ub + 2 * kMaxSlots; gl.sq_t = gl.sq_sdf + 2 * kMaxSlots;
-    int *li_ = reinterpret_cast<int *>(gl.sq_t + 2 * kMaxSlots);
-    gl.pt = li_; gl.iter = li_ + 2; gl.nsamp = li_ + 4; gl.phase = li_ + 6; gl.req = reinterpret_cast<unsigned *>(li_ + 8);
-    gl.sq_k = li_ + 10;
-  }
-  const GsipState ga = local ? gl : gs;
-  const size_t stride_a = local ? (size_t)2 : stride;
-  const int start = ctl->start;
-  const int *cur = gs.list[it0 & 1] + start;
-  const int lane = (int)(threadIdx.x & 63);
-  const int h = lane >> 5, l = lane & (LP - 1);
-  const bool duo = ppw == 1 && MODE != 0 && (clist_on & 8) == 0;
-  const int hs = duo ? 0 : h;
-  const unsigned lt_mask = (1u << l) - 1u;
-  unsigned n_eval = 0, n_scan = 0, n_solved = 0, n_spec = 0, n_rscan = 0;
-  unsigned long long rc[16] = {0, 0, 0, 0, 0, 0, 0, 0, 0, 0, 0, 0, 0, 0, 0, 0};
-  unsigned long long sc[12] = {0, 0, 0, 0, 0, 0, 0, 0, 0, 0, 0, 0};
-  const unsigned long long t_wave0 = SVSDF_SITE_CLOCK();
-  int n_emit_tot = 0;
-  const int n_static = (int)(gridDim.x * (blockDim.x >> 6)) * ppw;
-  int q_next = wave_g * ppw, q_end = min(wave_g * ppw + ppw, n_act);
-  bool exhausted = false;
-  int a = -1;
-  int steps = 0;
-  bool own = false;
-  for (int guard = 0; guard < (1 << 24); ++guard) {
-#pragma unroll
-    for (int hh = 0; hh < 2; ++hh) {
-      const int ah = __builtin_amdgcn_readlane(a, hh * 32);
-      if (ah >= 0 || hh >= ppw) continue;
-      if (q_next >= q_end && !exhausted) {
-        unsigned b = 0;
-        if (lane == 0) b = atomicAdd(&ctl->work[min(it0 + 1, kWorkCounters - 1)], (unsigned)kTailFetch);
-        b = __builtin_amdgcn_readfirstlane(b);
-        const long long bb = (long long)b + n_static;
-        if (bb >= n_act) exhausted = true;
-        else { q_next = (int)bb; q_end = (int)min((long long)n_act, bb + kTailFetch); }
-      }
-      if (q_next < q_end) {
-        const int e = q_next++;
-        if (h == hh || duo) {
-          a = cur[e]; steps = 0; own = false;
-          if (local && l == 0 && h == hh) {
-            const size_t ia_ = (size_t)a;
-            gl.pt[hs] = gs.pt[ia_]; gl.r[hs] = gs.r[ia_]; gl.theta0[hs] = gs.theta0[ia_]; gl.theta_res[hs] = gs.theta_res[ia_];
-            gl.iter[hs] = gs.iter[ia_]; gl.nsamp[hs] = gs.nsamp[ia_]; gl.phase[hs] = gs.phase[ia_]; gl.req[hs] = 0u;
-          }
-        }
-      }
-    }
-    if (__builtin_amdgcn_readlane(a, 0) < 0 && __builtin_amdgcn_readlane(a, 32) < 0) break;
-    if (local) {
-      __builtin_amdgcn_fence(__ATOMIC_RELEASE, "workgroup");
-      __builtin_amdgcn_wave_barrier();
-      __builtin_amdgcn_fence(__ATOMIC_ACQUIRE, "workgroup");
-    }
-    RoundOut<1> ro;
-    ro.list_me[0] = false; ro.mlist[0] = 0u; ro.n_emit = 0; ro.push_next = false; ro.finished = false;
-    if (a >= 0) {
-      const double dl = (steps >= all_after) ? 1e300 : delta, bd = (steps >= all_after) ? 1e300 : band_delta;
-      round_point<SHAPE, LP, MODE, true>(sp, pose, chunks, K, nch, px_, py_, ga, stride_a, start, local ? hs : a, dl, bd, res_sdf, res_t, res_gx,
-                                   res_gy, n_rscan, ro, clist_w + (size_t)h * kMaxCand, clist_on, rc, duo ? h : -1,
-                                   (clist_on & 16) ? reinterpret_cast<const ChunkAnchor *>(chunks_g + nch) : nullptr);
-      ++steps;
-      if (ro.n_emit > 0) own = true;
-      if (l == 0 && (!duo || h == 0)) n_emit_tot += ro.n_emit;
-    }
-    const size_t ia = local ? (size_t)hs : (size_t)(a >= 0 ? a : 0);
-    if (ro.finished) a = -1;
-    const unsigned m_mine = (a >= 0 && (!duo || h == 0)) ? ro.mlist[0] : 0u;
-    const int n0 = __popc((unsigned)__builtin_amdgcn_readlane((int)m_mine, 0));
-    const int n1 = __popc((unsigned)__builtin_amdgcn_readlane((int)m_mine, 32));
-    const int nq = n0 + n1;
-    if ((m_mine >> l) & 1u) {
-      const bool seeded = own ? (MODE != 0) : (prev_mode != 0);
-      qlist[(h ? n0 : 0) + __popc(m_mine & lt_mask)] = (unsigned)sample_slot(stride_a, ia, l) | (seeded ? 0x80000000u : 0u);
-    }
-    __builtin_amdgcn_fence(__ATOMIC_RELEASE, "workgroup");
-    __builtin_amdgcn_wave_barrier();
-    __builtin_amdgcn_fence(__ATOMIC_ACQUIRE, "workgroup");
-    if (nq > 0) {
-      if (nq <= 2) {
-        tail_solve_pass<SHAPE, 32>(tr, tk, sp, pose, chunks, K, nch, ga, qlist, 0, nq, prune, wave_lds, n_eval, n_scan, n_solved, n_spec, sc);
-      } else if (nq <= 8) {
-        tail_solve_pass<SHAPE, 8>(tr, tk, sp, pose, chunks, K, nch, ga, qlist, 0, nq, prune, wave_lds, n_eval, n_scan, n_solved, n_spec, sc);
-      } else {
-        for (int base = 0; base < nq; base += 32)
-          tail_solve_pass<SHAPE, 2>(tr, tk, sp, pose, chunks, K, nch, ga, qlist, base, nq, prune, wave_lds, n_eval, n_scan, n_solved, n_spec, sc);
-      }
-      __builtin_amdgcn_fence(__ATOMIC_RELEASE, "workgroup");
-      __builtin_amdgcn_wave_barrier();
-      __builtin_amdgcn_fence(__ATOMIC_ACQUIRE, "workgroup");
-    }
-  }
-  unsigned long long te = (unsigned long long)n_eval + n_scan, ts = n_solved, tc = n_scan, tp = n_spec, tr_ = n_rscan;
-  int em = n_emit_tot;
-#pragma unroll
-  for (int m = 32; m >= 1; m >>= 1) {
-    te += __shfl_xor(te, m, 64); ts += __shfl_xor(ts, m, 64); tc += __shfl_xor(tc, m, 64); tp += __shfl_xor(tp, m, 64);
-    tr_ += __shfl_xor(tr_, m, 64); em += __shfl_xor(em, m, 64);
-  }
-  if (lane == 0 && (te || tr_ || em)) {
-    StatSlot *ss = stat_slot(ctl->stat);
-    if (te) atomicAdd(&ss->evals, te);
-    if (ts) atomicAdd(&ss->solves, ts);
-    if (tc) atomicAdd(&ss->scan, tc);
-    if (tp) atomicAdd(&ss->spec, tp);
-    if (tr_) atomicAdd(&ss->round_scan, tr_);
-    if (em) atomicAdd(&ctl->n_seed[it0], em);
-    if (ts) atomicAdd(&ctl->n_solve[it0], (int)ts);
-  }
-#ifdef SVSDF_SITE_STATS
-  if (lane == 0) {
-    rc[6] = SVSDF_SITE_CLOCK() - t_wave0;
-    StatSlot *ss = stat_slot(ctl->stat);
-    for (int i = 0; i < 8; ++i) if (rc[i]) atomicAdd(&ss->pad[12 + i], rc[i]);
-    for (int i = 8; i < 11; ++i) if (sc[i]) atomicAdd(&ss->pad[i], sc[i]);
-  }
-  {
-    unsigned long long ex = rc[8], ln = rc[12];
-#pragma unroll
-    for (int m = 32; m >= 1; m >>= 1) { ex += __shfl_xor(ex, m, 64); ln += __shfl_xor(ln, m, 64); }
-    if (lane == 0 && ex) { StatSlot *ss = stat_slot(ctl->stat); atomicAdd(&ss->pad[20], ex); atomicAdd(&ss->pad[21], ln); }
-    unsigned long long steps = ex;
-#pragma unroll
-    for (int i = 0; i < 4; ++i) {
-      unsigned long long v = sc[i];
-#pragma unroll
-      for (int m = 32; m >= 1; m >>= 1) v += __shfl_xor(v, m, 64);
-      steps += v;
-    }
-    if (lane == 0) { StatSlot *ss = stat_slot(ctl->stat); atomicMax(&ss->pad[22], steps); atomicMax(&ss->pad[23], rc[6]); }
-  }
-#pragma unroll
-  for (int i = 0; i < 8; ++i) {
-    unsigned long long v = sc[i];
-#pragma unroll
-    for (int m = 32; m >= 1; m >>= 1) v += __shfl_xor(v, m, 64);
-    if (lane == 0 && v) atomicAdd(&stat_slot(ctl->stat)->pad[i], v);
-  }
-#endif
+  constexpr bool REC = false;
+  BatchCtl *const ctl0 = nullptr;
+#include "svsdf_body_tail.hpp"
+}
+template <int SHAPE, int MODE, int WAVES = SVSDF_TAIL_WAVES>
+__global__ void __launch_bounds__(kTailBlock, WAVES)
+k_tail_rec(const TrajDev *__restrict__ trg, const double *__restrict__ tk, const Pose *__restrict__ pose_g,
+           const Chunk *__restrict__ chunks_g, ShapeParams sp, const double *__restrict__ px_, const double *__restrict__ py_,
+           GsipState gs, size_t stride, int it0, int prev_mode, double delta, double band_delta, int all_after, int ppw,
+           double *__restrict__ res_sdf, double *__restrict__ res_t, double *__restrict__ res_gx, double *__restrict__ res_gy,
+           BatchCtl *__restrict__ ctl, int clist_on, int prune, BatchCtl *__restrict__ ctl0) {
+  constexpr bool REC = true;
+#include "svsdf_body_tail.hpp"
 }
 
 __device__ __forceinline__ bool smoothed_l1(double x, double mu, double &f, double &df) {
@@ -2421,6 +2311,7 @@
     if (lane < kMaxIter) {
       stats_out[9 + lane] = ns;
       stats_out[11 + kMaxIter + lane] = na;
+      stats_out[17 + 2 * kMaxIter + lane] = (unsigned long long)ctl[0].long_hist[lane];
     }
     if (lane == 0) {
       unsigned long long in = 0, nf = (unsigned long long)__hip_atomic_load(nonfinite, __ATOMIC_RELAXED, __HIP_MEMORY_SCOPE_AGENT), rem = 0;
@@ -2435,6 +2326,9 @@
       stats_out[11 + 2 * kMaxIter] = (unsigned long long)ctl[0].n_int;
       stats_out[12 + 2 * kMaxIter] = ctl[0].clk[0];
       stats_out[13 + 2 * kMaxIter] = ctl[0].clk[1];
+      stats_out[14 + 2 * kMaxIter] = (unsigned long long)ctl[0].long_cursor[0];
+      stats_out[15 + 2 * kMaxIter] = (unsigned long long)ctl[0].long_cursor[1];
+      stats_out[16 + 2 * kMaxIter] = (unsigned long long)ctl[0].long_n_in;
     }
   }
 }
diff --git a/implicit-svsdf-planner_amd/csrc/svsdf_launch.hpp b/implicit-svsdf-planner_amd/csrc/svsdf_launch.hpp
--- a/implicit-svsdf-planner_amd/csrc/svsdf_launch.hpp
+++ b/implicit-svsdf-planner_amd/csrc/svsdf_launch.hpp
@@ -25,11 +25,13 @@
   GsipState gs; size_t stride; int it0, prev_mode; double delta, band_delta; int all_after, ppw;
   double *res_sdf, *res_t, *res_gx, *res_gy; BatchCtl *ctl; int clist_on, prune;
   int latency;
+  BatchCtl *rec_ctl0 = nullptr;
 };
 struct ClassifyLaunch {
   const TrajDev *traj; ShapeParams sp; const double *px, *py, *sdf, *t; double *res_sdf, *res_t, *res_gx, *res_gy;
   GsipState gs; BatchCtl *ctl; int *n_int; int icap;
   const ScaleDev *scl = nullptr;
+  PointSel sel{};
 };
 constexpr int kScaledLanes[3] = {4, 8, 32};
 inline int scaled_lanes(int G) { return G >= 32 ? 32 : G >= 8 ? 8 : 4; }
diff --git a/implicit-svsdf-planner_amd/csrc/svsdf_pipeline.hip b/implicit-svsdf-planner_amd/csrc/svsdf_pipeline.hip
--- a/implicit-svsdf-planner_amd/csrc/svsdf_pipeline.hip
+++ b/implicit-svsdf-planner_amd/csrc/svsdf_pipeline.hip
@@ -149,6 +149,9 @@
 }
 namespace svsdf_impl {
 
+constexpr int kLongPerCu = 24;
+constexpr bool kLongAuto = true;
+void long_decide(svsdf_ctx *ctx, bool with_long);
 size_t table_lds_doubles(const svsdf_ctx *ctx) {
   return 4 * (size_t)ctx->K + 4 * (size_t)((ctx->K + kChunk - 1) / kChunk);
 }
@@ -238,6 +241,12 @@
     (void)hipEventRecord(ctx->ev_pool[e1], st);
     ctx->round_events.emplace_back(e0, e1);
   }
+  if (ctx->long_rec_from > 0 && it + 1 == ctx->long_rec_from) {
+    const unsigned cgrid = (unsigned)std::max<long long>(1, std::min<long long>((ctx->long_cap_now + 255) / 256, 64));
+    hipLaunchKernelGGL(k_long_collect, dim3(cgrid), dim3(256), 0, st, ctx->gs.list[(it + 1) & 1], ctx->gs.pt, ctx->d_ctl + b, it + 1, ctx->d_ctl);
+    (void)record_launch(ctx, SVSDF_KERNEL_LONG_COLLECT, -1, cgrid, 256, 0, ctx->long_cap_now, b);
+    debug_sync(st, "k_long_collect", b, it + 1);
+  }
 }
 
 size_t tail_lds_bytes(const svsdf_ctx *ctx, bool poly_lds, bool local) {
@@ -245,12 +254,12 @@
   return lds_tables + (kTailBlock / 64) * (local ? kTailWaveLds : kTailWaveLds - kTailLocalBytes);
 }
 
-void launch_tail(svsdf_ctx *ctx, hipStream_t st, int b, int it0) {
+void launch_tail(svsdf_ctx *ctx, hipStream_t st, int b, int it0, bool long_chain = false) {
   const int mode = bound_mode_of(ctx);
   const bool scans = mode != 0;
   const double sel = (scans && !ctx->select_env) ? ctx->scan_delta : ctx->select_delta;
   const int all_it = (scans && !ctx->all_iter_env) ? 7 : ctx->delta_all_iter;
-  const int all_after = (ctx->tail_all_after < 0) ? std::max(0, all_it - it0) : ctx->tail_all_after;
+  const int all_after = (ctx->tail_all_after < 0 || long_chain) ? std::max(0, all_it - it0) : ctx->tail_all_after;
   long long pts = std::max(1, ctx->bcount[b]);
   if (ctx->have_prev_nactive && it0 <= ctx->prev_tail_iter && it0 < kMaxIter)
     pts = std::min<long long>(pts, ctx->prev_nactive[it0] / std::max(1, ctx->nbatch) * 5 / 4 + 64);
@@ -275,7 +284,8 @@
   const TailLaunch a{ctx->d_traj, d_tk, ctx->d_pose, ctx->d_chunks, ctx->sp, ctx->d_px, ctx->d_py, ctx->gs, ctx->icap, it0, mode,
                      sel, ctx->select_delta, all_after, ppw, ctx->d_res_sdf, ctx->d_res_t, ctx->d_res_gx, ctx->d_res_gy,
                      ctx->d_ctl + b, ctx->round_list | (local ? 4 : 0) | (ctx->tail_duo ? 0 : 8) | ((ctx->scan_anchors && ctx->lipschitz_ok) ? 16 : 0), ctx->prune,
-                     (ctx->tail_latency && ppw == 1 && pts <= (long long)ctx->n_cu * 4 * svsdf::kTailLatencyWaves) ? 1 : 0};
+                     (ctx->tail_latency && ppw == 1 && pts <= (long long)ctx->n_cu * 4 * svsdf::kTailLatencyWaves && !long_chain) ? 1 : 0,
+                     long_chain ? ctx->d_ctl : nullptr};
   size_t e0 = 0, e1 = 0;
   if (ctx->profile) { e0 = next_event(ctx); (void)hipEventRecord(ctx->ev_pool[e0], st); }
   const int shape = poly_lds ? (int)kPolygonLds : ctx->cfg.shape_id;
@@ -303,12 +313,48 @@
   return (ctx->prev_nactive[0] <= below) ? 0 : -1;
 }
 
-void launch_classify(svsdf_ctx *ctx, hipStream_t st, int b) {
+bool long_auto_on() { return kLongAuto; }
+long long long_cap_of(const svsdf_ctx *ctx) {
+  const long long c = ctx->long_cap >= 0 ? ctx->long_cap : (long long)ctx->n_cu * kLongPerCu;
+  return std::min<long long>(c, (long long)ctx->P);
+}
+
+int forget_long(svsdf_ctx *ctx, size_t P) {
+  ctx->long_valid = false;
+  ctx->long_n = 0;
+  ctx->long_list_cap[0] = ctx->long_list_cap[1] = 0;
+  if (ctx->d_long_flag && P > 0) HIPCHK(hipMemsetAsync(ctx->d_long_flag, 0, P, ctx->stream));
+  if (ctx->d_ctl) HIPCHK(hipMemsetAsync(&ctx->d_ctl->long_cursor[0], 0, 3 * sizeof(int), ctx->stream));
+  return SVSDF_OK;
+}
+
+void long_decide(svsdf_ctx *ctx, bool with_long) {
+  ctx->long_run = false;
+  ctx->long_rec_from = 0;
+  ctx->long_cap_now = 0;
+  const int nb = ctx->saved_nbatch > 0 ? ctx->saved_nbatch : ctx->nbatch;
+  const long long cap = std::min<long long>(long_cap_of(ctx), (long long)ctx->long_alloc);
+  const bool on = ctx->long_from > 0 || (ctx->long_from < 0 && kLongAuto);
+  if (!with_long || !on || cap <= 0 || ctx->scaled || nb < 2 || choose_tail_iter(ctx) >= 0 ||
+      tail_lds_bytes(ctx, false, false) > ctx->lds_limit)
+    return;
+  ctx->long_cap_now = cap;
+  if (ctx->long_from > 0) ctx->long_rec_from = std::min(ctx->long_from, (int)kMaxIter - 1);
+  else if (ctx->have_long_alive) {
+    for (int r = 1; r < kMaxIter; ++r)
+      if (ctx->long_alive[r] <= cap) { ctx->long_rec_from = ctx->long_alive[r] > 0 ? r : 0; break; }
+  }
+  ctx->long_run = ctx->long_valid && ctx->long_n > 0;
+}
+
+void launch_classify(svsdf_ctx *ctx, hipStream_t st, int b, bool long_chain = false) {
   const unsigned grid = (unsigned)std::min<long long>(((long long)ctx->bcount[b] + kBlock - 1) / kBlock, 2048);
   const size_t lds = (size_t)traj_lds_doubles(ctx->N) * sizeof(double);
-  const ClassifyLaunch a{ctx->d_traj, ctx->sp, ctx->d_px, ctx->d_py, ctx->d_sdf, ctx->d_t, ctx->d_res_sdf, ctx->d_res_t,
-                         ctx->d_res_gx, ctx->d_res_gy, ctx->gs, ctx->d_ctl + b, &ctx->d_ctl->n_int, (int)ctx->icap,
-                         ctx->scaled ? &ctx->scale : nullptr};
+  ClassifyLaunch a{ctx->d_traj, ctx->sp, ctx->d_px, ctx->d_py, ctx->d_sdf, ctx->d_t, ctx->d_res_sdf, ctx->d_res_t,
+                   ctx->d_res_gx, ctx->d_res_gy, ctx->gs, ctx->d_ctl + b, &ctx->d_ctl->n_int, (int)ctx->icap,
+                   ctx->scaled ? &ctx->scale : nullptr};
+  if (long_chain) a.sel = PointSel{ctx->d_long[ctx->long_o ^ 1], &ctx->d_ctl->long_n_in, nullptr};
+  else if (ctx->long_run) a.sel = PointSel{nullptr, nullptr, ctx->d_long_flag};
   if (!launch_k_classify(ctx->cfg.shape_id, grid, lds, st, a) && ctx->launch_err.empty())
     ctx->launch_err = "k_classify: shape not compiled into this build";
   (void)record_launch(ctx, ctx->scaled ? SVSDF_KERNEL_CLASSIFY_SCALED : SVSDF_KERNEL_CLASSIFY, compiled_shape(ctx->cfg.shape_id), grid,
@@ -316,7 +362,7 @@
   debug_sync(st, "k_classify", b, 0);
 }
 
-int upload_traj(svsdf_ctx *ctx, int N, const double *coeffs, const double *T, bool clear_nonfinite = false) {
+int upload_traj(svsdf_ctx *ctx, int N, const double *coeffs, const double *T, bool clear_nonfinite = false, bool with_long = false) {
   if (N < 1 || N > kMaxPieces) return fail(ctx, SVSDF_ERR_INVALID, "N out of range [1, 128]");
   double td = 0.0;
   for (int i = 0; i < N; ++i) td += T[i];
@@ -420,9 +466,14 @@
   ctx->K = (int)K;
   HIPCHK(hipMemcpyAsync(ctx->d_in, ctx->h_in, need * sizeof(double), hipMemcpyHostToDevice, ctx->stream));
   const size_t lds = (size_t)traj_lds_doubles(N) * sizeof(double);
+  long_decide(ctx, with_long);
   hipLaunchKernelGGL(k_prep, dim3(1), dim3(1024), lds, ctx->stream, ctx->d_in, N, dur, (int)K,
                      ctx->piece_time_mode, ctx->d_traj,
-                     ctx->d_pose, ctx->d_chunks, ctx->r_bound, ctx->d_ctl, ctx->nbatch, clear_nonfinite ? ctx->d_nonfinite : nullptr);
+                     ctx->d_pose, ctx->d_chunks, ctx->r_bound, ctx->d_ctl, ctx->nbatch + 1, clear_nonfinite ? ctx->d_nonfinite : nullptr,
+                     ctx->d_long[ctx->long_o ^ 1], ctx->d_long[ctx->long_o], ctx->long_alloc ? ctx->d_long_flag : nullptr, ctx->long_run ? 1 : 0,
+                     (int)std::min<long long>(ctx->long_list_cap[ctx->long_o ^ 1], (long long)ctx->long_alloc),
+                     (int)std::min<long long>(ctx->long_list_cap[ctx->long_o], (long long)ctx->long_alloc), ctx->long_o,
+                     ctx->long_rec_from, (int)ctx->long_cap_now);
   (void)record_launch(ctx, SVSDF_KERNEL_PREP, -1, 1, 1024, lds, (long long)K, 0);
   ctx->ltab_mode = 0;
   return SVSDF_OK;
@@ -507,12 +558,25 @@
   reset_launches(ctx);
   const size_t e_begin = next_event(ctx);
   (void)hipEventRecord(ctx->ev_pool[e_begin], ctx->stream);
-  int rc = upload_traj(ctx, N, coeffs, T, true);
+  int rc = upload_traj(ctx, N, coeffs, T, true, true);
   if (rc) return rc;
   if ((rc = build_layer_tables(ctx))) return rc;
   const bool fork = ctx->nbatch > 1;
   if (fork) HIPCHK(hipEventRecord(ctx->ev_prep, ctx->stream));
   const int m = ctx->tail_iter = choose_tail_iter(ctx);
+  const double cull_thresh = (allow_cull && ctx->cull && ctx->cull_ok) ? ctx->cfg.safety_hor + 1e-9 : std::numeric_limits<double>::infinity();
+  if (ctx->long_run) {
+    const int lb = ctx->nbatch;
+    ctx->bstart[lb] = (int)ctx->P;
+    ctx->bcount[lb] = (int)ctx->long_n;
+    QuerySet ql{};
+    ql.qx = ctx->d_px; ql.qy = ctx->d_py; ql.stride = 0; ql.count_ptr = &ctx->d_ctl->long_n_in;
+    ql.count_fixed = 0; ql.list = ctx->d_long[ctx->long_o ^ 1]; ql.base = 0; ql.n_outer = 1;
+    launch_solve(ctx, ctx->G_env ? ctx->G : default_lanes(ctx, (size_t)ctx->long_n), ctx->stream, ql, ctx->long_n, ctx->d_sdf, ctx->d_t,
+                 ctx->d_ctl + lb, 0, cull_thresh);
+    launch_classify(ctx, ctx->stream, lb, true);
+    launch_tail(ctx, ctx->stream, lb, 0, true);
+  }
   for (int b = 0; b < ctx->nbatch; ++b) {
     hipStream_t st = batch_stream(ctx, b);
     BatchCtl *ctl = ctx->d_ctl + b;
@@ -520,7 +584,7 @@
     QuerySet qm{};
     qm.qx = ctx->d_px; qm.qy = ctx->d_py; qm.stride = 0; qm.count_ptr = nullptr;
     qm.count_fixed = ctx->bcount[b]; qm.list = nullptr; qm.base = ctx->bstart[b]; qm.n_outer = 1;
-    const double cull_thresh = (allow_cull && ctx->cull && ctx->cull_ok) ? ctx->cfg.safety_hor + 1e-9 : std::numeric_limits<double>::infinity();
+    qm.skip = ctx->long_run ? ctx->d_long_flag : nullptr;
     launch_solve(ctx, ctx->G, st, qm, ctx->bcount[b], ctx->d_sdf, ctx->d_t, ctl, 0, cull_thresh);
     launch_classify(ctx, st, b);
     if (m == 0) launch_tail(ctx, st, b, 0);
@@ -569,6 +633,7 @@
 
 int reduce_and_read(svsdf_ctx *ctx, bool with_partial) {
   const int N = ctx->N;
+  const int nctl = ctx->nbatch + (ctx->long_run ? 1 : 0);
   bool host_written = false;
   if (with_partial) {
     const unsigned grid = (unsigned)std::min<size_t>((ctx->P + kBlock - 1) / kBlock, 512);
@@ -587,20 +652,20 @@
       hipLaunchKernelGGL(k_reduce_sc, dim3(grid), dim3(kBlock), lds, ctx->stream, ctx->d_traj, ctx->d_px, ctx->d_py,
                          (int)ctx->P, ctx->d_res_sdf, ctx->d_res_t, ctx->d_res_gx, ctx->d_res_gy,
                          ctx->cfg.safety_hor, ctx->cfg.weight_p, ctx->d_block_partials, ctx->d_nonfinite, ctx->d_out,
-                         ctx->d_ctl, ctx->nbatch, ctx->it_done, (int)kOutPartial, (int)kOutDoubles, ctx->d_ticket, ctx->h_out_dev, fuse,
+                         ctx->d_ctl, nctl, ctx->it_done, (int)kOutPartial, (int)kOutDoubles, ctx->d_ticket, ctx->h_out_dev, fuse,
                          ctx->scale);
     else
       hipLaunchKernelGGL(k_reduce, dim3(grid), dim3(kBlock), lds, ctx->stream, ctx->d_traj, ctx->d_px, ctx->d_py,
                          (int)ctx->P, ctx->d_res_sdf, ctx->d_res_t, ctx->d_res_gx, ctx->d_res_gy,
                          ctx->cfg.safety_hor, ctx->cfg.weight_p, ctx->d_block_partials, ctx->d_nonfinite, ctx->d_out,
-                         ctx->d_ctl, ctx->nbatch, ctx->it_done, (int)kOutPartial, (int)kOutDoubles, ctx->d_ticket, ctx->h_out_dev, fuse);
+                         ctx->d_ctl, nctl, ctx->it_done, (int)kOutPartial, (int)kOutDoubles, ctx->d_ticket, ctx->h_out_dev, fuse);
     if (svsdf_launch_rec *r = record_launch(ctx, ctx->scaled ? SVSDF_KERNEL_REDUCE_SCALED : SVSDF_KERNEL_REDUCE, -1, grid, (unsigned)kBlock, lds,
                                             (long long)ctx->P, 0)) r->fused = fuse;
     if (!fuse) {
       hipLaunchKernelGGL(k_final, dim3((unsigned)plen), dim3(64), 0, ctx->stream, ctx->d_block_partials, (int)grid, ctx->d_sums);
       (void)record_launch(ctx, SVSDF_KERNEL_FINAL, -1, (unsigned)plen, 64, 0, (long long)grid, 0);
       hipLaunchKernelGGL(k_finish, dim3(1), dim3(kBlock), 0, ctx->stream, ctx->d_sums, N, ctx->d_out, ctx->d_ctl,
-                         ctx->nbatch, ctx->it_done, ctx->d_nonfinite,
+                         nctl, ctx->it_done, ctx->d_nonfinite,
                          reinterpret_cast<unsigned long long *>(ctx->d_out + kOutPartial), ctx->h_out_dev, (int)kOutDoubles);
       (void)record_launch(ctx, SVSDF_KERNEL_FINISH, -1, 1, (unsigned)kBlock, 0, 0, 0);
     }
@@ -608,7 +673,7 @@
   } else {
     HIPCHK(hipMemsetAsync(ctx->d_sums, 0, kOutPartial * sizeof(double), ctx->stream));
     hipLaunchKernelGGL(k_finish, dim3(1), dim3(kBlock), 0, ctx->stream, ctx->d_sums, N, ctx->d_out, ctx->d_ctl,
-                       ctx->nbatch, ctx->it_done, ctx->d_nonfinite,
+                       nctl, ctx->it_done, ctx->d_nonfinite,
                        reinterpret_cast<unsigned long long *>(ctx->d_out + kOutPartial), ctx->h_out_dev, (int)kOutDoubles);
     (void)record_launch(ctx, SVSDF_KERNEL_FINISH, -1, 1, (unsigned)kBlock, 0, 0, 0);
     host_written = ctx->h_out_dev != nullptr;
@@ -670,6 +735,22 @@
   ctx->have_prev_nactive = true;
   ctx->stats.tail_iter = ctx->tail_iter;
   ctx->stats.tail_points = (ctx->tail_iter >= 0 && ctx->tail_iter < kMaxIter) ? (unsigned long long)st[11 + kMaxIter + ctx->tail_iter] : 0ull;
+  {
+    const long long appended = (long long)st[14 + 2 * kMaxIter + ctx->long_o];
+    const long long kept = std::min(appended, ctx->long_cap_now);
+    ctx->stats.long_points = ctx->long_run ? (unsigned long long)st[16 + 2 * kMaxIter] : 0ull;
+    ctx->stats.long_dropped = (unsigned long long)(appended - kept);
+    long long tail_alive = 0;
+    for (int r = kMaxIter - 1; r >= 0; --r) {
+      if (ctx->long_run) tail_alive += (long long)st[17 + 2 * kMaxIter + r];
+      ctx->long_alive[r] = (long long)st[11 + kMaxIter + r] + (r > 0 ? tail_alive : 0);
+    }
+    ctx->have_long_alive = ctx->tail_iter < 0;
+    ctx->long_list_cap[ctx->long_o] = ctx->long_rec_from > 0 ? ctx->long_cap_now : 0;
+    ctx->long_valid = ctx->long_rec_from > 0;
+    ctx->long_n = ctx->long_valid ? kept : 0;
+    ctx->long_o ^= 1;
+  }
   if (ctx->adaptive_iters && ctx->tail_iter < 0) ctx->first_iters = std::max(2, std::min((int)st[7] + 1, (int)kMaxIter));
   if (ctx->profile_span && !ctx->profile) {
     float ms = 0.f;
@@ -872,6 +953,20 @@
   return SVSDF_OK;
 }
 
+int alloc_long_buffers(svsdf_ctx *ctx, size_t P, size_t cap) {
+  int rc = 0;
+  cap = std::min(cap, P);
+  ctx->long_alloc = 0;
+  if ((P + cap) * kMaxSlots > 0x7fffffffull) cap = 0;
+  if ((rc = dev_alloc(ctx, &ctx->d_long[0], cap))) return rc;
+  if ((rc = dev_alloc(ctx, &ctx->d_long[1], cap))) return rc;
+  if ((rc = dev_alloc(ctx, &ctx->gs.list[0], P + cap))) return rc;
+  if ((rc = dev_alloc(ctx, &ctx->gs.list[1], P + cap))) return rc;
+  if ((rc = dev_alloc(ctx, &ctx->gs.solve, (P + cap) * kMaxSlots))) return rc;
+  ctx->long_alloc = cap;
+  return forget_long(ctx, P);
+}
+
 int alloc_point_buffers(svsdf_ctx *ctx, size_t P) {
   int rc = 0;
   if ((rc = dev_alloc(ctx, &ctx->d_px, P))) return rc;
@@ -882,9 +977,8 @@
   if ((rc = dev_alloc(ctx, &ctx->d_res_t, P))) return rc;
   if ((rc = dev_alloc(ctx, &ctx->d_res_gx, P))) return rc;
   if ((rc = dev_alloc(ctx, &ctx->d_res_gy, P))) return rc;
-  if ((rc = dev_alloc(ctx, &ctx->gs.list[0], P))) return rc;
-  if ((rc = dev_alloc(ctx, &ctx->gs.list[1], P))) return rc;
-  if ((rc = dev_alloc(ctx, &ctx->gs.solve, P * kMaxSlots))) return rc;
+  if ((rc = dev_alloc(ctx, &ctx->d_long_flag, P))) return rc;
+  if ((rc = alloc_long_buffers(ctx, P, (size_t)std::max<long long>(ctx->long_cap >= 0 ? ctx->long_cap : 0, (long long)ctx->n_cu * kLongPerCu)))) return rc;
   ctx->icap_fitted = false;
   size_t cap0 = std::min(P, std::max<size_t>(P / 2, 4096));
   if (const char *e = std::getenv("SVSDF_ICAP_INIT")) cap0 = std::max<size_t>(1, (size_t)std::atoll(e));
@@ -941,8 +1035,8 @@
   nb = std::max(1, std::min(nb, kMaxBatches));
   const size_t Ps = ctx->P;
   ctx->nbatch = nb;
-  std::vector<BatchCtl> hc(kMaxBatches);
-  std::memset(hc.data(), 0, sizeof(BatchCtl) * kMaxBatches);
+  std::vector<BatchCtl> hc(kMaxBatches + 1);
+  std::memset(hc.data(), 0, sizeof(BatchCtl) * (kMaxBatches + 1));
   for (int b = 0; b < nb; ++b) {
     const size_t s = Ps * (size_t)b / nb, e = Ps * (size_t)(b + 1) / nb;
     ctx->bstart[b] = (int)s;
@@ -950,8 +1044,10 @@
     hc[b].start = (int)s;
     hc[b].count = (int)(e - s);
   }
-  HIPCHK(hipMemcpy(ctx->d_ctl, hc.data(), sizeof(BatchCtl) * kMaxBatches, hipMemcpyHostToDevice));
-  return SVSDF_OK;
+  hc[nb].start = (int)Ps;
+  hc[nb].count = 0;
+  HIPCHK(hipMemcpy(ctx->d_ctl, hc.data(), sizeof(BatchCtl) * (kMaxBatches + 1), hipMemcpyHostToDevice));
+  return forget_long(ctx, Ps);
 }
 
 void CloudPlan::release() {
@@ -1062,6 +1158,7 @@
   if (rcb) return rcb;
   ctx->have_prev_nsolve = false;
   ctx->have_prev_nactive = false;
+  ctx->have_long_alive = false;
   ctx->prev_tail_iter = -1;
   ctx->ub_tune = 0;
   ctx->bt_state = 0;
diff --git a/implicit-svsdf-planner_amd/csrc/svsdf_shape_slice.hip b/implicit-svsdf-planner_amd/csrc/svsdf_shape_slice.hip
--- a/implicit-svsdf-planner_amd/csrc/svsdf_shape_slice.hip
+++ b/implicit-svsdf-planner_amd/csrc/svsdf_shape_slice.hip
@@ -88,9 +88,14 @@
   hipLaunchKernelGGL((k_tail<S, MODE, WAVES>), dim3(grid), dim3(kTailBlock), lds, st, a.traj, a.tk, a.pose, a.chunks, a.sp,  \
                      a.px, a.py, a.gs, a.stride, a.it0, a.prev_mode, a.delta, a.band_delta, a.all_after, a.ppw, a.res_sdf,   \
                      a.res_t, a.res_gx, a.res_gy, a.ctl, a.clist_on, a.prune)
-#define TAIL(MODE) do { if (a.latency) TAIL_W(MODE, kTailLatencyWaves); else TAIL_W(MODE, SVSDF_TAIL_WAVES); } while (0)
+#define TAIL_REC(MODE)                                                                                                      \
+  hipLaunchKernelGGL((k_tail_rec<S, MODE>), dim3(grid), dim3(kTailBlock), lds, st, a.traj, a.tk, a.pose, a.chunks, a.sp,      \
+                     a.px, a.py, a.gs, a.stride, a.it0, a.prev_mode, a.delta, a.band_delta, a.all_after, a.ppw, a.res_sdf,   \
+                     a.res_t, a.res_gx, a.res_gy, a.ctl, a.clist_on, a.prune, a.rec_ctl0)
+#define TAIL(MODE) do { if (a.rec_ctl0) TAIL_REC(MODE); else if (a.latency) TAIL_W(MODE, kTailLatencyWaves); else TAIL_W(MODE, SVSDF_TAIL_WAVES); } while (0)
     if (mode == 3) TAIL(3); else if (mode == 2) TAIL(2); else if (mode == 1) TAIL(1); else TAIL(0);
 #undef TAIL
+#undef TAIL_REC
 #undef TAIL_W
     return true;
   }
@@ -103,10 +108,10 @@
   } else {
     if (a.scl)
       hipLaunchKernelGGL((k_classify_sc<S>), dim3(grid), dim3(kBlock), lds, st, a.traj, a.sp, a.px, a.py, a.sdf, a.t,
-                         a.res_sdf, a.res_t, a.res_gx, a.res_gy, a.gs, a.ctl, a.n_int, a.icap, *a.scl);
+                         a.res_sdf, a.res_t, a.res_gx, a.res_gy, a.gs, a.ctl, a.n_int, a.icap, a.sel, *a.scl);
     else
       hipLaunchKernelGGL((k_classify<S>), dim3(grid), dim3(kBlock), lds, st, a.traj, a.sp, a.px, a.py, a.sdf, a.t,
-                         a.res_sdf, a.res_t, a.res_gx, a.res_gy, a.gs, a.ctl, a.n_int, a.icap);
+                         a.res_sdf, a.res_t, a.res_gx, a.res_gy, a.gs, a.ctl, a.n_int, a.icap, a.sel);
     return true;
   }
 }
diff --git a/implicit-svsdf-planner_amd/svsdf_amd/binding.py b/implicit-svsdf-planner_amd/svsdf_amd/binding.py
--- a/implicit-svsdf-planner_amd/svsdf_amd/binding.py
+++ b/implicit-svsdf-planner_amd/svsdf_amd/binding.py
@@ -68,12 +68,13 @@
                 ("round_ms", C.c_double), ("round_ms_sum", C.c_double), ("batches", C.c_int),
                 ("speculative_evals", C.c_ulonglong), ("plan_settled", C.c_int), ("tail_iter", C.c_int),
                 ("tail_launches", C.c_uint), ("tail_points", C.c_ulonglong), ("tail_ms", C.c_double),
-                ("tail_ms_sum", C.c_double), ("shader_clock_mhz", C.c_double), ("fanout_ms", C.c_double)]
+                ("tail_ms_sum", C.c_double), ("shader_clock_mhz", C.c_double), ("fanout_ms", C.c_double),
+                ("long_points", C.c_ulonglong), ("long_dropped", C.c_ulonglong)]
 
 
 class Plan(C.Structure):
     _fields_ = [("bound_mode", C.c_int), ("batches", C.c_int), ("lanes_per_query", C.c_int), ("tail_iter", C.c_int),
-                ("settled", C.c_int), ("layer_tables", C.c_int)]
+                ("settled", C.c_int), ("layer_tables", C.c_int), ("long_from", C.c_int), ("long_cap", C.c_int)]
 
 
 PLAN_AUTO = -1
@@ -88,7 +89,7 @@
 
 LAUNCH_REC_CAP = 512
 KERNELS = ["prep", "solve", "classify", "round", "tail", "reduce", "final", "finish",
-           "solve_scaled", "classify_scaled", "reduce_scaled", "layer_tables"]
+           "solve_scaled", "classify_scaled", "reduce_scaled", "layer_tables", "long_collect"]
 
 
 class Scale(C.Structure):
@@ -683,8 +684,9 @@
         return {k: getattr(pl, k) for k, _ in Plan._fields_}
 
     def set_plan(self, bound_mode=PLAN_AUTO, batches=PLAN_AUTO, lanes_per_query=PLAN_AUTO, tail_iter=PLAN_AUTO,
-                 layer_tables=PLAN_AUTO):
-        pl = Plan(int(bound_mode), int(batches), int(lanes_per_query), int(tail_iter), 0, int(layer_tables))
+                 layer_tables=PLAN_AUTO, long_from=0, long_cap=PLAN_AUTO):
+        pl = Plan(int(bound_mode), int(batches), int(lanes_per_query), int(tail_iter), 0, int(layer_tables), int(long_from),
+                  int(long_cap))
         self._chk(self.L.svsdf_set_plan(self.ctx, C.byref(pl)), "svsdf_set_plan")
 
     def set_combine(self, combine):
diff --git a/include/svsdf_c.h b/include/svsdf_c.h
--- a/include/svsdf_c.h
+++ b/include/svsdf_c.h
@@ -216,6 +216,8 @@
   double tail_ms_sum;
   double shader_clock_mhz;
   double fanout_ms;
+  unsigned long long long_points;
+  unsigned long long long_dropped;
 } svsdf_stats;
 int svsdf_last_stats(const svsdf_ctx *ctx, svsdf_stats *out);
 
@@ -232,7 +234,8 @@
   SVSDF_KERNEL_SOLVE_SCALED = 8,
   SVSDF_KERNEL_CLASSIFY_SCALED = 9,
   SVSDF_KERNEL_REDUCE_SCALED = 10,
-  SVSDF_KERNEL_LAYER_TABLES = 11
+  SVSDF_KERNEL_LAYER_TABLES = 11,
+  SVSDF_KERNEL_LONG_COLLECT = 12
 };
 typedef struct svsdf_launch_rec {
   int struct_size;
@@ -272,6 +275,8 @@
   int tail_iter;
   int settled;
   int layer_tables;
+  int long_from;
+  int long_cap;
 } svsdf_plan;
 int svsdf_get_plan(const svsdf_ctx *ctx, svsdf_plan *out);
 int svsdf_set_plan(svsdf_ctx *ctx, const svsdf_plan *plan);
```

After: 179.5 million. -2.1%, worse.
